# nimblephysics/nimblephysics

Measured on NVIDIA H100. Metric: differentiable world-steps/sec (fwd+bwd), batched Atlas, higher is better.
Workload: dtype f32

## Files before the change

nimblephysics_b200/csrc/nb2_dyn.cuh:

```cuda
#pragma once
#include <stddef.h>

#include "nb2_math.cuh"
#include "nb2_model.h"
#include "../../include/nb2.h"

namespace nb2 {

#define NB2_FWD_BODY_WORDS 16
struct FwdLayout {
  int oQ, oV, oAct, oBody, oSlot, oFree, total;
};
NB2_HD FwdLayout fwd_layout(int nb, int n, int nslots, int nfree) {
  FwdLayout L;
  L.oQ = 0; L.oV = n; L.oAct = 2 * n; L.oBody = 3 * n;
  L.oSlot = L.oBody + NB2_FWD_BODY_WORDS * nb;
  L.oFree = L.oSlot + 27 * nslots;
  L.total = L.oFree + 18 * nfree;
  return L;
}
struct BwdLayout {
  int oGQ, oGV, oLam, oQb, oVb, oSt, oAct, oBody, oSlot, oFree, total;
};
NB2_HD BwdLayout bwd_layout(int nb, int n, int nslots, int nfree, int slotw = 18) {
  BwdLayout L;
  L.oGQ = 0; L.oGV = n; L.oLam = 2 * n; L.oQb = 3 * n; L.oVb = 4 * n; L.oSt = 5 * n; L.oAct = 7 * n; L.oBody = 8 * n;
  L.oSlot = L.oBody + 7 * nb;
  L.oFree = L.oSlot + slotw * nslots;
  L.total = L.oFree + 6 * nfree;
  return L;
}

template <class R, int ST> NB2_HD V6<R> ld6(const R* p) {
  V6<R> v; v.a.x = p[0]; v.a.y = p[ST]; v.a.z = p[2 * ST]; v.l.x = p[3 * ST]; v.l.y = p[4 * ST]; v.l.z = p[5 * ST]; return v;
}
template <class R, int ST> NB2_HD void st6(R* p, const V6<R>& v) {
  p[0] = v.a.x; p[ST] = v.a.y; p[2 * ST] = v.a.z; p[3 * ST] = v.l.x; p[4 * ST] = v.l.y; p[5 * ST] = v.l.z;
}
template <class R, int ST> NB2_HD void add6(R* p, const V6<R>& v) {
  p[0] += v.a.x; p[ST] += v.a.y; p[2 * ST] += v.a.z; p[3 * ST] += v.l.x; p[4 * ST] += v.l.y; p[5 * ST] += v.l.z;
}
template <class R, int ST> NB2_HD SI<R> ldSI(const R* p) {
  SI<R> I;
  I.A.xx = p[0]; I.A.yy = p[ST]; I.A.zz = p[2 * ST]; I.A.xy = p[3 * ST]; I.A.xz = p[4 * ST]; I.A.yz = p[5 * ST];
  I.B.m00 = p[6 * ST]; I.B.m01 = p[7 * ST]; I.B.m02 = p[8 * ST]; I.B.m10 = p[9 * ST]; I.B.m11 = p[10 * ST]; I.B.m12 = p[11 * ST];
  I.B.m20 = p[12 * ST]; I.B.m21 = p[13 * ST]; I.B.m22 = p[14 * ST];
  I.C.xx = p[15 * ST]; I.C.yy = p[16 * ST]; I.C.zz = p[17 * ST]; I.C.xy = p[18 * ST]; I.C.xz = p[19 * ST]; I.C.yz = p[20 * ST];
  return I;
}
template <class R, int ST, bool ADD> NB2_HD void stSI(R* p, const SI<R>& I) {
#define NB2_W(k, val) if (ADD) p[(k) * ST] += (val); else p[(k) * ST] = (val);
  NB2_W(0, I.A.xx) NB2_W(1, I.A.yy) NB2_W(2, I.A.zz) NB2_W(3, I.A.xy) NB2_W(4, I.A.xz) NB2_W(5, I.A.yz)
  NB2_W(6, I.B.m00) NB2_W(7, I.B.m01) NB2_W(8, I.B.m02) NB2_W(9, I.B.m10) NB2_W(10, I.B.m11) NB2_W(11, I.B.m12)
  NB2_W(12, I.B.m20) NB2_W(13, I.B.m21) NB2_W(14, I.B.m22)
  NB2_W(15, I.C.xx) NB2_W(16, I.C.yy) NB2_W(17, I.C.zz) NB2_W(18, I.C.xy) NB2_W(19, I.C.xz) NB2_W(20, I.C.yz)
#undef NB2_W
}
template <class R> NB2_HD void sv_st6(R* sv, size_t B, int k, const V6<R>& v) {
  sv[(size_t)k * B] = v.a.x; sv[(size_t)(k + 1) * B] = v.a.y; sv[(size_t)(k + 2) * B] = v.a.z;
  sv[(size_t)(k + 3) * B] = v.l.x; sv[(size_t)(k + 4) * B] = v.l.y; sv[(size_t)(k + 5) * B] = v.l.z;
}
template <class R> NB2_HD V6<R> tof(const V6<R>& v) { return v; }
template <class R> NB2_HD V6<R> sv_ld6(const R* sv, size_t B, int k) {
  V6<R> v;
  v.a.x = (R)sv[(size_t)k * B]; v.a.y = (R)sv[(size_t)(k + 1) * B]; v.a.z = (R)sv[(size_t)(k + 2) * B];
  v.l.x = (R)sv[(size_t)(k + 3) * B]; v.l.y = (R)sv[(size_t)(k + 4) * B]; v.l.z = (R)sv[(size_t)(k + 5) * B];
  return v;
}

#define NB2_BT_WORDS 22
template <class R> NB2_HD Xf<R> xtree(const Nb2ModelDev<R>& M, const R* bt, int i) {
  Xf<R> T;
  if (bt) {
    const R* t = bt + NB2_BT_WORDS * i;
    T.R_.m00 = t[0]; T.R_.m01 = t[1]; T.R_.m02 = t[2]; T.R_.m10 = t[3]; T.R_.m11 = t[4]; T.R_.m12 = t[5];
    T.R_.m20 = t[6]; T.R_.m21 = t[7]; T.R_.m22 = t[8];
    T.p = mk3<R>(t[9], t[10], t[11]);
    return T;
  }
  T.R_.m00 = M.Xtree[i][0]; T.R_.m01 = M.Xtree[i][1]; T.R_.m02 = M.Xtree[i][2];
  T.R_.m10 = M.Xtree[i][3]; T.R_.m11 = M.Xtree[i][4]; T.R_.m12 = M.Xtree[i][5];
  T.R_.m20 = M.Xtree[i][6]; T.R_.m21 = M.Xtree[i][7]; T.R_.m22 = M.Xtree[i][8];
  T.p = mk3<R>(M.Xtree[i][9], M.Xtree[i][10], M.Xtree[i][11]);
  return T;
}
template <class R> NB2_HD Xf<R> xtree(const Nb2ModelDev<R>& M, int i) { return xtree<R>(M, (const R*)nullptr, i); }
template <class R> NB2_HD Xf<R> xf_rev(const Nb2ModelDev<R>& M, const R* bt, int i, R s, R c) {
  Xf<R> X = xtree(M, bt, i), T;
  T.R_.m00 = c * X.R_.m00 + s * X.R_.m01; T.R_.m01 = c * X.R_.m01 - s * X.R_.m00; T.R_.m02 = X.R_.m02;
  T.R_.m10 = c * X.R_.m10 + s * X.R_.m11; T.R_.m11 = c * X.R_.m11 - s * X.R_.m10; T.R_.m12 = X.R_.m12;
  T.R_.m20 = c * X.R_.m20 + s * X.R_.m21; T.R_.m21 = c * X.R_.m21 - s * X.R_.m20; T.R_.m22 = X.R_.m22;
  T.p = X.p;
  return T;
}
template <class R> NB2_HD Xf<R> xf_rev(const Nb2ModelDev<R>& M, int i, R s, R c) { return xf_rev<R>(M, (const R*)nullptr, i, s, c); }
template <class R> NB2_HD Xf<R> xf_pris(const Nb2ModelDev<R>& M, const R* bt, int i, R d) {
  Xf<R> T = xtree(M, bt, i);
  T.p.x += T.R_.m02 * d; T.p.y += T.R_.m12 * d; T.p.z += T.R_.m22 * d;
  return T;
}
template <class R> NB2_HD Xf<R> xf_pris(const Nb2ModelDev<R>& M, int i, R d) { return xf_pris<R>(M, (const R*)nullptr, i, d); }
template <class R> NB2_HD void inertia_of(const Nb2ModelDev<R>& M, const R* bt, const double* wi, size_t wiB, int i, R* m, V3<R>* h, S3<R>* Ib) {
  if (wi) {
    const double* t = wi + (size_t)(10 * i) * wiB;
    *m = (R)t[0]; *h = mk3<R>((R)t[wiB], (R)t[2 * wiB], (R)t[3 * wiB]);
    Ib->xx = (R)t[4 * wiB]; Ib->yy = (R)t[5 * wiB]; Ib->zz = (R)t[6 * wiB];
    Ib->xy = (R)t[7 * wiB]; Ib->xz = (R)t[8 * wiB]; Ib->yz = (R)t[9 * wiB];
    return;
  }
  if (bt) {
    const R* t = bt + NB2_BT_WORDS * i + 12;
    *m = t[0]; *h = mk3<R>(t[1], t[2], t[3]);
    Ib->xx = t[4]; Ib->yy = t[5]; Ib->zz = t[6]; Ib->xy = t[7]; Ib->xz = t[8]; Ib->yz = t[9];
    return;
  }
  *m = M.inertia[i][0];
  *h = mk3<R>(M.inertia[i][1], M.inertia[i][2], M.inertia[i][3]);
  Ib->xx = M.inertia[i][4]; Ib->yy = M.inertia[i][5]; Ib->zz = M.inertia[i][6];
  Ib->xy = M.inertia[i][7]; Ib->xz = M.inertia[i][8]; Ib->yz = M.inertia[i][9];
}
template <class R, int ST> NB2_HD Xf<R> ldXf(const R* p) {
  Xf<R> T;
  T.R_.m00 = p[0]; T.R_.m01 = p[ST]; T.R_.m02 = p[2 * ST]; T.R_.m10 = p[3 * ST]; T.R_.m11 = p[4 * ST]; T.R_.m12 = p[5 * ST];
  T.R_.m20 = p[6 * ST]; T.R_.m21 = p[7 * ST]; T.R_.m22 = p[8 * ST];
  T.p = mk3<R>(p[9 * ST], p[10 * ST], p[11 * ST]);
  return T;
}
template <class R, int ST> NB2_HD void stXf(R* p, const Xf<R>& T) {
  p[0] = T.R_.m00; p[ST] = T.R_.m01; p[2 * ST] = T.R_.m02; p[3 * ST] = T.R_.m10; p[4 * ST] = T.R_.m11; p[5 * ST] = T.R_.m12;
  p[6 * ST] = T.R_.m20; p[7 * ST] = T.R_.m21; p[8 * ST] = T.R_.m22; p[9 * ST] = T.p.x; p[10 * ST] = T.p.y; p[11 * ST] = T.p.z;
}
template <class R, int ST> NB2_HD Xf<R> body_xf_fwd(const Nb2ModelDev<R>& M, const R* bt, int i, const R* scr, const FwdLayout& L) {
  const int jt = M.jtype[i];
  if (jt == NB2_JT_REV) { const R* b = scr + (size_t)(L.oBody + NB2_FWD_BODY_WORDS * i + 6) * ST; return xf_rev(M, bt, i, b[0], b[ST]); }
  if (jt == NB2_JT_PRIS) return xf_pris(M, bt, i, scr[(size_t)(L.oQ + M.dof_off[i]) * ST]);
  return ldXf<R, ST>(scr + (size_t)(L.oFree + 18 * M.free_idx[i]) * ST);
}
template <class R> NB2_HD V6<R> S_times(int jt, R x) {
  V6<R> s = zero6<R>();
  if (jt == NB2_JT_REV) s.a.z = x; else s.l.z = x;
  return s;
}
template <class R> NB2_HD R S_dot(int jt, const V6<R>& f) { return (jt == NB2_JT_REV) ? f.a.z : f.l.z; }

template <class R, int ST> NB2_HD R tau_of(const Nb2ModelDev<R>& M, const R* scr, int oAct, int d) {
  const int a = M.act_of_dof[d];
  return (a >= 0) ? scr[(size_t)(oAct + a) * ST] : R(0);
}

template <class R, int ST>
NB2_HD void fwd_pass1(const Nb2ModelDev<R>& M, R* scr, int lo, int hi, const R* bt = nullptr) {
  const int nb = M.nb, n = M.ndof;
  const FwdLayout L = fwd_layout(nb, n, M.nslots, M.nfree);
  const R dt = M.dt;
  (void)nb; (void)n; (void)dt;
  for (int i = lo; i < hi; i++) {
    const int jt = M.jtype[i], p = M.parent[i], o = M.dof_off[i];
    R* bs = scr + (size_t)(L.oBody + NB2_FWD_BODY_WORDS * i) * ST;
    V6<R> Vp = (p >= 0) ? ld6<R, ST>(scr + (size_t)(L.oBody + NB2_FWD_BODY_WORDS * p) * ST) : zero6<R>();
    V6<R> V;
    if (jt == NB2_JT_REV) {
      R s, c; nb2_sincos(scr[(size_t)(L.oQ + o) * ST], &s, &c);
      bs[6 * ST] = s; bs[7 * ST] = c;
      V = AdInvT(xf_rev(M, bt, i, s, c), Vp);
      V.a.z += scr[(size_t)(L.oV + o) * ST];
    } else if (jt == NB2_JT_PRIS) {
      V = AdInvT(xf_pris(M, bt, i, scr[(size_t)(L.oQ + o) * ST]), Vp);
      V.l.z += scr[(size_t)(L.oV + o) * ST];
    } else {
      const R* q = scr + (size_t)(L.oQ + o) * ST;
      const R* v = scr + (size_t)(L.oV + o) * ST;
      Xf<R> X = xtree(M, bt, i), T;
      M3<R> Rq = expmap(mk3<R>(q[0], q[ST], q[2 * ST]));
      T.R_ = mul(X.R_, Rq);
      T.p = mul(X.R_, mk3<R>(q[3 * ST], q[4 * ST], q[5 * ST])) + X.p;
      stXf<R, ST>(scr + (size_t)(L.oFree + 18 * M.free_idx[i]) * ST, T);
      V = AdInvT(T, Vp) + ld6<R, ST>(v);
    }
    st6<R, ST>(bs, V);
  }

}

template <class R, int ST>
NB2_HD void fwd_pass2(const Nb2ModelDev<R>& M, R* scr, R* sv, size_t B, bool save, int lo, int hi, const R* bt = nullptr, R* iinv_out = nullptr,
                      const double* wi = nullptr, size_t wiB = 0) {
  const int nb = M.nb, n = M.ndof;
  const FwdLayout L = fwd_layout(nb, n, M.nslots, M.nfree);
  const R dt = M.dt;
  (void)nb; (void)n; (void)dt;
  SI<R> hI = zeroSI<R>();
  V6<R> hp = zero6<R>();
  bool hvalid = false;
  for (int i = hi - 1; i >= lo; i--) {
    const int jt = M.jtype[i], p = M.parent[i], o = M.dof_off[i], fl = M.flags[i];
    R* bs = scr + (size_t)(L.oBody + NB2_FWD_BODY_WORDS * i) * ST;
    R m; V3<R> h; S3<R> Ib; inertia_of(M, bt, wi, wiB, i, &m, &h, &Ib);
    const V6<R> V = ld6<R, ST>(bs);
    SI<R> IA = rigidSI(m, h, Ib);
    V6<R> pA = crf(V, mulG(m, h, Ib, V));
    if (hvalid) { IA = IA + hI; pA = pA + hp; }
    if (fl & NB2_F_HAS_SLOT) {
      for (int k = 0; k < M.slot_count[i]; k++) {
        const R* sl = scr + (size_t)(L.oSlot + 27 * (M.slot_self[i] + k)) * ST;
        IA = IA + ldSI<R, ST>(sl);
        pA = pA + ld6<R, ST>(sl + 21 * ST);
      }
    }
    SI<R> Pi; V6<R> beta;
    if (jt != NB2_JT_FREE) {
      const R vq = scr[(size_t)(L.oV + o) * ST];
      V6<R> U, eta;
      R D;
      if (jt == NB2_JT_REV) {
        U.a = mk3<R>(IA.A.xz, IA.A.yz, IA.A.zz); U.l = mk3<R>(IA.B.m20, IA.B.m21, IA.B.m22); D = IA.A.zz;
        eta.a = mk3<R>(V.a.y * vq, -V.a.x * vq, R(0)); eta.l = mk3<R>(V.l.y * vq, -V.l.x * vq, R(0));
      } else {
        U.a = mk3<R>(IA.B.m02, IA.B.m12, IA.B.m22); U.l = mk3<R>(IA.C.xz, IA.C.yz, IA.C.zz); D = IA.C.zz;
        eta.a = zero3<R>(); eta.l = mk3<R>(V.a.y * vq, -V.a.x * vq, R(0));
      }
      const R psi = nb2_rcp(D);
      const R qv = scr[(size_t)(L.oQ + o) * ST];
      const R u = tau_of<R, ST>(M, scr, L.oAct, o) - M.spring[o] * (qv - M.rest[o] + vq * dt) - M.damping[o] * vq
                  - (dot(U, eta) + S_dot(jt, pA));
      st6<R, ST>(bs + 8 * ST, U);
      bs[14 * ST] = psi; bs[15 * ST] = u;
      if (p >= 0) {
        const R k = -psi;
        Pi = IA;
        Pi.A.xx += k * U.a.x * U.a.x; Pi.A.yy += k * U.a.y * U.a.y; Pi.A.zz += k * U.a.z * U.a.z;
        Pi.A.xy += k * U.a.x * U.a.y; Pi.A.xz += k * U.a.x * U.a.z; Pi.A.yz += k * U.a.y * U.a.z;
        Pi.C.xx += k * U.l.x * U.l.x; Pi.C.yy += k * U.l.y * U.l.y; Pi.C.zz += k * U.l.z * U.l.z;
        Pi.C.xy += k * U.l.x * U.l.y; Pi.C.xz += k * U.l.x * U.l.z; Pi.C.yz += k * U.l.y * U.l.z;
        Pi.B.m00 += k * U.a.x * U.l.x; Pi.B.m01 += k * U.a.x * U.l.y; Pi.B.m02 += k * U.a.x * U.l.z;
        Pi.B.m10 += k * U.a.y * U.l.x; Pi.B.m11 += k * U.a.y * U.l.y; Pi.B.m12 += k * U.a.y * U.l.z;
        Pi.B.m20 += k * U.a.z * U.l.x; Pi.B.m21 += k * U.a.z * U.l.y; Pi.B.m22 += k * U.a.z * U.l.z;
        beta = pA + mul(IA, eta) + U * (psi * u);
      }
    } else {
      const R* q = scr + (size_t)(L.oQ + o) * ST;
      const R* v = scr + (size_t)(L.oV + o) * ST;
      R t[6];
#pragma unroll
      for (int k = 0; k < 6; k++) t[k] = tau_of<R, ST>(M, scr, L.oAct, o + k);
      const V6<R> Vj = ld6<R, ST>(v);
      const V6<R> eta = ad(V, Vj);
      const V6<R> bf = mul(IA, eta) + pA;
      V6<R> u;
      u.a.x = t[0] - M.spring[o] * (q[0] - M.rest[o] + Vj.a.x * dt) - M.damping[o] * Vj.a.x - bf.a.x;
      u.a.y = t[1] - M.spring[o + 1] * (q[ST] - M.rest[o + 1] + Vj.a.y * dt) - M.damping[o + 1] * Vj.a.y - bf.a.y;
      u.a.z = t[2] - M.spring[o + 2] * (q[2 * ST] - M.rest[o + 2] + Vj.a.z * dt) - M.damping[o + 2] * Vj.a.z - bf.a.z;
      u.l.x = t[3] - M.spring[o + 3] * (q[3 * ST] - M.rest[o + 3] + Vj.l.x * dt) - M.damping[o + 3] * Vj.l.x - bf.l.x;
      u.l.y = t[4] - M.spring[o + 4] * (q[4 * ST] - M.rest[o + 4] + Vj.l.y * dt) - M.damping[o + 4] * Vj.l.y - bf.l.y;
      u.l.z = t[5] - M.spring[o + 5] * (q[5 * ST] - M.rest[o + 5] + Vj.l.z * dt) - M.damping[o + 5] * Vj.l.z - bf.l.z;
      const SI<R> Iinv = spd6_inverse(IA);
      const V6<R> y = mul(Iinv, u);
      st6<R, ST>(scr + (size_t)(L.oFree + 18 * M.free_idx[i] + 12) * ST, y);
      if (iinv_out) stSI<R, 1, false>(iinv_out + 21 * M.free_idx[i], Iinv);
      if (save) {
        const int k0 = nb * 21 + M.free_idx[i] * 33;
        R* s = sv + (size_t)k0 * B;
        s[0] = (R)Iinv.A.xx; s[B] = (R)Iinv.A.yy; s[2 * B] = (R)Iinv.A.zz; s[3 * B] = (R)Iinv.A.xy; s[4 * B] = (R)Iinv.A.xz; s[5 * B] = (R)Iinv.A.yz;
        s[6 * B] = (R)Iinv.B.m00; s[7 * B] = (R)Iinv.B.m01; s[8 * B] = (R)Iinv.B.m02; s[9 * B] = (R)Iinv.B.m10; s[10 * B] = (R)Iinv.B.m11; s[11 * B] = (R)Iinv.B.m12;
        s[12 * B] = (R)Iinv.B.m20; s[13 * B] = (R)Iinv.B.m21; s[14 * B] = (R)Iinv.B.m22;
        s[15 * B] = (R)Iinv.C.xx; s[16 * B] = (R)Iinv.C.yy; s[17 * B] = (R)Iinv.C.zz; s[18 * B] = (R)Iinv.C.xy; s[19 * B] = (R)Iinv.C.xz; s[20 * B] = (R)Iinv.C.yz;
      }
      if (p >= 0) { Pi = zeroSI<R>(); beta = bf + u; }
    }
    hvalid = false;
    if (p >= 0) {
      const Xf<R> T = body_xf_fwd<R, ST>(M, bt, i, scr, L);
      const SI<R> Ic = xform_inertia(T, Pi);
      const V6<R> pc = dAdInvT(T, beta);
      if (fl & NB2_F_HANDOFF) { hI = Ic; hp = pc; hvalid = true; }
      else {
        R* sl = scr + (size_t)(L.oSlot + 27 * M.slot_parent[i]) * ST;
        stSI<R, ST, false>(sl, Ic); st6<R, ST>(sl + 21 * ST, pc);
      }
    }
  }

}

template <class R, int ST>
NB2_HD void fwd_pass3(const Nb2ModelDev<R>& M, R* scr, R* sv, size_t B, bool save, int lo, int hi, const R* bt = nullptr) {
  const int nb = M.nb, n = M.ndof;
  const FwdLayout L = fwd_layout(nb, n, M.nslots, M.nfree);
  const R dt = M.dt;
  (void)nb; (void)n; (void)dt;
  V6<R> A0; A0.a = zero3<R>(); A0.l = mk3<R>(-M.gravity[0], -M.gravity[1], -M.gravity[2]);
  for (int i = lo; i < hi; i++) {
    const int jt = M.jtype[i], p = M.parent[i], o = M.dof_off[i];
    R* bs = scr + (size_t)(L.oBody + NB2_FWD_BODY_WORDS * i) * ST;
    const Xf<R> T = body_xf_fwd<R, ST>(M, bt, i, scr, L);
    const V6<R> Ap = AdInvT(T, (p >= 0) ? ld6<R, ST>(scr + (size_t)(L.oBody + NB2_FWD_BODY_WORDS * p) * ST) : A0);
    const V6<R> V = ld6<R, ST>(bs);
    V6<R> A;
    if (jt != NB2_JT_FREE) {
      const R vq = scr[(size_t)(L.oV + o) * ST], qv = scr[(size_t)(L.oQ + o) * ST];
      const V6<R> U = ld6<R, ST>(bs + 8 * ST);
      const R psi = bs[14 * ST], u = bs[15 * ST];
      const R qdd = psi * (u - dot(U, Ap));
      A = Ap;
      if (jt == NB2_JT_REV) { A.a.z += qdd; A.a.x += V.a.y * vq; A.a.y -= V.a.x * vq; A.l.x += V.l.y * vq; A.l.y -= V.l.x * vq; }
      else { A.l.z += qdd; A.l.x += V.a.y * vq; A.l.y -= V.a.x * vq; }
      scr[(size_t)(L.oQ + o) * ST] = qv + vq * dt;
      scr[(size_t)(L.oV + o) * ST] = vq + qdd * dt;
      if (save) {
        R* s = sv + (size_t)(i * 21) * B;
        sv_st6(s, B, 0, tof(V)); sv_st6(s, B, 6, tof(A)); sv_st6(s, B, 12, tof(U));
        s[18 * B] = (R)psi;
        s[19 * B] = (jt == NB2_JT_REV) ? (R)bs[6 * ST] : R(0); s[20 * B] = (jt == NB2_JT_REV) ? (R)bs[7 * ST] : R(0);
        sv[(size_t)(nb * 21 + M.nfree * 33 + o) * B] = qdd;
      }
    } else {
      const R* q = scr + (size_t)(L.oQ + o) * ST;
      const R* fr = scr + (size_t)(L.oFree + 18 * M.free_idx[i]) * ST;
      const V6<R> Vj = ld6<R, ST>(scr + (size_t)(L.oV + o) * ST);
      const V6<R> y = ld6<R, ST>(fr + 12 * ST);
      const V6<R> qdd = y - Ap;
      A = y + ad(V, Vj);
      const V3<R> phi = mk3<R>(q[0], q[ST], q[2 * ST]);
      const M3<R> Rq = expmap(phi);
      const V3<R> phin = logmap(mul(Rq, expmap(Vj.a * dt)));
      const V3<R> pn = mk3<R>(q[3 * ST], q[4 * ST], q[5 * ST]) + mul(Rq, Vj.l * dt);
      R* qo = scr + (size_t)(L.oQ + o) * ST;
      R* vo = scr + (size_t)(L.oV + o) * ST;
      qo[0] = phin.x; qo[ST] = phin.y; qo[2 * ST] = phin.z; qo[3 * ST] = pn.x; qo[4 * ST] = pn.y; qo[5 * ST] = pn.z;
      vo[0] = Vj.a.x + qdd.a.x * dt; vo[ST] = Vj.a.y + qdd.a.y * dt; vo[2 * ST] = Vj.a.z + qdd.a.z * dt;
      vo[3 * ST] = Vj.l.x + qdd.l.x * dt; vo[4 * ST] = Vj.l.y + qdd.l.y * dt; vo[5 * ST] = Vj.l.z + qdd.l.z * dt;
      if (save) {
        R* s = sv + (size_t)(i * 21) * B;
        sv_st6(s, B, 0, tof(V)); sv_st6(s, B, 6, tof(A));
        for (int k = 12; k < 21; k++) s[(size_t)k * B] = R(0);
        R* sf = sv + (size_t)(nb * 21 + M.free_idx[i] * 33 + 21) * B;
        for (int k = 0; k < 12; k++) sf[(size_t)k * B] = fr[(size_t)k * ST];
        R* sq = sv + (size_t)(nb * 21 + M.nfree * 33 + o) * B;
        sq[0] = qdd.a.x; sq[B] = qdd.a.y; sq[2 * B] = qdd.a.z; sq[3 * B] = qdd.l.x; sq[4 * B] = qdd.l.y; sq[5 * B] = qdd.l.z;
      }
    }
    st6<R, ST>(bs, A);
  }
}

#define NB2_IO_UNROLL 4
struct alignas(16) F4 { float x, y, z, w; };
NB2_HD unsigned fast_div(unsigned idx, unsigned magic) {
#ifdef __CUDA_ARCH__
  return __umulhi(idx, magic);
#else
  return (unsigned)(((unsigned long long)idx * magic) >> 32);
#endif
}
template <class F> NB2_HD void group_read(const float* src, int tot, int tid, int nthr, const F& f) {
  if ((((size_t)src) & 15) == 0) {
    const F4* s4 = reinterpret_cast<const F4*>(src);
    const int tot4 = tot >> 2;
    for (int base = tid; base < tot4; base += nthr * NB2_IO_UNROLL) {
      F4 v[NB2_IO_UNROLL];
#pragma unroll
      for (int u = 0; u < NB2_IO_UNROLL; u++) { const int j = base + u * nthr; if (j < tot4) v[u] = s4[j]; }
#pragma unroll
      for (int u = 0; u < NB2_IO_UNROLL; u++) {
        const int j = base + u * nthr;
        if (j < tot4) { f(4 * j, v[u].x); f(4 * j + 1, v[u].y); f(4 * j + 2, v[u].z); f(4 * j + 3, v[u].w); }
      }
    }
    for (int idx = 4 * tot4 + tid; idx < tot; idx += nthr) f(idx, src[idx]);
  } else {
    for (int base = tid; base < tot; base += nthr * NB2_IO_UNROLL) {
      float v[NB2_IO_UNROLL];
#pragma unroll
      for (int u = 0; u < NB2_IO_UNROLL; u++) { const int idx = base + u * nthr; v[u] = (idx < tot) ? src[idx] : 0.f; }
#pragma unroll
      for (int u = 0; u < NB2_IO_UNROLL; u++) { const int idx = base + u * nthr; if (idx < tot) f(idx, v[u]); }
    }
  }
}
template <class F> NB2_HD void group_write(float* dst, int tot, int tid, int nthr, const F& f) {
  if ((((size_t)dst) & 15) == 0) {
    F4* d4 = reinterpret_cast<F4*>(dst);
    const int tot4 = tot >> 2;
    for (int j = tid; j < tot4; j += nthr) { F4 v; v.x = f(4 * j); v.y = f(4 * j + 1); v.z = f(4 * j + 2); v.w = f(4 * j + 3); d4[j] = v; }
    for (int idx = 4 * tot4 + tid; idx < tot; idx += nthr) dst[idx] = f(idx);
  } else {
    for (int idx = tid; idx < tot; idx += nthr) dst[idx] = f(idx);
  }
}

template <class R, int ST> struct WordScatter {
  R* scr0; int width, base; unsigned magic; float* copy;
  NB2_HD void operator()(int idx, float v) const {
    const int slot = (int)fast_div((unsigned)idx, magic), d = idx - slot * width;
    scr0[(size_t)(base + d) * ST + slot] = (R)v;
    if (copy) copy[idx] = v;
  }
};
template <class R, int ST> struct WordGather {
  const R* scr0; int width, base; unsigned magic;
  NB2_HD float operator()(int idx) const {
    const int slot = (int)fast_div((unsigned)idx, magic), d = idx - slot * width;
    return (float)scr0[(size_t)(base + d) * ST + slot];
  }
};

template <class R, int ST>
NB2_HD void fwd_load(const Nb2ModelDev<R>& M, R* scr0, const float* st0, const float* act0, int nworlds, int tid, int nthr,
                     float* st_copy0 = nullptr, float* act_copy0 = nullptr) {
  const int n2 = 2 * M.ndof, na = M.na;
  const FwdLayout L = fwd_layout(M.nb, M.ndof, M.nslots, M.nfree);
  WordScatter<R, ST> ss{scr0, n2, L.oQ, M.magic_n2, st_copy0};
  group_read(st0, nworlds * n2, tid, nthr, ss);
  WordScatter<R, ST> as{scr0, na, L.oAct, M.magic_na, act_copy0};
  group_read(act0, nworlds * na, tid, nthr, as);
}
template <class R, int ST>
NB2_HD void fwd_store(const Nb2ModelDev<R>& M, const R* scr0, float* out0, int nworlds, int tid, int nthr) {
  const int n2 = 2 * M.ndof;
  const FwdLayout L = fwd_layout(M.nb, M.ndof, M.nslots, M.nfree);
  WordGather<R, ST> sg{scr0, n2, L.oQ, M.magic_n2};
  group_write(out0, nworlds * n2, tid, nthr, sg);
}

#define NB2_FWD_STAGES 8
#define NB2_FWD_SYNC_MASK 0x6Bu
#define NB2_FWD_SYNC_MASK_1LANE 0x41u
template <class R, int ST>
NB2_HD void world_forward_stage(const Nb2ModelDev<R>& M, R* scr, R* sv, size_t B, bool save, int lane, int stage, const R* bt = nullptr, R* iinv_out = nullptr,
                                const double* wi = nullptr, size_t wiB = 0) {
  const int pass = (stage + 1) >> 1;
  const bool trunk = (stage == 1) | (stage == 4) | (stage == 5);
  if (trunk && lane != 0) return;
  const int nr = trunk ? M.trunk_n : M.limb_n[lane];
  for (int rr = 0; rr < nr; rr++) {
    const int r = (pass == 2) ? nr - 1 - rr : rr;
    const int lo = trunk ? M.trunk_lo[r] : M.limb_lo[lane][r], hi = trunk ? M.trunk_hi[r] : M.limb_hi[lane][r];
    if (pass == 1) fwd_pass1<R, ST>(M, scr, lo, hi, bt);
    else if (pass == 2) fwd_pass2<R, ST>(M, scr, sv, B, save, lo, hi, bt, iinv_out, wi, wiB);
    else fwd_pass3<R, ST>(M, scr, sv, B, save, lo, hi, bt);
  }
}

template <class T, int ST> struct SPd { T* p; NB2_HD T& operator[](int i) const { return p[(size_t)i * ST]; } NB2_HD SPd operator+(int k) const { SPd r; r.p = p + (size_t)k * ST; return r; } };
template <int ST>
struct BwdContactData {
  SPd<double, ST> Aacc, Uplus, aeff, vplus, inj, JcTmu;
  const int16_t* inj_of_body;
  int active; int error;
  int bounce = 0, pass2 = 0;
};

NB2_HD float mul_rn(float a, float b) {
#ifdef __CUDA_ARCH__
  return __fmul_rn(a, b);
#else
  return a * b;
#endif
}
NB2_HD double mul_rn(double a, double b) {
#ifdef __CUDA_ARCH__
  return __dmul_rn(a, b);
#else
  return a * b;
#endif
}
template <class R> NB2_HD V3<R> cross_rn(const V3<R>& a, const V3<R>& b) {
  return mk3<R>(mul_rn(a.y, b.z) - mul_rn(a.z, b.y), mul_rn(a.z, b.x) - mul_rn(a.x, b.z), mul_rn(a.x, b.y) - mul_rn(a.y, b.x));
}
template <class R> NB2_HD void inertia_param_form(const V6<R>& Y, const V6<R>& X, R* t) {
  t[0] = mul_rn(Y.l.x, X.l.x) + mul_rn(Y.l.y, X.l.y) + mul_rn(Y.l.z, X.l.z);
  const V3<R> dh = cross_rn(X.l, Y.a) + cross_rn(Y.l, X.a);
  t[1] = dh.x; t[2] = dh.y; t[3] = dh.z;
  t[4] = mul_rn(Y.a.x, X.a.x); t[5] = mul_rn(Y.a.y, X.a.y); t[6] = mul_rn(Y.a.z, X.a.z);
  t[7] = mul_rn(Y.a.x, X.a.y) + mul_rn(Y.a.y, X.a.x); t[8] = mul_rn(Y.a.x, X.a.z) + mul_rn(Y.a.z, X.a.x);
  t[9] = mul_rn(Y.a.y, X.a.z) + mul_rn(Y.a.z, X.a.y);
}

template <class R, int ST, bool CONTACT>
NB2_HD void bwd_B1(const Nb2ModelDev<R>& M, R* scr, const float* st, const R* sv, size_t B, int lo, int hi, const R* bt = nullptr) {
  const int nb = M.nb, n = M.ndof;
  constexpr int SLOTW = CONTACT ? 42 : 18;
  const BwdLayout L = bwd_layout(nb, n, M.nslots, M.nfree, SLOTW);
  const R dt = M.dt;
  const int kFree = nb * 21, kQdd = nb * 21 + M.nfree * 33;
  (void)n; (void)dt; (void)kFree; (void)kQdd;
  V6<R> hp = zero6<R>();
  bool hvalid = false;
  for (int i = hi - 1; i >= lo; i--) {
    const int jt = M.jtype[i], p = M.parent[i], o = M.dof_off[i], fl = M.flags[i];
    const R* s = sv + (size_t)(i * 21) * B;
    V6<R> pI = hvalid ? hp : zero6<R>();
    if (fl & NB2_F_HAS_SLOT)
      for (int k = 0; k < M.slot_count[i]; k++) pI = pI + ld6<R, ST>(scr + (size_t)(L.oSlot + SLOTW * (M.slot_self[i] + k)) * ST);
    V6<R> beta;
    if (jt != NB2_JT_FREE) {
      const R up = scr[(size_t)(L.oGV + o) * ST] - S_dot(jt, pI);
      scr[(size_t)(L.oBody + 7 * i) * ST] = up;
      if (p >= 0) beta = pI + sv_ld6<R>(s, B, 12) * ((R)s[18 * B] * up);
    } else {
      const V6<R> up = ld6<R, ST>(scr + (size_t)(L.oGV + o) * ST) - pI;
      st6<R, ST>(scr + (size_t)(L.oFree + 6 * M.free_idx[i]) * ST, up);
      if (p >= 0) beta = pI + up;
    }
    hvalid = false;
    if (p >= 0) {
      Xf<R> T;
      if (jt == NB2_JT_REV) T = xf_rev(M, bt, i, (R)s[19 * B], (R)s[20 * B]);
      else if (jt == NB2_JT_PRIS) T = xf_pris(M, bt, i, scr[(size_t)(L.oSt + o) * ST]);
      else { R t12[12]; for (int k = 0; k < 12; k++) t12[k] = (R)sv[(size_t)(kFree + M.free_idx[i] * 33 + 21 + k) * B]; T = ldXf<R, 1>(t12); }
      const V6<R> pc = dAdInvT(T, beta);
      if (fl & NB2_F_HANDOFF) { hp = pc; hvalid = true; }
      else {
        R* sl = scr + (size_t)(L.oSlot + SLOTW * M.slot_parent[i]) * ST;
        st6<R, ST>(sl, pc);
      }
    }
  }
}

template <class R, int ST, bool CONTACT>
NB2_HD void bwd_B2(const Nb2ModelDev<R>& M, R* scr, const float* st, const R* sv, size_t B, int lo, int hi, const R* bt = nullptr) {
  const int nb = M.nb, n = M.ndof;
  constexpr int SLOTW = CONTACT ? 42 : 18;
  const BwdLayout L = bwd_layout(nb, n, M.nslots, M.nfree, SLOTW);
  const R dt = M.dt;
  const int kFree = nb * 21, kQdd = nb * 21 + M.nfree * 33;
  (void)n; (void)dt; (void)kFree; (void)kQdd;
  for (int i = lo; i < hi; i++) {
    const int jt = M.jtype[i], p = M.parent[i], o = M.dof_off[i];
    const R* s = sv + (size_t)(i * 21) * B;
    R* bs = scr + (size_t)(L.oBody + 7 * i) * ST;
    V6<R> W;
    if (jt != NB2_JT_FREE) {
      Xf<R> T = (jt == NB2_JT_REV) ? xf_rev(M, bt, i, (R)s[19 * B], (R)s[20 * B]) : xf_pris(M, bt, i, scr[(size_t)(L.oSt + o) * ST]);
      W = (p >= 0) ? AdInvT(T, ld6<R, ST>(scr + (size_t)(L.oBody + 7 * p + 1) * ST)) : zero6<R>();
      const R lam = (R)s[18 * B] * (bs[0] - dot(sv_ld6<R>(s, B, 12), W));
      scr[(size_t)(L.oLam + o) * ST] = lam;
      if (jt == NB2_JT_REV) W.a.z += lam; else W.l.z += lam;
    } else {
      const R* sf = sv + (size_t)(kFree + M.free_idx[i] * 33) * B;
      R t12[12]; for (int k = 0; k < 12; k++) t12[k] = (R)sf[(size_t)(21 + k) * B];
      const Xf<R> T = ldXf<R, 1>(t12);
      const V6<R> Wp = (p >= 0) ? AdInvT(T, ld6<R, ST>(scr + (size_t)(L.oBody + 7 * p + 1) * ST)) : zero6<R>();
      R i21[21]; for (int k = 0; k < 21; k++) i21[k] = (R)sf[(size_t)k * B];
      const SI<R> Iinv = ldSI<R, 1>(i21);
      W = mul(Iinv, ld6<R, ST>(scr + (size_t)(L.oFree + 6 * M.free_idx[i]) * ST));
      st6<R, ST>(scr + (size_t)(L.oLam + o) * ST, W - Wp);
    }
    st6<R, ST>(bs + ST, W);
  }
}

template <class R, int ST, bool CONTACT>
NB2_HD void bwd_B3(const Nb2ModelDev<R>& M, R* scr, const float* st, const R* sv, size_t B, const BwdContactData<ST>& cd, int lo, int hi,
                   float* gI = nullptr, const R* bt = nullptr, size_t gIB = 0, const double* wi = nullptr, size_t wiB = 0, double* gIa = nullptr) {
  const int nb = M.nb, n = M.ndof;
  constexpr int SLOTW = CONTACT ? 42 : 18;
  const BwdLayout L = bwd_layout(nb, n, M.nslots, M.nfree, SLOTW);
  const R dt = M.dt;
  const int kFree = nb * 21, kQdd = nb * 21 + M.nfree * 33;
  (void)n; (void)dt; (void)kFree; (void)kQdd;
  V6<R> hA = zero6<R>(), hV = zero6<R>(), hf = zero6<R>();
  V6<R> hUw = zero6<R>(), hUp = zero6<R>(), hG = zero6<R>(), hH = zero6<R>();
  bool hvalid = false;
  for (int i = hi - 1; i >= lo; i--) {
    const int jt = M.jtype[i], p = M.parent[i], o = M.dof_off[i], fl = M.flags[i];
    const R* s = sv + (size_t)(i * 21) * B;
    R m; V3<R> h; S3<R> Ib; inertia_of(M, bt, wi, wiB, i, &m, &h, &Ib);
    const V6<R> V = sv_ld6<R>(s, B, 0);
    V6<R> A = sv_ld6<R>(s, B, 6);
    if (CONTACT && cd.active && !cd.pass2) { const auto a6 = cd.Aacc + 6 * i; A.a = mk3<R>((R)a6[0], (R)a6[1], (R)a6[2]); A.l = mk3<R>((R)a6[3], (R)a6[4], (R)a6[5]); }
    const V6<R> W = ld6<R, ST>(scr + (size_t)(L.oBody + 7 * i + 1) * ST);
    const V6<R> GV = mulG(m, h, Ib, V);
    V6<R> f = mulG(m, h, Ib, A) + crf(V, GV);
    if (gI || gIa) {
      V6<R> Y2;
      Y2.a = cross_rn(V.a, W.a);
      Y2.l = cross_rn(V.a, W.l) + cross_rn(V.l, W.a);
      R t[10];
      inertia_param_form(W, A, t);
      R t2[10];
      inertia_param_form(Y2, V, t2);
#pragma unroll
      for (int k = 0; k < 10; k++) {
        const float gk = (float)(-dt * (t[k] - t2[k]));
        if (gIa) gIa[(size_t)(10 * i + k) * gIB] += (double)gk;
        else if (CONTACT && cd.pass2) gI[(size_t)(10 * i + k) * gIB] += gk; else gI[(size_t)(10 * i + k) * gIB] = gk;
      }
    }
    V6<R> Abar = mulG(m, h, Ib, W);
    V6<R> Vbar = mulG(m, h, Ib, ad(W, V)) - crf(W, GV);
    if (hvalid) { Abar = Abar + hA; Vbar = Vbar + hV; f = f + hf; }
    V6<R> Uw = zero6<R>(), Up = zero6<R>(), Gc = zero6<R>(), Hc = zero6<R>();
    if (CONTACT && cd.active) {
      const int ci = cd.inj_of_body[i];
      if (ci >= 0) {
        const auto b24 = cd.inj + 24 * ci;
        Uw.a = mk3<R>((R)b24[0], (R)b24[1], (R)b24[2]); Uw.l = mk3<R>((R)b24[3], (R)b24[4], (R)b24[5]);
        Up.a = mk3<R>((R)b24[6], (R)b24[7], (R)b24[8]); Up.l = mk3<R>((R)b24[9], (R)b24[10], (R)b24[11]);
        Gc.a = mk3<R>((R)b24[12], (R)b24[13], (R)b24[14]); Gc.l = mk3<R>((R)b24[15], (R)b24[16], (R)b24[17]);
        Hc.a = mk3<R>((R)b24[18], (R)b24[19], (R)b24[20]); Hc.l = mk3<R>((R)b24[21], (R)b24[22], (R)b24[23]);
      }
      if (hvalid) { Uw = Uw + hUw; Up = Up + hUp; Gc = Gc + hG; Hc = Hc + hH; }
    }
    if (fl & NB2_F_HAS_SLOT) {
      for (int k = 0; k < M.slot_count[i]; k++) {
        const R* sl = scr + (size_t)(L.oSlot + SLOTW * (M.slot_self[i] + k)) * ST;
        Abar = Abar + ld6<R, ST>(sl); Vbar = Vbar + ld6<R, ST>(sl + 6 * ST); f = f + ld6<R, ST>(sl + 12 * ST);
        if (CONTACT && cd.active) { Uw = Uw + ld6<R, ST>(sl + 18 * ST); Up = Up + ld6<R, ST>(sl + 24 * ST); Gc = Gc + ld6<R, ST>(sl + 30 * ST); Hc = Hc + ld6<R, ST>(sl + 36 * ST); }
      }
    }
    V6<R> Sv, Sa, Sl;
    Xf<R> T;
    if (jt != NB2_JT_FREE) {
      Sv = S_times<R>(jt, scr[(size_t)(L.oSt + n + o) * ST]);
      Sa = S_times<R>(jt, (CONTACT && cd.active && !cd.pass2) ? (R)cd.aeff[o] : (R)sv[(size_t)(kQdd + o) * B]);
      Sl = S_times<R>(jt, scr[(size_t)(L.oLam + o) * ST]);
      T = (jt == NB2_JT_REV) ? xf_rev(M, bt, i, (R)s[19 * B], (R)s[20 * B]) : xf_pris(M, bt, i, scr[(size_t)(L.oSt + o) * ST]);
    } else {
      Sv.a = mk3<R>(scr[(size_t)(L.oSt + n + o) * ST], scr[(size_t)(L.oSt + n + o + 1) * ST], scr[(size_t)(L.oSt + n + o + 2) * ST]); Sv.l = mk3<R>(scr[(size_t)(L.oSt + n + o + 3) * ST], scr[(size_t)(L.oSt + n + o + 4) * ST], scr[(size_t)(L.oSt + n + o + 5) * ST]);
      Sa = sv_ld6<R>(sv + (size_t)(kQdd + o) * B, B, 0);
      if (CONTACT && cd.active && !cd.pass2) { const auto a6 = cd.aeff + o; Sa.a = mk3<R>((R)a6[0], (R)a6[1], (R)a6[2]); Sa.l = mk3<R>((R)a6[3], (R)a6[4], (R)a6[5]); }
      Sl = ld6<R, ST>(scr + (size_t)(L.oLam + o) * ST);
      R t12[12]; for (int k = 0; k < 12; k++) t12[k] = (R)sv[(size_t)(kFree + M.free_idx[i] * 33 + 21 + k) * B];
      T = ldXf<R, 1>(t12);
    }
    Vbar = Vbar + crf(Sv, Abar);
    const V6<R> vb6 = Vbar - crf(V, Abar);
    const V6<R> Alam = A - Sa - ad(V, Sv), Vlam = V - Sv, Wlam = W - Sl;
    V6<R> c6 = zero6<R>() - (crf(Alam, Abar) + crf(Vlam, Vbar) + crf(Wlam, f));
    if (CONTACT && cd.active) {
      V6<R> Upl; { const auto u6 = cd.Uplus + 6 * i; Upl.a = mk3<R>((R)u6[0], (R)u6[1], (R)u6[2]); Upl.l = mk3<R>((R)u6[3], (R)u6[4], (R)u6[5]); }
      V6<R> Svp;
      if (jt != NB2_JT_FREE) Svp = S_times<R>(jt, (R)cd.vplus[o]);
      else { const auto v6p = cd.vplus + o; Svp.a = mk3<R>((R)v6p[0], (R)v6p[1], (R)v6p[2]); Svp.l = mk3<R>((R)v6p[3], (R)v6p[4], (R)v6p[5]); }
      c6 = c6 - crf(Wlam, Uw) - crf(Upl - Svp, Up) + Gc;
      if (!cd.pass2) {
        if (jt != NB2_JT_FREE) cd.JcTmu[o] = (double)S_dot(jt, Hc);
        else { auto j6 = cd.JcTmu + o; j6[0] = (double)Hc.a.x; j6[1] = (double)Hc.a.y; j6[2] = (double)Hc.a.z; j6[3] = (double)Hc.l.x; j6[4] = (double)Hc.l.y; j6[5] = (double)Hc.l.z; }
      }
    }
    const bool add = CONTACT && cd.pass2;
    if (jt != NB2_JT_FREE) {
      const R vb = S_dot(jt, vb6), qb = S_dot(jt, c6);
      scr[(size_t)(L.oVb + o) * ST] = add ? scr[(size_t)(L.oVb + o) * ST] + vb : vb;
      scr[(size_t)(L.oQb + o) * ST] = add ? scr[(size_t)(L.oQb + o) * ST] + qb : qb;
    } else {
      const V3<R> phi = mk3<R>(scr[(size_t)(L.oSt + o) * ST], scr[(size_t)(L.oSt + o + 1) * ST], scr[(size_t)(L.oSt + o + 2) * ST]);
      V6<R> qb, vb = vb6;
      qb.a = mulT(so3_Jr(phi), c6.a);
      qb.l = mul(expmap(phi), c6.l);
      if (add) { vb = vb + ld6<R, ST>(scr + (size_t)(L.oVb + o) * ST); qb = qb + ld6<R, ST>(scr + (size_t)(L.oQb + o) * ST); }
      st6<R, ST>(scr + (size_t)(L.oVb + o) * ST, vb);
      st6<R, ST>(scr + (size_t)(L.oQb + o) * ST, qb);
    }
    hvalid = false;
    if (p >= 0) {
      const V6<R> cA = dAdInvT(T, Abar), cV = dAdInvT(T, Vbar), cf = dAdInvT(T, f);
      V6<R> cUw, cUp, cG, cH;
      if (CONTACT && cd.active) { cUw = dAdInvT(T, Uw); cUp = dAdInvT(T, Up); cG = dAdInvT(T, Gc); cH = dAdInvT(T, Hc); }
      if (fl & NB2_F_HANDOFF) { hA = cA; hV = cV; hf = cf; if (CONTACT && cd.active) { hUw = cUw; hUp = cUp; hG = cG; hH = cH; } hvalid = true; }
      else {
        R* sl = scr + (size_t)(L.oSlot + SLOTW * M.slot_parent[i]) * ST;
        st6<R, ST>(sl, cA); st6<R, ST>(sl + 6 * ST, cV); st6<R, ST>(sl + 12 * ST, cf);
        if (CONTACT && cd.active) { st6<R, ST>(sl + 18 * ST, cUw); st6<R, ST>(sl + 24 * ST, cUp); st6<R, ST>(sl + 30 * ST, cG); st6<R, ST>(sl + 36 * ST, cH); }
      }
    }
  }
}

template <class R, int ST>
NB2_HD void finish_dof(const Nb2ModelDev<R>& M, R* scr, const BwdLayout& L, int d, R gq_, R gv_, R lam) {
  const int n = M.ndof;
  float gq = (float)gq_, gv = (float)gv_;
  const float qd = (float)scr[(size_t)(L.oSt + d) * ST], vd = (float)scr[(size_t)(L.oSt + n + d) * ST];
  if (qd == M.pos_lo[d] && gq > 0.f) gq = 0.f;
  if (qd == M.pos_hi[d] && gq < 0.f) gq = 0.f;
  if (vd == M.vel_lo[d] && gv > 0.f) gv = 0.f;
  if (vd == M.vel_hi[d] && gv < 0.f) gv = 0.f;
  scr[(size_t)(L.oQb + d) * ST] = (R)gq;
  scr[(size_t)(L.oVb + d) * ST] = (R)gv;
  const int a = M.act_of_dof[d];
  if (a >= 0) {
    float gt = (float)(M.dt * lam);
    const float fd = (float)scr[(size_t)(L.oAct + a) * ST];
    if (fd == M.force_lo[d] && gt > 0.f) gt = 0.f;
    if (fd == M.force_hi[d] && gt < 0.f) gt = 0.f;
    scr[(size_t)(L.oAct + a) * ST] = (R)gt;
  }
}

template <class R, int ST, bool CONTACT>
NB2_HD void bwd_assemble(const Nb2ModelDev<R>& M, R* scr, const float* st, const BwdContactData<ST>& cd, int lo, int hi) {
  const int nb = M.nb, n = M.ndof;
  constexpr int SLOTW = CONTACT ? 42 : 18;
  const BwdLayout L = bwd_layout(nb, n, M.nslots, M.nfree, SLOTW);
  const R dt = M.dt;
  const int kFree = nb * 21, kQdd = nb * 21 + M.nfree * 33;
  (void)n; (void)dt; (void)kFree; (void)kQdd;
  for (int i = lo; i < hi; i++) {
    const int jt = M.jtype[i], o = M.dof_off[i];
    if (jt != NB2_JT_FREE) {
      const R lam = scr[(size_t)(L.oLam + o) * ST];
      const R gq = scr[(size_t)(L.oGQ + o) * ST];
      R gv = scr[(size_t)(L.oGV + o) * ST];
      if (CONTACT && cd.active) gv -= (R)cd.JcTmu[o];
      finish_dof<R, ST>(M, scr, L, o, gq - dt * (scr[(size_t)(L.oQb + o) * ST] + M.spring[o] * lam),
                        dt * gq + gv - dt * (scr[(size_t)(L.oVb + o) * ST] + (M.damping[o] + dt * M.spring[o]) * lam), lam);
    } else {
      const V3<R> phi = mk3<R>(scr[(size_t)(L.oSt + o) * ST], scr[(size_t)(L.oSt + o + 1) * ST], scr[(size_t)(L.oSt + o + 2) * ST]);
      const V3<R> w = mk3<R>(scr[(size_t)(L.oSt + n + o) * ST], scr[(size_t)(L.oSt + n + o + 1) * ST], scr[(size_t)(L.oSt + n + o + 2) * ST]);
      const V3<R> vl = mk3<R>(scr[(size_t)(L.oSt + n + o + 3) * ST], scr[(size_t)(L.oSt + n + o + 4) * ST], scr[(size_t)(L.oSt + n + o + 5) * ST]);
      const M3<R> Rq = expmap(phi), E = expmap(w * dt);
      const V3<R> phin = logmap(mul(Rq, E));
      const V6<R> g = ld6<R, ST>(scr + (size_t)(L.oGQ + o) * ST);
      const V3<R> t = mulT(so3_Jr_inv(phin), g.a);
      V6<R> gq, gvp;
      gq.a = mulT(so3_Jr(phi), mul(E, t) + cross(vl * dt, mulT(Rq, g.l)));
      gq.l = g.l;
      gvp.a = mulT(so3_Jr(w * dt), t) * dt;
      gvp.l = mulT(Rq, g.l) * dt;
      const V6<R> lam = ld6<R, ST>(scr + (size_t)(L.oLam + o) * ST);
      const V6<R> qb = ld6<R, ST>(scr + (size_t)(L.oQb + o) * ST), vb = ld6<R, ST>(scr + (size_t)(L.oVb + o) * ST);
      V6<R> gv = ld6<R, ST>(scr + (size_t)(L.oGV + o) * ST);
      if (CONTACT && cd.active) { const auto j6 = cd.JcTmu + o; gv.a = gv.a - mk3<R>((R)j6[0], (R)j6[1], (R)j6[2]); gv.l = gv.l - mk3<R>((R)j6[3], (R)j6[4], (R)j6[5]); }
      R lamv[6] = {lam.a.x, lam.a.y, lam.a.z, lam.l.x, lam.l.y, lam.l.z};
      R qbv[6] = {qb.a.x, qb.a.y, qb.a.z, qb.l.x, qb.l.y, qb.l.z}, vbv[6] = {vb.a.x, vb.a.y, vb.a.z, vb.l.x, vb.l.y, vb.l.z};
      R gqv[6] = {gq.a.x, gq.a.y, gq.a.z, gq.l.x, gq.l.y, gq.l.z}, gvpv[6] = {gvp.a.x, gvp.a.y, gvp.a.z, gvp.l.x, gvp.l.y, gvp.l.z};
      R gvv[6] = {gv.a.x, gv.a.y, gv.a.z, gv.l.x, gv.l.y, gv.l.z};
#pragma unroll
      for (int k = 0; k < 6; k++) {
        finish_dof<R, ST>(M, scr, L, o + k, gqv[k] - dt * (qbv[k] + M.spring[o + k] * lamv[k]),
                          gvpv[k] + gvv[k] - dt * (vbv[k] + (M.damping[o + k] + dt * M.spring[o + k]) * lamv[k]), lamv[k]);
      }
    }
  }
}

template <class R, int ST, bool CONTACT>
NB2_HD void bwd_load(const Nb2ModelDev<R>& M, R* scr0, const float* st0, const float* act0, const float* gnext0, int nworlds, int tid, int nthr) {
  const int n = M.ndof, n2 = 2 * n;
  constexpr int SLOTW = CONTACT ? 42 : 18;
  const BwdLayout L = bwd_layout(M.nb, n, M.nslots, M.nfree, SLOTW);
  WordScatter<R, ST> sg{scr0, n2, L.oGQ, M.magic_n2, nullptr};
  group_read(gnext0, nworlds * n2, tid, nthr, sg);
  WordScatter<R, ST> sx{scr0, n2, L.oSt, M.magic_n2, nullptr};
  group_read(st0, nworlds * n2, tid, nthr, sx);
  WordScatter<R, ST> sa{scr0, M.na, L.oAct, M.magic_na, nullptr};
  group_read(act0, nworlds * M.na, tid, nthr, sa);
}
struct NanGather { NB2_HD float operator()(int) const { return nanf(""); } };
template <class F> struct AddTo { F f; const float* dst; NB2_HD float operator()(int idx) const { return dst[idx] + f(idx); } };
template <class R, int ST, bool CONTACT>
NB2_HD void bwd_store(const Nb2ModelDev<R>& M, const R* scr0, float* gstate0, float* gaction0,
                      bool cd_error, int nworlds, int tid, int nthr, bool accumulate_state = false) {
  const int n = M.ndof, n2 = 2 * n, na = M.na;
  constexpr int SLOTW = CONTACT ? 42 : 18;
  const BwdLayout L = bwd_layout(M.nb, n, M.nslots, M.nfree, SLOTW);
  if (cd_error) {
    group_write(gstate0, nworlds * n2, tid, nthr, NanGather());
    group_write(gaction0, nworlds * na, tid, nthr, NanGather());
    return;
  }
  WordGather<R, ST> gs{scr0, n2, L.oQb, M.magic_n2};
  if (accumulate_state) {
    AddTo<WordGather<R, ST>> acc{gs, gstate0};
    group_write(gstate0, nworlds * n2, tid, nthr, acc);
  } else group_write(gstate0, nworlds * n2, tid, nthr, gs);
  WordGather<R, ST> ga{scr0, na, L.oAct, M.magic_na};
  group_write(gaction0, nworlds * na, tid, nthr, ga);
}

#define NB2_BWD_STAGES 10
#define NB2_BWD_SYNC_MASK 0x14Bu
#define NB2_BWD_SYNC_MASK_1LANE 0x101u
#define NB2_CBWD_ITERS 10
struct CBwdIter { int stage; bool second; };
NB2_HD constexpr CBwdIter cbwd_iter(int it) {
  return {(it < 4) ? it + 1 : (it == 4 || it == 6) ? 5 : (it == 5 || it == 7) ? 7 : (it == 8) ? 6 : 8, static_cast<bool>((it == 6) | (it == 7))};
}
template <class R, int ST, bool CONTACT = false>
NB2_HD void world_backward_stage(const Nb2ModelDev<R>& M, R* scr, const R* sv, size_t B, int lane, int stage, float* gI = nullptr, const R* bt = nullptr,
                                 size_t gIB = 0, const BwdContactData<ST>* cdp = nullptr, const double* wi = nullptr, size_t wiB = 0,
                                 double* gIa = nullptr) {
  const float* st = nullptr;
  BwdContactData<ST> cd;
  if (CONTACT && cdp) cd = *cdp; else { cd.active = 0; cd.error = 0; cd.inj_of_body = nullptr; }
  const int pass = (stage == 1 || stage == 2) ? 1 : (stage == 3 || stage == 4) ? 2 : (stage == 5 || stage == 7) ? 3 : 4;
  const bool trunk = (stage == 2) | (stage == 3) | (stage == 7) | (stage == 8);
  if (trunk && lane != 0) return;
  const int nr = trunk ? M.trunk_n : M.limb_n[lane];
  for (int rr = 0; rr < nr; rr++) {
    const int r = (pass == 1 || pass == 3) ? nr - 1 - rr : rr;
    const int lo = trunk ? M.trunk_lo[r] : M.limb_lo[lane][r], hi = trunk ? M.trunk_hi[r] : M.limb_hi[lane][r];
    if (pass == 1) bwd_B1<R, ST, CONTACT>(M, scr, st, sv, B, lo, hi, bt);
    else if (pass == 2) bwd_B2<R, ST, CONTACT>(M, scr, st, sv, B, lo, hi, bt);
    else if (pass == 3) bwd_B3<R, ST, CONTACT>(M, scr, st, sv, B, cd, lo, hi, gI, bt, gIB ? gIB : B, wi, wiB, gIa);
    else bwd_assemble<R, ST, CONTACT>(M, scr, st, cd, lo, hi);
  }
}

template <class R> NB2_HD R comp6(const V6<R>& v, int k) {
  return k == 0 ? v.a.x : k == 1 ? v.a.y : k == 2 ? v.a.z : k == 3 ? v.l.x : k == 4 ? v.l.y : v.l.z;
}
template <class R, int ST>
NB2_HD void id_rows_load(R* scr0, const R* src, int width, unsigned magic, int base, int nworlds, int tid, int nthr) {
  for (int idx = tid; idx < nworlds * width; idx += nthr) {
    const int slot = (int)fast_div((unsigned)idx, magic), d = idx - slot * width;
    scr0[(size_t)(base + d) * ST + slot] = src[idx];
  }
}
template <class R, int ST>
NB2_HD void id_rows_store(const R* scr0, R* dst, int width, unsigned magic, int base, int nworlds, int tid, int nthr) {
  for (int idx = tid; idx < nworlds * width; idx += nthr) {
    const int slot = (int)fast_div((unsigned)idx, magic), d = idx - slot * width;
    dst[idx] = scr0[(size_t)(base + d) * ST + slot];
  }
}

template <class R, int ST>
NB2_HD void id_pass_acc(const Nb2ModelDev<R>& M, R* scr, R* sv, size_t B, bool save, int lo, int hi, const R* bt) {
  const FwdLayout L = fwd_layout(M.nb, M.ndof, M.nslots, M.nfree);
  const R rdt = R(1) / M.dt;
  const int kFree = M.nb * 21, kQdd = M.nb * 21 + M.nfree * 33;
  V6<R> A0; A0.a = zero3<R>(); A0.l = mk3<R>(-M.gravity[0], -M.gravity[1], -M.gravity[2]);
  for (int i = lo; i < hi; i++) {
    const int jt = M.jtype[i], p = M.parent[i], o = M.dof_off[i];
    R* bs = scr + (size_t)(L.oBody + NB2_FWD_BODY_WORDS * i) * ST;
    const Xf<R> T = body_xf_fwd<R, ST>(M, bt, i, scr, L);
    const V6<R> Ap = AdInvT(T, (p >= 0) ? ld6<R, ST>(scr + (size_t)(L.oBody + NB2_FWD_BODY_WORDS * p + 8) * ST) : A0);
    const V6<R> V = ld6<R, ST>(bs);
    V6<R> A = Ap;
    if (jt != NB2_JT_FREE) {
      const R vq = scr[(size_t)(L.oV + o) * ST];
      const R a = (scr[(size_t)(L.oAct + o) * ST] - vq) * rdt;
      if (jt == NB2_JT_REV) { A.a.z += a; A.a.x += V.a.y * vq; A.a.y -= V.a.x * vq; A.l.x += V.l.y * vq; A.l.y -= V.l.x * vq; }
      else { A.l.z += a; A.l.x += V.a.y * vq; A.l.y -= V.a.x * vq; }
      if (save) sv[(size_t)(kQdd + o) * B] = a;
    } else {
      const V6<R> Vj = ld6<R, ST>(scr + (size_t)(L.oV + o) * ST);
      const V6<R> a = (ld6<R, ST>(scr + (size_t)(L.oAct + o) * ST) - Vj) * rdt;
      A = Ap + a + ad(V, Vj);
      if (save) {
        sv_st6(sv + (size_t)(kQdd + o) * B, B, 0, a);
        const R* fr = scr + (size_t)(L.oFree + 18 * M.free_idx[i]) * ST;
        R* sf = sv + (size_t)(kFree + M.free_idx[i] * 33 + 21) * B;
        for (int k = 0; k < 12; k++) sf[(size_t)k * B] = fr[(size_t)k * ST];
      }
    }
    st6<R, ST>(bs + 8 * ST, A);
    if (save) {
      R* s = sv + (size_t)(i * 21) * B;
      sv_st6(s, B, 0, V); sv_st6(s, B, 6, A);
      s[19 * B] = (jt == NB2_JT_REV) ? bs[6 * ST] : R(0); s[20 * B] = (jt == NB2_JT_REV) ? bs[7 * ST] : R(0);
    }
  }
}

template <class R, int ST>
NB2_HD void id_pass_force(const Nb2ModelDev<R>& M, R* scr, int lo, int hi, const R* bt, const double* wi, size_t wiB) {
  const FwdLayout L = fwd_layout(M.nb, M.ndof, M.nslots, M.nfree);
  const R dt = M.dt;
  V6<R> hf = zero6<R>();
  bool hvalid = false;
  for (int i = hi - 1; i >= lo; i--) {
    const int jt = M.jtype[i], p = M.parent[i], o = M.dof_off[i], fl = M.flags[i];
    const R* bs = scr + (size_t)(L.oBody + NB2_FWD_BODY_WORDS * i) * ST;
    R m; V3<R> h; S3<R> Ib; inertia_of(M, bt, wi, wiB, i, &m, &h, &Ib);
    const V6<R> V = ld6<R, ST>(bs), A = ld6<R, ST>(bs + 8 * ST);
    V6<R> f = mulG(m, h, Ib, A) + crf(V, mulG(m, h, Ib, V));
    if (hvalid) f = f + hf;
    if (fl & NB2_F_HAS_SLOT)
      for (int k = 0; k < M.slot_count[i]; k++) f = f + ld6<R, ST>(scr + (size_t)(L.oSlot + 27 * (M.slot_self[i] + k)) * ST);
    const int nd = (jt == NB2_JT_FREE) ? 6 : 1;
    for (int k = 0; k < nd; k++) {
      const int d = o + k;
      const R qd = scr[(size_t)(L.oQ + d) * ST], vd = scr[(size_t)(L.oV + d) * ST];
      const R fk = (jt == NB2_JT_FREE) ? comp6(f, k) : S_dot(jt, f);
      scr[(size_t)(L.oAct + d) * ST] = fk + M.spring[d] * (qd - M.rest[d] + vd * dt) + M.damping[d] * vd;
    }
    hvalid = false;
    if (p >= 0) {
      const V6<R> fc = dAdInvT(body_xf_fwd<R, ST>(M, bt, i, scr, L), f);
      if (fl & NB2_F_HANDOFF) { hf = fc; hvalid = true; }
      else st6<R, ST>(scr + (size_t)(L.oSlot + 27 * M.slot_parent[i]) * ST, fc);
    }
  }
}

#define NB2_ID_FWD_STAGES 6
#define NB2_ID_FWD_SYNC_MASK 0x1Bu
#define NB2_ID_FWD_SYNC_MASK_1LANE 0x11u
template <class R, int ST>
NB2_HD void id_forward_stage(const Nb2ModelDev<R>& M, R* scr, R* sv, size_t B, bool save, int lane, int stage, const R* bt,
                             const double* wi, size_t wiB) {
  const bool trunk = (stage == 1) | (stage == 4);
  if (trunk && lane != 0) return;
  const int nr = trunk ? M.trunk_n : M.limb_n[lane];
  for (int rr = 0; rr < nr; rr++) {
    const int r = (stage >= 3) ? nr - 1 - rr : rr;
    const int lo = trunk ? M.trunk_lo[r] : M.limb_lo[lane][r], hi = trunk ? M.trunk_hi[r] : M.limb_hi[lane][r];
    if (stage <= 2) { fwd_pass1<R, ST>(M, scr, lo, hi, bt); id_pass_acc<R, ST>(M, scr, sv, B, save, lo, hi, bt); }
    else id_pass_force<R, ST>(M, scr, lo, hi, bt, wi, wiB);
  }
}
template <class R, int ST>
NB2_HD void id_load(const Nb2ModelDev<R>& M, R* scr0, const R* st0, const R* nv0, int nworlds, int tid, int nthr) {
  const FwdLayout L = fwd_layout(M.nb, M.ndof, M.nslots, M.nfree);
  id_rows_load<R, ST>(scr0, st0, 2 * M.ndof, M.magic_n2, L.oQ, nworlds, tid, nthr);
  id_rows_load<R, ST>(scr0, nv0, M.ndof, M.magic_n, L.oAct, nworlds, tid, nthr);
}
template <class R, int ST>
NB2_HD void id_store(const Nb2ModelDev<R>& M, const R* scr0, R* tau0, int nworlds, int tid, int nthr) {
  const FwdLayout L = fwd_layout(M.nb, M.ndof, M.nslots, M.nfree);
  id_rows_store<R, ST>(scr0, tau0, M.ndof, M.magic_n, L.oAct, nworlds, tid, nthr);
}

NB2_HD int id_bwd_words(int nb, int n, int nslots, int nfree) { return bwd_layout(nb, n, nslots, nfree).total + 6 * nslots; }
template <class R, int ST>
NB2_HD Xf<R> id_saved_xf(const Nb2ModelDev<R>& M, const R* bt, int i, const R* scr, const BwdLayout& L, const R* sv, size_t B) {
  const int jt = M.jtype[i];
  const R* s = sv + (size_t)(i * 21) * B;
  if (jt == NB2_JT_REV) return xf_rev(M, bt, i, s[19 * B], s[20 * B]);
  if (jt == NB2_JT_PRIS) return xf_pris(M, bt, i, scr[(size_t)(L.oSt + M.dof_off[i]) * ST]);
  R t12[12];
  for (int k = 0; k < 12; k++) t12[k] = sv[(size_t)(M.nb * 21 + M.free_idx[i] * 33 + 21 + k) * B];
  return ldXf<R, 1>(t12);
}
template <class R, int ST>
NB2_HD void id_bwd_field(const Nb2ModelDev<R>& M, R* scr, const R* sv, size_t B, int lo, int hi, const R* bt) {
  const BwdLayout L = bwd_layout(M.nb, M.ndof, M.nslots, M.nfree);
  for (int i = lo; i < hi; i++) {
    const int jt = M.jtype[i], p = M.parent[i], o = M.dof_off[i];
    V6<R> W = (p >= 0) ? AdInvT(id_saved_xf<R, ST>(M, bt, i, scr, L, sv, B), ld6<R, ST>(scr + (size_t)(L.oBody + 7 * p + 1) * ST)) : zero6<R>();
    if (jt != NB2_JT_FREE) W = W + S_times<R>(jt, scr[(size_t)(L.oLam + o) * ST]);
    else W = W + ld6<R, ST>(scr + (size_t)(L.oLam + o) * ST);
    st6<R, ST>(scr + (size_t)(L.oBody + 7 * i + 1) * ST, W);
  }
}
template <class R, int ST>
NB2_HD void id_bwd_mass(const Nb2ModelDev<R>& M, R* scr, const R* sv, size_t B, int lo, int hi, const R* bt, const double* wi, size_t wiB,
                        double* gI, size_t gIB) {
  const BwdLayout L = bwd_layout(M.nb, M.ndof, M.nslots, M.nfree);
  const int oS = L.total;
  const R dt = M.dt, rdt = R(1) / M.dt;
  V6<R> hA = zero6<R>();
  bool hvalid = false;
  for (int i = hi - 1; i >= lo; i--) {
    const int jt = M.jtype[i], p = M.parent[i], o = M.dof_off[i], fl = M.flags[i];
    R m; V3<R> h; S3<R> Ib; inertia_of(M, bt, wi, wiB, i, &m, &h, &Ib);
    const V6<R> W = ld6<R, ST>(scr + (size_t)(L.oBody + 7 * i + 1) * ST);
    V6<R> Ab = mulG(m, h, Ib, W);
    if (hvalid) Ab = Ab + hA;
    if (fl & NB2_F_HAS_SLOT)
      for (int k = 0; k < M.slot_count[i]; k++) Ab = Ab + ld6<R, ST>(scr + (size_t)(oS + 6 * (M.slot_self[i] + k)) * ST);
    if (gI) {
      const R* s = sv + (size_t)(i * 21) * B;
      const V6<R> V = sv_ld6<R>(s, B, 0), A = sv_ld6<R>(s, B, 6);
      V6<R> Y2;
      Y2.a = cross_rn(V.a, W.a);
      Y2.l = cross_rn(V.a, W.l) + cross_rn(V.l, W.a);
      R t[10], t2[10];
      inertia_param_form(W, A, t);
      inertia_param_form(Y2, V, t2);
      for (int k = 0; k < 10; k++) gI[(size_t)(10 * i + k) * gIB] = (double)(t[k] - t2[k]);
    }
    const int nd = (jt == NB2_JT_FREE) ? 6 : 1;
    for (int k = 0; k < nd; k++) {
      const int d = o + k;
      const R ml = ((jt == NB2_JT_FREE) ? comp6(Ab, k) : S_dot(jt, Ab)) * rdt, lam = scr[(size_t)(L.oLam + d) * ST];
      scr[(size_t)(L.oQb + d) * ST] += M.spring[d] * lam;
      scr[(size_t)(L.oVb + d) * ST] += (M.damping[d] + dt * M.spring[d]) * lam - ml;
      scr[(size_t)(L.oGQ + d) * ST] = ml;
    }
    hvalid = false;
    if (p >= 0) {
      const V6<R> cA = dAdInvT(id_saved_xf<R, ST>(M, bt, i, scr, L, sv, B), Ab);
      if (fl & NB2_F_HANDOFF) { hA = cA; hvalid = true; }
      else st6<R, ST>(scr + (size_t)(oS + 6 * M.slot_parent[i]) * ST, cA);
    }
  }
}
#define NB2_ID_BWD_STAGES 8
#define NB2_ID_BWD_SYNC_MASK 0x53u
#define NB2_ID_BWD_SYNC_MASK_1LANE 0x41u
template <class R, int ST>
NB2_HD void id_backward_stage(const Nb2ModelDev<R>& M, R* scr, const R* sv, size_t B, int lane, int stage, const R* bt,
                              const double* wi, size_t wiB, double* gI, size_t gIB) {
  const bool trunk = (stage == 1) | (stage == 5) | (stage == 6);
  if (trunk && lane != 0) return;
  BwdContactData<ST> cd; cd.active = 0; cd.error = 0; cd.inj_of_body = nullptr;
  const int nr = trunk ? M.trunk_n : M.limb_n[lane];
  for (int rr = 0; rr < nr; rr++) {
    const int r = (stage >= 3) ? nr - 1 - rr : rr;
    const int lo = trunk ? M.trunk_lo[r] : M.limb_lo[lane][r], hi = trunk ? M.trunk_hi[r] : M.limb_hi[lane][r];
    if (stage <= 2) id_bwd_field<R, ST>(M, scr, sv, B, lo, hi, bt);
    else if (stage == 3 || stage == 5) bwd_B3<R, ST, false>(M, scr, nullptr, sv, B, cd, lo, hi, nullptr, bt, B, wi, wiB, nullptr);
    else id_bwd_mass<R, ST>(M, scr, sv, B, lo, hi, bt, wi, wiB, gI, gIB);
  }
}
template <class R, int ST>
NB2_HD void id_bwd_load(const Nb2ModelDev<R>& M, R* scr0, const R* st0, const R* gtau0, int nworlds, int tid, int nthr) {
  const BwdLayout L = bwd_layout(M.nb, M.ndof, M.nslots, M.nfree);
  id_rows_load<R, ST>(scr0, st0, 2 * M.ndof, M.magic_n2, L.oSt, nworlds, tid, nthr);
  id_rows_load<R, ST>(scr0, gtau0, M.ndof, M.magic_n, L.oLam, nworlds, tid, nthr);
}
template <class R, int ST>
NB2_HD void id_bwd_store(const Nb2ModelDev<R>& M, const R* scr0, R* gstate0, R* gnext0, int nworlds, int tid, int nthr) {
  const BwdLayout L = bwd_layout(M.nb, M.ndof, M.nslots, M.nfree);
  id_rows_store<R, ST>(scr0, gstate0, 2 * M.ndof, M.magic_n2, L.oQb, nworlds, tid, nthr);
  id_rows_store<R, ST>(scr0, gnext0, M.ndof, M.magic_n, L.oGQ, nworlds, tid, nthr);
}

struct CidChain {
  int n;
  int16_t body[NB2_MAX_BODIES];
};
template <class R> NB2_HD int cid_chain(const Nb2ModelDev<R>& M, int body, CidChain* c) {
  if (body < 0 || body >= M.nb) return -1;
  int k = 0;
  for (int i = body; i >= 0; i = M.parent[i]) k++;
  c->n = k;
  for (int i = body; i >= 0; i = M.parent[i]) c->body[--k] = (int16_t)i;
  return M.jtype[c->body[0]] == NB2_JT_FREE ? c->n : -1;
}
template <class R> NB2_HD Xf<R> cid_xf(const Nb2ModelDev<R>& M, int i, const R* q) {
  const int jt = M.jtype[i], o = M.dof_off[i];
  if (jt == NB2_JT_REV) { R s, c; nb2_sincos(q[o], &s, &c); return xf_rev(M, i, s, c); }
  if (jt == NB2_JT_PRIS) return xf_pris(M, i, q[o]);
  const Xf<R> X = xtree(M, i);
  Xf<R> T;
  T.R_ = mul(X.R_, expmap(mk3<R>(q[o], q[o + 1], q[o + 2])));
  T.p = mul(X.R_, mk3<R>(q[o + 3], q[o + 4], q[o + 5])) + X.p;
  return T;
}
template <class R> NB2_HD V6<R> row6(const R* p) { V6<R> v; v.a = mk3<R>(p[0], p[1], p[2]); v.l = mk3<R>(p[3], p[4], p[5]); return v; }
template <class R> NB2_HD void put6(R* p, const V6<R>& v) { p[0] = v.a.x; p[1] = v.a.y; p[2] = v.a.z; p[3] = v.l.x; p[4] = v.l.y; p[5] = v.l.z; }
template <class R> NB2_HD void cid_sub_joint_force(const Nb2ModelDev<R>& M, int i, const V6<R>& F, R* tau) {
  const int jt = M.jtype[i], o = M.dof_off[i];
  if (jt == NB2_JT_FREE) { for (int k = 0; k < 6; k++) tau[o + k] -= comp6(F, k); }
  else tau[o] -= S_dot(jt, F);
}
template <class R> NB2_HD void cid_free_q_grad(const R* q, int o, const V6<R>& c, R* gq) {
  const V3<R> phi = mk3<R>(q[o], q[o + 1], q[o + 2]);
  const V3<R> ga = mulT(so3_Jr(phi), c.a), gl = mul(expmap(phi), c.l);
  gq[o] += ga.x; gq[o + 1] += ga.y; gq[o + 2] += ga.z; gq[o + 3] += gl.x; gq[o + 4] += gl.y; gq[o + 5] += gl.z;
}

template <class R, class Op> NB2_HD void cid_walk(const Nb2ModelDev<R>& M, const CidChain& c, const R* q, V6<R> F, Op op) {
  for (int k = 1; k < c.n; k++) {
    const int i = c.body[k];
    F = dAdT(cid_xf(M, i, q), F);
    op(i, F);
  }
}
template <class R> NB2_HD void cid_walk_tau(const Nb2ModelDev<R>& M, const CidChain& c, const R* q, const V6<R>& Fr, R* tau) {
  cid_walk(M, c, q, Fr, [&](int i, const V6<R>& F) { cid_sub_joint_force(M, i, F, tau); });
}

template <class R> NB2_HD void cid_forward(const Nb2ModelDev<R>& M, const CidChain& c, const R* q, R* tau, R* wrench) {
  const int r = c.body[0], o = M.dof_off[r];
  const V6<R> F = row6(tau + o);
// ... 157 lines not shown
```

nimblephysics_b200/csrc/nb2_kernels.cu:

```cuda
#include <cuda_runtime.h>
#include <stdio.h>
#include <stdlib.h>

#include <atomic>
#include <mutex>
#include <string>
#include <type_traits>
#include <vector>

#include "../../include/nb2.h"
#include "nb2_dyn.cuh"
#include "nb2_mm.cuh"
#include "nb2_cw.cuh"
#include "nb2_host_model.h"

static thread_local std::string g_err;
static std::atomic<long long> g_launches{0};

#define NB2_CUDA(call)                                                                           \
  do {                                                                                           \
    cudaError_t e_ = (call);                                                                     \
    if (e_ != cudaSuccess) {                                                                     \
      g_err = std::string(#call) + ": " + cudaGetErrorString(e_);                                \
      return NB2_ERR_CUDA;                                                                       \
    }                                                                                            \
  } while (0)

namespace {

template <int K> struct CoopShape {
  static constexpr int WPW = 32 / K;
  static constexpr int ST = (K == 1) ? 32 : WPW + 1;
};

template <int K> __host__ __device__ constexpr int body_table_words(int nb) { return (K > 1) ? ((nb * NB2_BT_WORDS + 3) & ~3) : 0; }
template <class R, int K>
__device__ __forceinline__ const R* stage_body_table(const Nb2ModelDev<R>& M, R* tab) {
  if constexpr (K == 1) return nullptr;
  else {
  using U = std::conditional_t<sizeof(R) == 4, float2, double>;
  constexpr int XU = 12 * sizeof(R) / sizeof(U), IU = 10 * sizeof(R) / sizeof(U), BU = XU + IU;
  static_assert(offsetof(Nb2ModelDev<R>, Xtree) % sizeof(U) == 0 && offsetof(Nb2ModelDev<R>, inertia) % sizeof(U) == 0, "unaligned body tables");
  const U* xs = reinterpret_cast<const U*>(&M.Xtree[0][0]);
  const U* is = reinterpret_cast<const U*>(&M.inertia[0][0]);
  U* t = reinterpret_cast<U*>(tab);
  for (int k = threadIdx.x; k < M.nb * BU; k += blockDim.x) {
    const int i = k / BU, j = k - i * BU;
    t[k] = (j < XU) ? xs[i * XU + j] : is[i * IU + j - XU];
  }
  __syncthreads();
  return tab;
  }
}

__device__ __forceinline__ unsigned smem_u32(const void* p) { return (unsigned)__cvta_generic_to_shared(p); }
__device__ __forceinline__ void mbar_init(unsigned long long* bar) {
  asm volatile("mbarrier.init.shared::cta.b64 [%0], 1;" ::"r"(smem_u32(bar)));
  asm volatile("fence.mbarrier_init.release.cluster;" ::: "memory");
}
__device__ __forceinline__ void mbar_expect_tx(unsigned long long* bar, unsigned bytes) {
  asm volatile("mbarrier.arrive.expect_tx.shared::cta.b64 _, [%0], %1;" ::"r"(smem_u32(bar)), "r"(bytes) : "memory");
}
__device__ __forceinline__ void bulk_g2s(void* dst, const void* src, unsigned bytes, unsigned long long* bar) {
  asm volatile("cp.async.bulk.shared::cluster.global.mbarrier::complete_tx::bytes [%0], [%1], %2, [%3];" ::"r"(smem_u32(dst)),
               "l"(__cvta_generic_to_global(src)), "r"(bytes), "r"(smem_u32(bar))
               : "memory");
}
__device__ __forceinline__ void mbar_wait(unsigned long long* bar, unsigned parity) {
  for (int it = 0; it < (1 << 20); it++) {
    unsigned ok;
    asm volatile("{ .reg .pred p; mbarrier.try_wait.parity.shared::cta.b64 p, [%1], %2; selp.u32 %0, 1, 0, p; }" : "=r"(ok) : "r"(smem_u32(bar)), "r"(parity) : "memory");
    if (ok) return;
  }
  __trap();
}
__device__ __forceinline__ bool bulk_ok(const void* p, size_t bytes) { return ((reinterpret_cast<size_t>(p) | bytes) & 15) == 0 && bytes > 0; }
template <int K> __host__ __device__ constexpr size_t staging_bytes(int floats_per_world) {
  return (((size_t)floats_per_world * CoopShape<K>::WPW * sizeof(float) + 15) & ~(size_t)15) + 16;
}

#ifdef NB2_STEP_CLOCKS
#define NB2_CLK_WARPS 8
#define NB2_CLK_EVERY 64
#define NB2_CLK_SLOTS 16
__device__ long long nb2_step_clk[2][NB2_CLK_WARPS][NB2_CLK_SLOTS];
#define NB2_CLK(dir, k)                                                                                                   \
  do {                                                                                                                    \
    const int w_ = blockIdx.x * (blockDim.x >> 5) + (threadIdx.x >> 5);                                                   \
    if ((threadIdx.x & 31) == 0 && w_ % NB2_CLK_EVERY == 0 && w_ / NB2_CLK_EVERY < NB2_CLK_WARPS) nb2_step_clk[dir][w_ / NB2_CLK_EVERY][k] = clock64(); \
  } while (0)
#else
#define NB2_CLK(dir, k)
#endif

template <class R, int K, bool PW>
__global__ void __launch_bounds__(128)
k_step_fwd(const __grid_constant__ Nb2ModelDev<R> M, int B, int w0, int count, const float* __restrict__ state,
           const float* __restrict__ action, float* __restrict__ next, R* __restrict__ saved, int words,
           float* __restrict__ state_copy, float* __restrict__ action_copy, const double* __restrict__ winertia) {
  extern __shared__ __align__(16) unsigned char nb2_smem[];
  NB2_CLK(0, 0);
  constexpr int WPW = CoopShape<K>::WPW, ST = CoopShape<K>::ST;
  const int li = threadIdx.x & 31, slot = li / K, lane = li % K;
  const int g0 = (blockIdx.x * (blockDim.x >> 5) + (threadIdx.x >> 5)) * WPW;
  const int nworlds = min(WPW, count - g0);
  const bool valid = slot < nworlds;
  const size_t wg = (size_t)w0 + (nworlds > 0 ? g0 : 0);
  R* scr0 = reinterpret_cast<R*>(nb2_smem) + body_table_words<K>(M.nb) + (size_t)(threadIdx.x >> 5) * words * ST;
  R* scr = scr0 + slot;
  R* sv = saved ? saved + wg + (valid ? slot : 0) : nullptr;
  const double* wi = PW ? winertia + wg + (valid ? slot : 0) : nullptr;
  constexpr unsigned sync_mask = (K > 1) ? NB2_FWD_SYNC_MASK : NB2_FWD_SYNC_MASK_1LANE;
  const float* st_src = state + wg * 2 * M.ndof;
  const float* act_src = action + wg * M.na;
  unsigned long long* bar = nullptr;
  if (nworlds > 0) {
    const size_t sb = (size_t)nworlds * 2 * M.ndof * sizeof(float), ab = (size_t)nworlds * M.na * sizeof(float);
    if (bulk_ok(st_src, sb) && bulk_ok(act_src, ab)) {
      unsigned char* stg = nb2_smem + (((size_t)body_table_words<K>(M.nb) + (size_t)(blockDim.x >> 5) * words * ST) * sizeof(R) + 15 & ~(size_t)15) +
                           (size_t)(threadIdx.x >> 5) * staging_bytes<K>(2 * M.ndof + M.na);
      bar = reinterpret_cast<unsigned long long*>(stg + staging_bytes<K>(2 * M.ndof + M.na) - 16);
      if (li == 0) {
        mbar_init(bar);
        mbar_expect_tx(bar, (unsigned)(sb + ab));
        bulk_g2s(stg, st_src, (unsigned)sb, bar);
        bulk_g2s(stg + sb, act_src, (unsigned)ab, bar);
      }
      st_src = reinterpret_cast<const float*>(stg);
      act_src = reinterpret_cast<const float*>(stg + sb);
    }
  }
  const R* bt = stage_body_table<R, K>(M, reinterpret_cast<R*>(nb2_smem));
  if (bar) {
    __syncwarp();
    mbar_wait(bar, 0);
  }
  NB2_CLK(0, 1);
#pragma unroll 1
  for (int sg = 0; sg < NB2_FWD_STAGES; sg++) {
    if (sg == 0) {
      if (nworlds > 0) nb2::fwd_load<R, ST>(M, scr0, st_src, act_src, nworlds, li, 32,
                                            state_copy ? state_copy + wg * 2 * M.ndof : nullptr, action_copy ? action_copy + wg * M.na : nullptr);
    }
    else if (sg == NB2_FWD_STAGES - 1) { if (nworlds > 0) nb2::fwd_store<R, ST>(M, scr0, next + wg * 2 * M.ndof, nworlds, li, 32); }
    else if (valid) nb2::world_forward_stage<R, ST>(M, scr, sv, (size_t)B, saved != nullptr, lane, sg, bt, nullptr, wi, (size_t)B);
    if ((sync_mask >> sg) & 1u) __syncwarp();
    NB2_CLK(0, 2 + sg);
  }
}

template <class R, int K, bool PW>
__global__ void __launch_bounds__(128)
k_step_bwd(const __grid_constant__ Nb2ModelDev<R> M, int B, int w0, int count, const float* __restrict__ state,
           const float* __restrict__ action, const R* __restrict__ saved, const float* __restrict__ gnext,
           float* __restrict__ gstate, float* __restrict__ gaction, float* __restrict__ ginertia, int words,
           int stage_saved, int accumulate_state, unsigned in_stage_off, const double* __restrict__ winertia, double* __restrict__ ginertia_acc) {
  extern __shared__ __align__(16) unsigned char nb2_smem[];
  NB2_CLK(1, 0);
  constexpr int WPW = CoopShape<K>::WPW, ST = CoopShape<K>::ST;
  const int li = threadIdx.x & 31, slot = li / K, lane = li % K;
  const int g0 = (blockIdx.x * (blockDim.x >> 5) + (threadIdx.x >> 5)) * WPW;
  const int nworlds = min(WPW, count - g0);
  const bool valid = slot < nworlds;
  const size_t wg = (size_t)w0 + (nworlds > 0 ? g0 : 0);
  const size_t w = wg + (valid ? slot : 0);
  R* scr0 = reinterpret_cast<R*>(nb2_smem) + body_table_words<K>(M.nb) + (size_t)(threadIdx.x >> 5) * words * ST;
  R* scr = scr0 + slot;
  const float* g_src = gnext + wg * 2 * M.ndof;
  const float* st_src = state + wg * 2 * M.ndof;
  const float* act_src = action + wg * M.na;
  unsigned long long* bar = nullptr;
  if (nworlds > 0 && in_stage_off) {
    const size_t sb = (size_t)nworlds * 2 * M.ndof * sizeof(float), ab = (size_t)nworlds * M.na * sizeof(float);
    if (bulk_ok(g_src, sb) && bulk_ok(st_src, sb) && bulk_ok(act_src, ab)) {
      unsigned char* stg = nb2_smem + in_stage_off + (size_t)(threadIdx.x >> 5) * staging_bytes<K>(4 * M.ndof + M.na);
      bar = reinterpret_cast<unsigned long long*>(stg + staging_bytes<K>(4 * M.ndof + M.na) - 16);
      if (li == 0) {
        mbar_init(bar);
        mbar_expect_tx(bar, (unsigned)(2 * sb + ab));
        bulk_g2s(stg, g_src, (unsigned)sb, bar);
        bulk_g2s(stg + sb, st_src, (unsigned)sb, bar);
        bulk_g2s(stg + 2 * sb, act_src, (unsigned)ab, bar);
      }
      g_src = reinterpret_cast<const float*>(stg);
      st_src = reinterpret_cast<const float*>(stg + sb);
      act_src = reinterpret_cast<const float*>(stg + 2 * sb);
    }
  }
  const R* svp = saved + wg + (valid ? slot : 0);
  size_t svB = (size_t)B;
  if (stage_saved && nworlds == WPW) {
    const int sw = nb2_saved_words(M.nb, M.ndof, M.nfree);
    R* svs = reinterpret_cast<R*>(nb2_smem) + ((body_table_words<K>(M.nb) + (size_t)(blockDim.x >> 5) * words * ST + 3) & ~(size_t)3)
             + (size_t)(threadIdx.x >> 5) * sw * WPW;
    constexpr int CH = (WPW * (int)sizeof(R)) / 16;
    const unsigned dst0 = (unsigned)__cvta_generic_to_shared(svs);
    const char* src0 = reinterpret_cast<const char*>(saved + wg);
    for (int idx = li; idx < sw * CH; idx += 32) {
      const int k = idx / CH, c = idx - k * CH;
      asm volatile("cp.async.cg.shared.global [%0], [%1], 16;" ::"r"(dst0 + (unsigned)(k * WPW * (int)sizeof(R) + c * 16)),
                   "l"(src0 + (size_t)k * B * sizeof(R) + c * 16));
    }
    asm volatile("cp.async.commit_group;");
    svp = svs + slot;
    svB = WPW;
  }
  constexpr unsigned sync_mask = (K > 1) ? NB2_BWD_SYNC_MASK : NB2_BWD_SYNC_MASK_1LANE;
  const R* bt = stage_body_table<R, K>(M, reinterpret_cast<R*>(nb2_smem));
  if (bar) {
    __syncwarp();
    mbar_wait(bar, 0);
  }
  NB2_CLK(1, 1);
#pragma unroll 1
  for (int sg = 0; sg < NB2_BWD_STAGES; sg++) {
    if (sg == 0) { if (nworlds > 0) nb2::bwd_load<R, ST, false>(M, scr0, st_src, act_src, g_src, nworlds, li, 32); }
    else if (sg == NB2_BWD_STAGES - 1) {
      if (nworlds > 0) nb2::bwd_store<R, ST, false>(M, scr0, gstate + wg * 2 * M.ndof, gaction + wg * M.na, false, nworlds, li, 32, accumulate_state != 0);
    } else if (valid) nb2::world_backward_stage<R, ST>(M, scr, svp, svB, lane, sg, ginertia ? ginertia + w : nullptr, bt, (size_t)B, nullptr,
                                                       (PW && winertia) ? winertia + w : nullptr, (size_t)B, (PW && ginertia_acc) ? ginertia_acc + w : nullptr);
    if (sg == 0 && stage_saved) asm volatile("cp.async.wait_group 0;" ::: "memory");
    if (((sync_mask >> sg) & 1u) || (sg == 0 && stage_saved)) __syncwarp();
    NB2_CLK(1, 2 + sg);
  }
}

template <class R, int K>
__global__ void __launch_bounds__(128)
k_id_fwd(const __grid_constant__ Nb2ModelDev<R> M, int B, const R* __restrict__ state, const R* __restrict__ next_vel, R* __restrict__ tau,
         R* __restrict__ saved, int words, const double* __restrict__ winertia) {
  extern __shared__ __align__(16) unsigned char nb2_smem[];
  constexpr int WPW = CoopShape<K>::WPW, ST = CoopShape<K>::ST;
  const int li = threadIdx.x & 31, slot = li / K, lane = li % K;
  const int g0 = (blockIdx.x * (blockDim.x >> 5) + (threadIdx.x >> 5)) * WPW;
  const int nworlds = min(WPW, B - g0);
  const bool valid = slot < nworlds;
  const size_t wg = nworlds > 0 ? g0 : 0, w = wg + (valid ? slot : 0);
  const R* bt = stage_body_table<R, K>(M, reinterpret_cast<R*>(nb2_smem));
  R* scr0 = reinterpret_cast<R*>(nb2_smem) + body_table_words<K>(M.nb) + (size_t)(threadIdx.x >> 5) * words * ST;
  R* scr = scr0 + slot;
  R* sv = saved ? saved + w : nullptr;
  const double* wi = winertia ? winertia + w : nullptr;
  constexpr unsigned sync_mask = (K > 1) ? NB2_ID_FWD_SYNC_MASK : NB2_ID_FWD_SYNC_MASK_1LANE;
#pragma unroll 1
  for (int sg = 0; sg < NB2_ID_FWD_STAGES; sg++) {
    if (sg == 0) { if (nworlds > 0) nb2::id_load<R, ST>(M, scr0, state + wg * 2 * M.ndof, next_vel + wg * M.ndof, nworlds, li, 32); }
    else if (sg == NB2_ID_FWD_STAGES - 1) { if (nworlds > 0) nb2::id_store<R, ST>(M, scr0, tau + wg * M.ndof, nworlds, li, 32); }
    else if (valid) nb2::id_forward_stage<R, ST>(M, scr, sv, (size_t)B, saved != nullptr, lane, sg, bt, wi, (size_t)B);
    if ((sync_mask >> sg) & 1u) __syncwarp();
  }
}

template <class R, int K>
__global__ void __launch_bounds__(128)
k_id_bwd(const __grid_constant__ Nb2ModelDev<R> M, int B, const R* __restrict__ state, const R* __restrict__ saved, const R* __restrict__ gtau,
         R* __restrict__ gstate, R* __restrict__ gnext, double* __restrict__ ginertia, int words, const double* __restrict__ winertia) {
  extern __shared__ __align__(16) unsigned char nb2_smem[];
  constexpr int WPW = CoopShape<K>::WPW, ST = CoopShape<K>::ST;
  const int li = threadIdx.x & 31, slot = li / K, lane = li % K;
  const int g0 = (blockIdx.x * (blockDim.x >> 5) + (threadIdx.x >> 5)) * WPW;
  const int nworlds = min(WPW, B - g0);
  const bool valid = slot < nworlds;
  const size_t wg = nworlds > 0 ? g0 : 0, w = wg + (valid ? slot : 0);
  const R* bt = stage_body_table<R, K>(M, reinterpret_cast<R*>(nb2_smem));
  R* scr0 = reinterpret_cast<R*>(nb2_smem) + body_table_words<K>(M.nb) + (size_t)(threadIdx.x >> 5) * words * ST;
  R* scr = scr0 + slot;
  const double* wi = winertia ? winertia + w : nullptr;
  double* gI = ginertia ? ginertia + w : nullptr;
  constexpr unsigned sync_mask = (K > 1) ? NB2_ID_BWD_SYNC_MASK : NB2_ID_BWD_SYNC_MASK_1LANE;
#pragma unroll 1
  for (int sg = 0; sg < NB2_ID_BWD_STAGES; sg++) {
    if (sg == 0) { if (nworlds > 0) nb2::id_bwd_load<R, ST>(M, scr0, state + wg * 2 * M.ndof, gtau + wg * M.ndof, nworlds, li, 32); }
    else if (sg == NB2_ID_BWD_STAGES - 1) {
      if (nworlds > 0) nb2::id_bwd_store<R, ST>(M, scr0, gstate + wg * 2 * M.ndof, gnext + wg * M.ndof, nworlds, li, 32);
    } else if (valid) nb2::id_backward_stage<R, ST>(M, scr, saved + w, (size_t)B, lane, sg, bt, wi, (size_t)B, gI, (size_t)B);
    if ((sync_mask >> sg) & 1u) __syncwarp();
  }
}

template <class R>
__global__ void __launch_bounds__(128)
k_cid_fwd(const __grid_constant__ Nb2ModelDev<R> M, const __grid_constant__ nb2::CidChain c, int B, const R* __restrict__ state,
          R* __restrict__ tau, R* __restrict__ wrench) {
  const int w = blockIdx.x * blockDim.x + threadIdx.x;
  if (w >= B) return;
  nb2::cid_forward<R>(M, c, state + (size_t)w * 2 * M.ndof, tau + (size_t)w * M.ndof, wrench + (size_t)w * 6);
}
template <class R>
__global__ void __launch_bounds__(128)
k_cid_bwd(const __grid_constant__ Nb2ModelDev<R> M, const __grid_constant__ nb2::CidChain c, int B, const R* __restrict__ state,
          const R* __restrict__ wrench, const R* __restrict__ gtau, const R* __restrict__ gwrench, R* __restrict__ seed, R* __restrict__ gstate) {
  const int w = blockIdx.x * blockDim.x + threadIdx.x;
  if (w >= B) return;
  const size_t n = M.ndof;
  nb2::cid_vjp<R>(M, c, state + w * 2 * n, wrench + (size_t)w * 6, gtau + w * n, gwrench + (size_t)w * 6, seed ? seed + w * n : nullptr,
                  seed ? nullptr : gstate + w * 2 * n);
}

template <class R>
__global__ void __launch_bounds__(128)
k_mcid_fwd(const __grid_constant__ Nb2ModelDev<R> M, const __grid_constant__ nb2::McidBodies<R> b, int B, const R* __restrict__ state,
           const R* __restrict__ guess, R* __restrict__ tau, R* __restrict__ wrench) {
  const int w = blockIdx.x * blockDim.x + threadIdx.x;
  if (w >= B) return;
  const size_t kw = (size_t)w * 6 * b.k;
  nb2::mcid_forward<R>(M, b, state + (size_t)w * 2 * M.ndof, guess ? guess + kw : nullptr, tau + (size_t)w * M.ndof, wrench + kw);
}
template <class R>
__global__ void __launch_bounds__(128)
k_mcid_bwd(const __grid_constant__ Nb2ModelDev<R> M, const __grid_constant__ nb2::McidBodies<R> b, int B, const R* __restrict__ state,
           const R* __restrict__ wrench, const R* __restrict__ guess, const R* __restrict__ gtau, const R* __restrict__ gwrench,
           R* __restrict__ seed, R* __restrict__ gguess, R* __restrict__ gstate) {
  const int w = blockIdx.x * blockDim.x + threadIdx.x;
  if (w >= B) return;
  const size_t n = M.ndof, kw = (size_t)w * 6 * b.k;
  nb2::mcid_vjp<R>(M, b, state + w * 2 * n, wrench + kw, guess ? guess + kw : nullptr, gtau + w * n, gwrench + kw, seed ? seed + w * n : nullptr,
                   seed && gguess ? gguess + kw : nullptr, seed ? nullptr : gstate + w * 2 * n);
}

template <class R>
__device__ __forceinline__ void mm_store_block(R* __restrict__ dst, const R* src, int words, int lane) {
  if (((reinterpret_cast<size_t>(dst) | (size_t)words * sizeof(R)) & 15) == 0) {
    const int nv = (int)((size_t)words * sizeof(R) / 16);
    for (int k = lane; k < nv; k += 32) reinterpret_cast<uint4*>(dst)[k] = reinterpret_cast<const uint4*>(src)[k];
  } else {
    for (int k = lane; k < words; k += 32) dst[k] = src[k];
  }
}
template <class R>
__global__ void __launch_bounds__(32)
k_mm_fwd(const __grid_constant__ Nb2ModelDev<R> M, int B, const R* __restrict__ pos, const double* __restrict__ winertia, R* __restrict__ out) {
  extern __shared__ __align__(16) unsigned char nb2_smem[];
  R* ws = reinterpret_cast<R*>(nb2_smem);
  const int lane = threadIdx.x;
  const size_t w = blockIdx.x, n = M.ndof;
  nb2::crba_init<R>(M, pos + w * n, winertia ? winertia + w : nullptr, (size_t)B, ws, lane, 32);
  __syncwarp();
  nb2::crba_composite<R>(M, ws, lane);
  __syncwarp();
  nb2::crba_columns<R>(M, ws, lane, 32);
  __syncwarp();
  mm_store_block<R>(out + w * n * n, ws + nb2::mm_layout(M.nb, M.ndof).oMat, M.ndof * M.ndof, lane);
}
template <class R>
__global__ void __launch_bounds__(32)
k_minv_fwd(const __grid_constant__ Nb2ModelDev<R> M, int B, const R* __restrict__ pos, const double* __restrict__ winertia, R* __restrict__ out) {
  extern __shared__ __align__(16) unsigned char nb2_smem[];
  R* ws = reinterpret_cast<R*>(nb2_smem);
// ... 399 lines not shown
      if (gv) fv = nb2::mk3<double>(gv[k], gv[k + 1], gv[k + 2]);
    }
    ik_fk_vjp(M, E.body, q, np + nb2::cross(We.p, fp), fp, nv + nb2::cross(We.p, fv), fv, g);
  }
}

__global__ void __launch_bounds__(64)
k_forward_dynamics(const __grid_constant__ Nb2ModelDev<double> M, int B, int words, const double* __restrict__ pos, const double* __restrict__ vel,
                   const double* __restrict__ force, double* __restrict__ accel, double* __restrict__ scratch) {
  const int w = blockIdx.x * blockDim.x + threadIdx.x;
  if (w >= B) return;
  double* scr = scratch + (size_t)w * words;
  const nb2::FwdLayout L = nb2::fwd_layout(M.nb, M.ndof, M.nslots, M.nfree);
  const int n = M.ndof;
  for (int d = 0; d < n; d++) { scr[L.oQ + d] = pos[(size_t)w * n + d]; scr[L.oV + d] = vel[(size_t)w * n + d]; }
  for (int a = 0; a < M.na; a++) scr[L.oAct + a] = force[(size_t)w * n + M.action_map[a]];
  for (int sg = 1; sg < NB2_FWD_STAGES - 1; sg++)
    for (int lane = 0; lane < M.lanes; lane++) nb2::world_forward_stage<double, 1>(M, scr, nullptr, 1, false, lane, sg);
  for (int d = 0; d < n; d++) accel[(size_t)w * n + d] = (scr[L.oV + d] - vel[(size_t)w * n + d]) / M.dt;
}

__global__ void __launch_bounds__(32)
k_lcp_batch(nb2::cw::Dims d, int B, int mcap, double cfm, int mode, int early_termination, const int* __restrict__ ms, const double* __restrict__ A,
            const double* __restrict__ b, const double* __restrict__ lo, const double* __restrict__ hi, const int* __restrict__ findex,
            const double* __restrict__ x0, double* __restrict__ x, int* __restrict__ labels, int* __restrict__ status) {
  extern __shared__ __align__(16) unsigned char nb2_smem[];
  const int w = blockIdx.x, lane = threadIdx.x & 31;
  if (w >= B) return;
  nb2::cw::Ws* wsm = warp_workspace(nb2_smem, d, lane);
  const nb2::cw::Ws ws = *wsm;
  const int m = ms[w], ld = m | 1;
  const size_t ov = (size_t)w * mcap;
  for (int e = lane; e < m * m; e += 32) { const int r = e / m, c = e - r * m; ws.A[(size_t)r * ld + c] = A[((size_t)w * mcap + r) * mcap + c]; }
  for (int i = lane; i < m; i += 32) { ws.b[i] = b[ov + i]; ws.lo[i] = lo[ov + i]; ws.hi[i] = hi[ov + i]; ws.findex[i] = findex[ov + i]; }
  __syncwarp();
  int st;
  if (mode == 0) {
    nb2::cw::DzWork W;
    for (int e = lane; e < m * ld; e += 32) ws.M1[e] = ws.A[e];
    for (int i = lane; i < m; i += 32) { ws.v1[i] = ws.b[i]; ws.v2[i] = ws.lo[i]; ws.v3[i] = ws.hi[i]; ws.i1[i] = ws.findex[i]; }
    __syncwarp();
    W.A = ws.M1; W.ld = ld; W.x = ws.x; W.b = ws.v1; W.w = ws.v5; W.lo = ws.v2; W.hi = ws.v3; W.L = ws.M2; W.d = ws.v6; W.delta_x = ws.v7; W.delta_w = ws.v8;
    W.Dell = ws.v9; W.ell = ws.v10; W.tmp = ws.v11; W.findex = ws.i1; W.p = ws.clampIdx; W.C = ws.ubIdx; W.state = ws.i4;
    st = nb2::cw::dantzig_solve(W, m, early_termination != 0);
  } else {
    st = nb2::cw::lcp_chain(m, ws, *wsm, cfm, x0 ? x0 + ov : nullptr);
  }
  __syncwarp();
  for (int i = lane; i < m; i += 32) { x[ov + i] = ws.x[i]; if (labels) labels[ov + i] = (mode == 1) ? ws.mapping[i] : 0; }
  if (lane == 0) status[w] = st;
}

constexpr int kMaxSmem = 227 * 1024;

}

template <class F> static int with_lanes(int lanes, F&& f) {
  switch (lanes) {
    case 1: return f(std::integral_constant<int, 1>());
    case 2: return f(std::integral_constant<int, 2>());
    case 4: return f(std::integral_constant<int, 4>());
    case 8: return f(std::integral_constant<int, 8>());
  }
  g_err = "bad lane count"; return NB2_ERR_INVALID;
}
template <class F> static int with_precision(int precision, F&& f) { return precision == NB2_FP64 ? f(double()) : f(float()); }
template <auto Kern> static int allow_max_smem() {
  static std::atomic<bool> done[64];
  int dev = 0; NB2_CUDA(cudaGetDevice(&dev));
  if (!done[dev & 63].load(std::memory_order_acquire)) {
    NB2_CUDA(cudaFuncSetAttribute(Kern, cudaFuncAttributeMaxDynamicSharedMemorySize, kMaxSmem));
    done[dev & 63].store(true, std::memory_order_release);
  }
  return NB2_OK;
}

struct LaunchShape { int warps_per_block = 0; int resident_warps = 0; };
struct nb2_variant {
  Nb2ModelDev<float> mf;
  Nb2ModelDev<double> md;
  int fwd_words, bwd_words, id_bwd_words;
  int depth;
  LaunchShape shape[4][2];
};
enum { LF_STEP_FWD = 0, LF_STEP_BWD = 1, LF_ID_FWD = 2, LF_ID_BWD = 3 };

struct nb2_model {
  Nb2ModelDev<float> mf;
  Nb2ModelDev<double> md;
  Nb2ContactDev contact;
  bool has_contacts = false;
  bool contact_restitution = false;
  int contact_mc = 0;
  int contact_variant = 0;
  int saved_words;
  int sm_count;
  std::vector<nb2_variant> variants;
  int forced_lanes = 0;
  float *d_state = nullptr, *d_action = nullptr, *d_next = nullptr, *d_gnext = nullptr,
        *d_gstate = nullptr, *d_gaction = nullptr;
  void* d_saved = nullptr;
  int host_cap = 0;
  int host_B = 0;
  void* hc_ws = nullptr; double *hc_x = nullptr, *hc_rec = nullptr; int32_t *hc_m = nullptr, *hc_labels = nullptr, *hc_status = nullptr, *hc_nc = nullptr, *hc_sticky = nullptr;
  int hc_cap = 0;
  cudaStream_t host_streams[4] = {nullptr, nullptr, nullptr, nullptr};
  std::mutex mu;
};

template <class R> static const Nb2ModelDev<R>& model_of(const nb2_variant& v);
template <> const Nb2ModelDev<float>& model_of<float>(const nb2_variant& v) { return v.mf; }
template <> const Nb2ModelDev<double>& model_of<double>(const nb2_variant& v) { return v.md; }

static void init_variant(nb2_variant& v) {
  v.fwd_words = nb2::fwd_layout(v.mf.nb, v.mf.ndof, v.mf.nslots, v.mf.nfree).total;
  v.bwd_words = nb2::bwd_layout(v.mf.nb, v.mf.ndof, v.mf.nslots, v.mf.nfree).total;
  v.id_bwd_words = nb2::id_bwd_words(v.mf.nb, v.mf.ndof, v.mf.nslots, v.mf.nfree);
  int trunk = 0, longest = 0;
  for (int r = 0; r < v.mf.trunk_n; r++) trunk += v.mf.trunk_hi[r] - v.mf.trunk_lo[r];
  for (int l = 0; l < v.mf.lanes; l++) {
    int len = 0;
    for (int r = 0; r < v.mf.limb_n[l]; r++) len += v.mf.limb_hi[l][r] - v.mf.limb_lo[l][r];
    if (len > longest) longest = len;
  }
  v.depth = trunk + longest;
}

template <class Kern>
static LaunchShape occupancy_shape(Kern kern, size_t bytes_per_warp, size_t bytes_per_block) {
  LaunchShape best;
  for (int w = 1; w <= 4; w *= 2) {
    const size_t smem = bytes_per_warp * w + bytes_per_block;
    if (smem > (size_t)kMaxSmem) break;
    int blocks = 0;
    if (cudaOccupancyMaxActiveBlocksPerMultiprocessor(&blocks, kern, w * 32, smem) != cudaSuccess) { cudaGetLastError(); continue; }
    if (blocks * w > best.resident_warps) { best.resident_warps = blocks * w; best.warps_per_block = w; }
  }
  return best;
}

static int block_warps(int total_warps, int sm_count, const LaunchShape& sh, size_t per_warp) {
  if ((long long)total_warps > (long long)sm_count * sh.resident_warps) return sh.warps_per_block;
  int w = 1;
  while (w < 4 && total_warps > sm_count * w && (size_t)(2 * w) * per_warp <= (size_t)kMaxSmem) w *= 2;
  return w;
}

template <class R, int K>
static int prepare_k(nb2_variant& v, int dir) {
  constexpr int ST = CoopShape<K>::ST;
  LaunchShape& sh = v.shape[dir][sizeof(R) == 8];
  const size_t scratch_and_staging =
      dir == LF_ID_FWD ? (size_t)v.fwd_words * ST * sizeof(R) : dir == LF_ID_BWD ? (size_t)v.id_bwd_words * ST * sizeof(R) :
      (size_t)(dir ? v.bwd_words : v.fwd_words) * ST * sizeof(R) +
          (dir ? staging_bytes<K>(4 * v.mf.ndof + v.mf.na) : staging_bytes<K>(2 * v.mf.ndof + v.mf.na));
  const size_t per_block = (size_t)body_table_words<K>(v.mf.nb) * sizeof(R) + 16;
  if (scratch_and_staging + per_block > (size_t)kMaxSmem) {
    g_err = "model needs " + std::to_string(scratch_and_staging) + " B of shared memory per warp (> 227 KB)"; return NB2_ERR_UNSUPPORTED;
  }
  int rc;
  if (dir == 0) {
    if ((rc = allow_max_smem<k_step_fwd<R, K, false>>()) || (rc = allow_max_smem<k_step_fwd<R, K, true>>())) return rc;
    if (!sh.warps_per_block) sh = occupancy_shape(k_step_fwd<R, K, false>, scratch_and_staging, per_block);
  } else if (dir == LF_STEP_BWD) {
    if ((rc = allow_max_smem<k_step_bwd<R, K, false>>()) || (rc = allow_max_smem<k_step_bwd<R, K, true>>())) return rc;
    if (!sh.warps_per_block) sh = occupancy_shape(k_step_bwd<R, K, false>, scratch_and_staging, per_block);
  } else if (dir == LF_ID_FWD) {
    if ((rc = allow_max_smem<k_id_fwd<R, K>>())) return rc;
    if (!sh.warps_per_block) sh = occupancy_shape(k_id_fwd<R, K>, scratch_and_staging, per_block);
  } else {
    if ((rc = allow_max_smem<k_id_bwd<R, K>>())) return rc;
    if (!sh.warps_per_block) sh = occupancy_shape(k_id_bwd<R, K>, scratch_and_staging, per_block);
  }
  if (!sh.warps_per_block) { g_err = "no launch shape fits this model"; return NB2_ERR_UNSUPPORTED; }
  return NB2_OK;
}
template <class R>
static int prepare_variant(nb2_variant& v, int dir) {
  return with_lanes(v.mf.lanes, [&](auto k) { return prepare_k<R, decltype(k)::value>(v, dir); });
}

template <class R>
static int pick_variant(nb2_model* m, int B, int dir, nb2_variant** out) {
  nb2_variant* best = nullptr;
  double best_cost = 0;
  for (auto& v : m->variants) {
    if (m->forced_lanes && v.mf.lanes != m->forced_lanes) continue;
    int rc = prepare_variant<R>(v, dir);
    if (rc) { if (m->variants.size() == 1 || m->forced_lanes) return rc; continue; }
    const LaunchShape& sh = v.shape[dir][sizeof(R) == 8];
    const double warps = ((double)B * v.mf.lanes + 31) / 32;
    double waves = warps / ((double)m->sm_count * sh.resident_warps);
    if (waves < 1) waves = 1;
    const double cost = (v.depth + 3) * waves;
    if (!best || cost < best_cost - 1e-9) { best = &v; best_cost = cost; }
  }
  if (!best) { g_err = "no usable schedule"; return NB2_ERR_UNSUPPORTED; }
  *out = best;
  return NB2_OK;
}

template <class R, int K>
static int launch_fwd_k(const nb2_variant& v, int sm_count, int Btot, int w0, int B, const float* state, const float* action,
                        float* next, R* saved, cudaStream_t st, float* state_copy, float* action_copy, const double* wi) {
  constexpr int WPW = CoopShape<K>::WPW, ST = CoopShape<K>::ST;
  const LaunchShape& sh = v.shape[0][sizeof(R) == 8];
  const size_t per_warp = (size_t)v.fwd_words * ST * sizeof(R) + staging_bytes<K>(2 * v.mf.ndof + v.mf.na);
  const int total_warps = (B + WPW - 1) / WPW;
  const int warps = block_warps(total_warps, sm_count, sh, per_warp);
  const int blocks = (total_warps + warps - 1) / warps;
  const size_t smem = per_warp * warps + (size_t)body_table_words<K>(v.mf.nb) * sizeof(R) + 16;
  if (wi) k_step_fwd<R, K, true><<<blocks, warps * 32, smem, st>>>(model_of<R>(v), Btot, w0, B, state, action, next, saved, v.fwd_words, state_copy, action_copy, wi);
  else k_step_fwd<R, K, false><<<blocks, warps * 32, smem, st>>>(model_of<R>(v), Btot, w0, B, state, action, next, saved, v.fwd_words, state_copy, action_copy, nullptr);
  g_launches++;
  NB2_CUDA(cudaGetLastError());
  return NB2_OK;
}
template <class R>
static int launch_fwd(nb2_model* m, int B, const float* state, const float* action, float* next, R* saved, cudaStream_t st,
                      int Btot = -1, int w0 = 0, float* state_copy = nullptr, float* action_copy = nullptr, const double* wi = nullptr) {
  if (Btot < 0) Btot = B;
  nb2_variant* pv = nullptr;
  int rc = pick_variant<R>(m, B, 0, &pv);
  if (rc) return rc;
  return with_lanes(pv->mf.lanes, [&](auto k) {
    return launch_fwd_k<R, decltype(k)::value>(*pv, m->sm_count, Btot, w0, B, state, action, next, saved, st, state_copy, action_copy, wi);
  });
}
static bool no_stage_saved() {
  static const bool off = [] { const char* e = getenv("NB2_NO_STAGE_SAVED"); return e && atoi(e); }();
  return off;
}
template <class R, int K>
static int launch_bwd_k(const nb2_variant& v, int sm_count, int Btot, int w0, int B, const float* state, const float* action,
                        const R* saved, const float* gnext, float* gstate, float* gaction, float* ginertia, cudaStream_t st, int accumulate,
                        const double* wi, double* gIa) {
  constexpr int WPW = CoopShape<K>::WPW, ST = CoopShape<K>::ST;
  const LaunchShape& sh = v.shape[1][sizeof(R) == 8];
  const size_t scratch_per_warp = (size_t)v.bwd_words * ST * sizeof(R);
  const int total_warps = (B + WPW - 1) / WPW;
  const int warps = block_warps(total_warps, sm_count, sh, scratch_per_warp);
  const int blocks = (total_warps + warps - 1) / warps;
  const size_t tab = (size_t)body_table_words<K>(v.mf.nb) * sizeof(R);
  const size_t stage_per_warp = (size_t)nb2_saved_words(v.mf.nb, v.mf.ndof, v.mf.nfree) * WPW * sizeof(R);
  const bool aligned = (((size_t)Btot * sizeof(R)) % 16 == 0) && (((size_t)w0 * sizeof(R)) % 16 == 0) && ((reinterpret_cast<size_t>(saved) & 15) == 0) &&
                       ((WPW * sizeof(R)) % 16 == 0);
  const size_t in_per_warp = staging_bytes<K>(4 * v.mf.ndof + v.mf.na);
  const size_t smem_staged = (scratch_per_warp + stage_per_warp) * warps + tab + 16;
  const int blocks_per_sm = (blocks + sm_count - 1) / sm_count;
  const bool stage = aligned && (smem_staged + in_per_warp * warps) * blocks_per_sm + 1024 * blocks_per_sm <= (size_t)kMaxSmem && !no_stage_saved();
  const size_t base = ((stage ? smem_staged : scratch_per_warp * warps + tab) + 15) & ~(size_t)15;
  const bool in_stage = base + in_per_warp * warps <= (size_t)kMaxSmem;
  const size_t smem = in_stage ? base + in_per_warp * warps : base;
  if (wi || gIa) k_step_bwd<R, K, true><<<blocks, warps * 32, smem, st>>>(model_of<R>(v), Btot, w0, B, state, action, saved, gnext, gstate, gaction, ginertia,
                                                                   v.bwd_words, stage ? 1 : 0, accumulate, in_stage ? (unsigned)base : 0u, wi, gIa);
  else k_step_bwd<R, K, false><<<blocks, warps * 32, smem, st>>>(model_of<R>(v), Btot, w0, B, state, action, saved, gnext, gstate, gaction, ginertia,
                                                                 v.bwd_words, stage ? 1 : 0, accumulate, in_stage ? (unsigned)base : 0u, nullptr, nullptr);
  g_launches++;
  NB2_CUDA(cudaGetLastError());
  return NB2_OK;
}
template <class R>
static int launch_bwd(nb2_model* m, int B, const float* state, const float* action,
                      const R* saved, const float* gnext, float* gstate, float* gaction, float* ginertia, cudaStream_t st,
                      int Btot = -1, int w0 = 0, int accumulate = 0, const double* wi = nullptr, double* gIa = nullptr) {
  if (Btot < 0) Btot = B;
  nb2_variant* pv = nullptr;
  int rc = pick_variant<R>(m, B, 1, &pv);
  if (rc) return rc;
  return with_lanes(pv->mf.lanes, [&](auto k) {
    return launch_bwd_k<R, decltype(k)::value>(*pv, m->sm_count, Btot, w0, B, state, action, saved, gnext, gstate, gaction, ginertia, st, accumulate, wi, gIa);
  });
}

template <class R, int K>
static int launch_id_k(const nb2_variant& v, int sm_count, int B, int dir, const R* state, const R* next_vel, R* tau, R* saved, const R* gtau,
                       R* gstate, R* gnext, double* gI, const double* wi, cudaStream_t st) {
  constexpr int WPW = CoopShape<K>::WPW, ST = CoopShape<K>::ST;
  const int words = dir == LF_ID_FWD ? v.fwd_words : v.id_bwd_words;
  const size_t per_warp = (size_t)words * ST * sizeof(R);
  const int total_warps = (B + WPW - 1) / WPW;
  const int warps = block_warps(total_warps, sm_count, v.shape[dir][sizeof(R) == 8], per_warp);
  const int blocks = (total_warps + warps - 1) / warps;
  const size_t smem = per_warp * warps + (size_t)body_table_words<K>(v.mf.nb) * sizeof(R);
  if (dir == LF_ID_FWD) k_id_fwd<R, K><<<blocks, warps * 32, smem, st>>>(model_of<R>(v), B, state, next_vel, tau, saved, words, wi);
  else k_id_bwd<R, K><<<blocks, warps * 32, smem, st>>>(model_of<R>(v), B, state, saved, gtau, gstate, gnext, gI, words, wi);
  g_launches++;
  NB2_CUDA(cudaGetLastError());
  return NB2_OK;
}
template <class R>
static int launch_id(nb2_model* m, int B, int dir, const R* state, const R* next_vel, R* tau, R* saved, const R* gtau, R* gstate, R* gnext,
                     double* gI, const double* wi, cudaStream_t st) {
  nb2_variant* pv = nullptr;
  int rc = pick_variant<R>(m, B, dir, &pv);
  if (rc) return rc;
  return with_lanes(pv->mf.lanes, [&](auto k) {
    return launch_id_k<R, decltype(k)::value>(*pv, m->sm_count, B, dir, state, next_vel, tau, saved, gtau, gstate, gnext, gI, wi, st);
  });
}

static int cid_chain_of(const nb2_model* m, int body, nb2::CidChain* c, const char* who) {
  if (nb2::cid_chain(m->mf, body, c) < 0) {
    g_err = std::string(who) + ": contact body " + std::to_string(body) + " is not a canonical body of the model under a free root";
    return NB2_ERR_INVALID;
  }
  return NB2_OK;
}
template <class R>
static int launch_cid(const nb2_model* m, const nb2::CidChain& c, int B, bool fwd, const R* state, R* tau, const R* wrench_in, R* wrench_out,
                      const R* gtau, const R* gwrench, R* seed, R* gstate, cudaStream_t st) {
  const int threads = 128, blocks = (B + threads - 1) / threads;
  if (fwd) k_cid_fwd<R><<<blocks, threads, 0, st>>>(model_of<R>(m->variants[0]), c, B, state, tau, wrench_out);
  else k_cid_bwd<R><<<blocks, threads, 0, st>>>(model_of<R>(m->variants[0]), c, B, state, wrench_in, gtau, gwrench, seed, gstate);
  g_launches++;
  NB2_CUDA(cudaGetLastError());
  return NB2_OK;
}

template <class R>
static int mcid_bodies_of(const nb2_model* m, int k, const int32_t* body, const double* point, nb2::McidBodies<R>* b, const char* who) {
  if (k < 1 || k > NB2_MAX_CONTACT_BODIES) {
    g_err = std::string(who) + ": " + std::to_string(k) + " contact bodies, expected 1.." + std::to_string(NB2_MAX_CONTACT_BODIES);
    return NB2_ERR_INVALID;
  }
  if (nb2::mcid_bodies(m->mf, k, body, point, b) < 0) {
    g_err = std::string(who) + ": the contact bodies are not canonical bodies of the model under one free root";
    return NB2_ERR_INVALID;
  }
  return NB2_OK;
}
template <class R>
static int launch_mcid(const nb2_model* m, const nb2::McidBodies<R>& b, int B, bool fwd, const R* state, const R* guess, R* tau,
                       const R* wrench_in, R* wrench_out, const R* gtau, const R* gwrench, R* seed, R* gguess, R* gstate, cudaStream_t st) {
  const int threads = 128, blocks = (B + threads - 1) / threads;
  if (fwd) k_mcid_fwd<R><<<blocks, threads, 0, st>>>(model_of<R>(m->variants[0]), b, B, state, guess, tau, wrench_out);
  else k_mcid_bwd<R><<<blocks, threads, 0, st>>>(model_of<R>(m->variants[0]), b, B, state, wrench_in, guess, gtau, gwrench, seed, gguess, gstate);
  g_launches++;
  NB2_CUDA(cudaGetLastError());
  return NB2_OK;
}

static int host_chunks(int B) {
  static const int forced = [] { const char* e = getenv("NB2_HOST_CHUNKS"); return e ? atoi(e) : 1; }();
  return (forced >= 1 && forced <= 4 && forced <= B) ? forced : 1;
}
static bool zero_copy_enabled() {
  static const bool on = [] { const char* e = getenv("NB2_NO_ZEROCOPY"); return !(e && atoi(e)); }();
  return on;
}
template <class T> static T* mapped_alias(const T* host) {
  cudaPointerAttributes a;
  if (cudaPointerGetAttributes(&a, host) != cudaSuccess) { cudaGetLastError(); return nullptr; }
  if (a.type != cudaMemoryTypeHost || !a.devicePointer) return nullptr;
  return (T*)a.devicePointer;
}

static nb2::cw::Dims cdims(const nb2_model* m, int MC, int bwd, int mode = NB2_WS_FULL) {
  return nb2::cw::make_dims(m->md.nb, m->md.ndof, m->md.nfree, MC, 3 * MC, m->contact.ncb, m->contact.max_chain_dofs, bwd, mode);
}
static int wpb_cap(int which) {
  static int caps[4] = {0, 0, 0, 0};
  static const bool init = [] { const char* e = getenv("NB2_WPB"); if (e) sscanf(e, "%d,%d,%d,%d", &caps[0], &caps[1], &caps[2], &caps[3]); return true; }();
  (void)init;
  return caps[which];
}
static int pick_wpb(int B, int sm_count, size_t smem_per_warp, int max_warps, int which = -1) {
  int w = (int)((size_t)kMaxSmem / (smem_per_warp ? smem_per_warp : 1));
  if (which >= 0 && wpb_cap(which) > 0 && wpb_cap(which) < max_warps) max_warps = wpb_cap(which);
  if (w > max_warps) w = max_warps;
  const int spread = (B + sm_count - 1) / sm_count;
  if (w > spread) w = spread;
  return w < 1 ? 1 : w;
}
static bool contact_fused() {
  static const bool on = [] { const char* e = getenv("NB2_CONTACT_FUSED"); return e && atoi(e); }();
  return on;
}
static int pool_slots(int B) { int s = B / 16; if (s < 32) s = 32; if (s > 4096) s = 4096; return s; }
static size_t pool_stride(const nb2_model* m) { return (nb2::cw::ws_doubles(cdims(m, NB2_MAX_CONTACTS, 1)) + 1) & ~(size_t)1; }
static CStepArgs cstep_args(const nb2_model* m, const nb2_variant& v, int B, void* workspace, int bwd) {
// ... 21 lines not shown
  P.todo = (int*)(P.exch + (size_t)B * P.exch_stride);
  return P;
}
template <auto Kern> static int cstep_smem_attr(size_t smem) {
  if (int rc = allow_max_smem<Kern>()) return rc;
  if (smem > (size_t)kMaxSmem) { g_err = "the fused contact kernel needs " + std::to_string(smem) + " B of shared memory per world (> 227 KB)"; return NB2_ERR_UNSUPPORTED; }
  return NB2_OK;
}

extern "C" {

const char* nb2_last_error(void) { return g_err.c_str(); }
const char* nb2_version(void) { return "nb2 0.2 (sm_90a; cooperative-lane ABA + adjoint, warp-per-world contact / boxed-LCP stage)"; }
long long nb2_launch_count(void) { return g_launches.load(); }

int nb2_model_create(const nb2_model_desc* desc, nb2_model** out) {
  if (!desc || !out) { g_err = "null argument"; return NB2_ERR_INVALID; }
  nb2_model* m = new nb2_model();
  std::string err;
  if (!nb2_fill_model(*desc, m->mf, err) || !nb2_fill_model(*desc, m->md, err)) {
    g_err = err; delete m;
    return (desc->nb > NB2_MAX_BODIES || desc->ndof > NB2_MAX_DOFS) ? NB2_ERR_UNSUPPORTED : NB2_ERR_INVALID;
  }
  if ((desc->nshapes > 0 && desc->npairs > 0) || desc->nlimits > 0) {
    if (!nb2_fill_contact(*desc, m->contact, err)) { g_err = err; delete m; return NB2_ERR_UNSUPPORTED; }
    m->has_contacts = true;
    for (int p = 0; p < desc->npairs; p++)
      if (m->contact.shape_rest[desc->pair_a[p]] * m->contact.shape_rest[desc->pair_b[p]] > 1e-3) m->contact_restitution = true;
    int mc = 0;
    for (int p = 0; p < desc->npairs; p++) mc += (desc->shape_type[desc->pair_a[p]] == 0 && desc->shape_type[desc->pair_b[p]] == 0) ? 4 : 1;
    mc += desc->nlimits;
    if (const char* e = getenv("NB2_CONTACT_MC")) mc = atoi(e);
    m->contact_mc = mc < 2 ? 2 : (mc > NB2_MAX_CONTACTS ? NB2_MAX_CONTACTS : mc);
  }
  {
    nb2_variant v;
    v.mf = m->mf; v.md = m->md;
    init_variant(v);
    m->variants.push_back(v);
  }
  m->saved_words = nb2_saved_words(m->mf.nb, m->mf.ndof, m->mf.nfree);
  int dev = 0;
  cudaDeviceProp prop;
  if (cudaGetDevice(&dev) != cudaSuccess || cudaGetDeviceProperties(&prop, dev) != cudaSuccess) {
    g_err = "no CUDA device available: nimblephysics_b200 has no CPU fallback";
    delete m;
    return NB2_ERR_CUDA;
  }
  m->sm_count = prop.multiProcessorCount;
  *out = m;
  return NB2_OK;
}

int nb2_model_add_schedule(nb2_model* m, const nb2_model_desc* desc) {
  if (!m || !desc) { g_err = "null argument"; return NB2_ERR_INVALID; }
  nb2_variant v;
  std::string err;
  if (!nb2_fill_model(*desc, v.mf, err) || !nb2_fill_model(*desc, v.md, err)) { g_err = err; return NB2_ERR_INVALID; }
  bool same = v.md.nb == m->md.nb && v.md.ndof == m->md.ndof && v.md.na == m->md.na && v.md.nfree == m->md.nfree && v.md.dt == m->md.dt;
  for (int i = 0; same && i < m->md.nb; i++) {
    same = v.md.parent[i] == m->md.parent[i] && v.md.jtype[i] == m->md.jtype[i] && v.md.dof_off[i] == m->md.dof_off[i];
    for (int k = 0; same && k < 12; k++) same = v.md.Xtree[i][k] == m->md.Xtree[i][k];
    for (int k = 0; same && k < 10; k++) same = v.md.inertia[i][k] == m->md.inertia[i][k];
  }
  if (!same) { g_err = "nb2_model_add_schedule: the descriptor describes a different model"; return NB2_ERR_INVALID; }
  for (const auto& o : m->variants) if (o.mf.lanes == v.mf.lanes) { g_err = "nb2_model_add_schedule: a schedule with this lane count exists"; return NB2_ERR_INVALID; }
  init_variant(v);
  std::lock_guard<std::mutex> lk(m->mu);
  m->variants.push_back(v);
  for (size_t k = 0; k < m->variants.size(); k++) if (m->variants[k].depth < m->variants[m->contact_variant].depth) m->contact_variant = (int)k;
  return NB2_OK;
}
int nb2_model_set_inertia(nb2_model* m, const double* inertia) {
  if (!m || !inertia) { g_err = "null argument"; return NB2_ERR_INVALID; }
  for (int i = 0; i < m->md.nb; i++)
    if (!(inertia[10 * i] > 0)) { g_err = "nb2_model_set_inertia: body " + std::to_string(i) + " has non-positive mass"; return NB2_ERR_INVALID; }
  std::lock_guard<std::mutex> lk(m->mu);
  auto put = [&](Nb2ModelDev<float>& mf, Nb2ModelDev<double>& md) {
    for (int i = 0; i < md.nb; i++)
      for (int k = 0; k < 10; k++) { md.inertia[i][k] = inertia[10 * i + k]; mf.inertia[i][k] = (float)inertia[10 * i + k]; }
  };
  put(m->mf, m->md);
  for (auto& v : m->variants) put(v.mf, v.md);
  return NB2_OK;
}
int nb2_model_set_lanes(nb2_model* m, int lanes) {
  if (!m) { g_err = "null argument"; return NB2_ERR_INVALID; }
  if (lanes != 0) {
    bool found = false;
    for (const auto& o : m->variants) found = found || o.mf.lanes == lanes;
    if (!found) { g_err = "nb2_model_set_lanes: no schedule with " + std::to_string(lanes) + " lanes was added"; return NB2_ERR_INVALID; }
  }
  m->forced_lanes = lanes;
  return NB2_OK;
}
int nb2_model_lanes_for(nb2_model* m, int B, int backward, int precision) {
  if (!m || B <= 0) return -1;
  nb2_variant* pv = nullptr;
  const int rc = with_precision(precision, [&](auto r) { return pick_variant<decltype(r)>(m, B, backward ? 1 : 0, &pv); });
  return rc ? -1 : pv->mf.lanes;
}

void nb2_model_destroy(nb2_model* m) {
  if (!m) return;
  cudaFree(m->d_state); cudaFree(m->d_action); cudaFree(m->d_next); cudaFree(m->d_saved);
  cudaFree(m->d_gnext); cudaFree(m->d_gstate); cudaFree(m->d_gaction);
  cudaFree(m->hc_ws); cudaFree(m->hc_x); cudaFree(m->hc_rec); cudaFree(m->hc_m); cudaFree(m->hc_labels); cudaFree(m->hc_status); cudaFree(m->hc_nc); cudaFree(m->hc_sticky);
  for (auto& hs : m->host_streams) if (hs) cudaStreamDestroy(hs);
  delete m;
}
int nb2_model_has_contacts(const nb2_model* m) { return (m && m->has_contacts) ? 1 : 0; }
size_t nb2_contact_workspace_bytes(const nb2_model* m, int B) {
  if (!m || !m->has_contacts || B <= 0) return 0;
  return 64 + ((size_t)pool_slots(B) * pool_stride(m) + (size_t)B * nb2::cw::xlayout(m->md.ndof).total) * sizeof(double) + (size_t)B * sizeof(int);
}
int nb2_step_forward_contact(const nb2_model* cm, int B, const float* state, const float* action, float* next_state,
                             void* saved_fp64, void* workspace, double* x_lcp, int32_t* m_lcp, int32_t* labels,
                             int32_t* status, int32_t* ncontacts, float* cinfo, double* contact_record, int32_t* status_accum, void* stream) {
  return nb2_step_forward_contact_pw(cm, B, state, action, nullptr, next_state, saved_fp64, workspace, x_lcp, m_lcp, labels, status, ncontacts, cinfo,
                                     contact_record, status_accum, stream);
}
int nb2_step_forward_contact_pw(const nb2_model* cm, int B, const float* state, const float* action, const double* world_inertia, float* next_state,
                                void* saved_fp64, void* workspace, double* x_lcp, int32_t* m_lcp, int32_t* labels,
                                int32_t* status, int32_t* ncontacts, float* cinfo, double* contact_record, int32_t* status_accum, void* stream) {
  nb2_model* m = const_cast<nb2_model*>(cm);
  if (m && B == 0) return NB2_OK;
  if (!m || B < 0 || !state || !action || !next_state || !workspace || !x_lcp || !m_lcp || !labels || !status || !ncontacts) {
    g_err = "nb2_step_forward_contact: bad argument"; return NB2_ERR_INVALID;
  }
  if (!m->has_contacts) { g_err = "nb2_step_forward_contact: the model has no collision pairs"; return NB2_ERR_INVALID; }
  if (contact_record && !saved_fp64) { g_err = "nb2_step_forward_contact: a contact record without the saved stream cannot be back-propagated"; return NB2_ERR_INVALID; }
  if (B == 0) return NB2_OK;
  cudaStream_t st = (cudaStream_t)stream;
  const nb2_variant& v = m->variants[m->contact_variant];
  const CStepArgs P = cstep_args(m, v, B, workspace, 0);
  const size_t smem = ((((size_t)P.fwd_words + 1) & ~(size_t)1) + NB2_WS_DESC_DOUBLES + P.ws_small_doubles) * sizeof(double);
  int rc = cstep_smem_attr<k_cstep_fwd>(smem);
  if (rc) return rc;
  NB2_CUDA(cudaMemsetAsync(workspace, 0, 64, st));
  if (contact_fused() || !saved_fp64) {
    k_cstep_fwd<<<B, 32, smem, st>>>(v.md, m->contact, P, state, action, next_state, (double*)saved_fp64, x_lcp, m_lcp, labels, status, ncontacts, cinfo,
                                     contact_record, status_accum, world_inertia);
    g_launches++;
    NB2_CUDA(cudaGetLastError());
    return NB2_OK;
  }
  const size_t smem_s = (NB2_WS_DESC_DOUBLES + nb2::cw::ws_doubles(P.ds_solve)) * sizeof(double);
  const size_t smem_a = (NB2_WS_DESC_DOUBLES + nb2::cw::ws_doubles(P.ds_apply)) * sizeof(double);
  if ((rc = cstep_smem_attr<k_cbuild>(smem)) || (rc = cstep_smem_attr<k_csolve<0>>(smem_s)) || (rc = cstep_smem_attr<k_csolve<1>>(smem_s)) ||
      (rc = cstep_smem_attr<k_capply>(smem_a)))
    return rc;
  const int wpb_b = pick_wpb(B, m->sm_count, smem, NB2_CBUILD_MAXW, 0), wpb_s = pick_wpb(B, m->sm_count, smem_s, NB2_CSOLVE_MAXW, 1),
            wpb_a = pick_wpb(B, m->sm_count, smem_a, NB2_CAPPLY_MAXW, 2);
  k_cbuild<<<(B + wpb_b - 1) / wpb_b, 32 * wpb_b, smem * wpb_b, st>>>(v.md, m->contact, P, state, action, next_state, (double*)saved_fp64, m_lcp, status, ncontacts, cinfo,
                                                                      contact_record, smem, world_inertia);
  k_csolve<0><<<(B + wpb_s - 1) / wpb_s, 32 * wpb_s, smem_s * wpb_s, st>>>(m->contact, P, m->md.ndof, x_lcp, m_lcp, labels, status, contact_record, status_accum, smem_s,
                                                                         P.todo, P.todo_count);
  k_csolve<1><<<(B + wpb_s - 1) / wpb_s, 32 * wpb_s, smem_s * wpb_s, st>>>(m->contact, P, m->md.ndof, x_lcp, m_lcp, labels, status, contact_record, status_accum, smem_s,
                                                                         P.todo, P.todo_count);
  k_capply<<<(B + wpb_a - 1) / wpb_a, 32 * wpb_a, smem_a * wpb_a, st>>>(v.md, m->contact, P, state, next_state, (const double*)saved_fp64, x_lcp, labels, contact_record,
                                                                        smem_a);
  g_launches += 4;
  NB2_CUDA(cudaGetLastError());
  return NB2_OK;
}
size_t nb2_contact_record_bytes(const nb2_model* m, int B) {
  if (!m || !m->has_contacts || B <= 0) return 0;
  return nb2::cw::record_doubles(m->mf.ndof) * sizeof(double) * (size_t)B;
}
}
static int cbwd_launch(nb2_model* m, int B, const float* state, const float* action, const void* saved_fp64, const double* contact_record, void* workspace,
                       const float* grad_next_state, float* grad_state, float* grad_action, float* grad_inertia, int32_t* status_accum, cudaStream_t st,
                       int accumulate, const double* wi = nullptr, double* gIa = nullptr) {
  const nb2_variant& v = m->variants[m->contact_variant];
  const CStepArgs P = cstep_args(m, v, B, workspace, 1);
  const size_t smem_base = ((((size_t)P.bwd_words + 1) & ~(size_t)1) + NB2_WS_DESC_DOUBLES + ((P.ws_small_doubles + 1) & ~(size_t)1)) * sizeof(double);
  const size_t smem_staged = smem_base + ((((size_t)P.saved_words + 1) & ~(size_t)1) + 2) * sizeof(double);
  const int stage = pick_wpb(B, m->sm_count, smem_staged, NB2_CBWD_MAXW, 3) == pick_wpb(B, m->sm_count, smem_base, NB2_CBWD_MAXW, 3);
  const size_t smem = stage ? smem_staged : smem_base;
  const bool bounce = m->contact_restitution;
  int rc = bounce ? cstep_smem_attr<k_cstep_bwd<true>>(smem) : cstep_smem_attr<k_cstep_bwd<false>>(smem);
  if (rc) return rc;
  NB2_CUDA(cudaMemsetAsync(workspace, 0, 64, st));
  const int wpb = pick_wpb(B, m->sm_count, smem, NB2_CBWD_MAXW, 3);
  if (bounce)
    k_cstep_bwd<true><<<(B + wpb - 1) / wpb, 32 * wpb, smem * wpb, st>>>(v.md, m->contact, P, state, action, (const double*)saved_fp64, contact_record, grad_next_state,
                                                                         grad_state, grad_action, grad_inertia, status_accum, smem, stage, accumulate, wi, gIa);
  else
    k_cstep_bwd<false><<<(B + wpb - 1) / wpb, 32 * wpb, smem * wpb, st>>>(v.md, m->contact, P, state, action, (const double*)saved_fp64, contact_record, grad_next_state,
                                                                          grad_state, grad_action, grad_inertia, status_accum, smem, stage, accumulate, wi, gIa);
  g_launches++;
// ... 676 lines not shown
```

Measured before the change: 64.81 million.

## Pack per-body and per-DOF model data into aligned shared-memory table records

```diff
diff --git a/nimblephysics_b200/csrc/nb2_dyn.cuh b/nimblephysics_b200/csrc/nb2_dyn.cuh
--- a/nimblephysics_b200/csrc/nb2_dyn.cuh
+++ b/nimblephysics_b200/csrc/nb2_dyn.cuh
@@ -1,5 +1,6 @@
 #pragma once
 #include <stddef.h>
+#include <string.h>
 
 #include "nb2_math.cuh"
 #include "nb2_model.h"
@@ -68,11 +69,61 @@
   return v;
 }
 
-#define NB2_BT_WORDS 22
+template <class R> struct BodyTab {
+  static constexpr int QUAD = 24 * (int)sizeof(R);
+  static constexpr int REC = QUAD + 16;
+  static constexpr int CLIP = (3 * (int)sizeof(R) + 4 + 15) & ~15;
+  static constexpr int DOF = CLIP + 32;
+  NB2_HD static constexpr int bytes(int nb, int ndof) { return nb * REC + ndof * DOF; }
+};
+template <class R> struct alignas(16) Q16 { R v[16 / sizeof(R)]; };
+template <class R, int N> NB2_HD void ld_q16(const R* t, R* out) {
+  constexpr int E = 16 / (int)sizeof(R);
+  static_assert(N % E == 0, "whole 16-byte units only");
+#pragma unroll
+  for (int k = 0; k < N / E; k++) {
+    const Q16<R> q = reinterpret_cast<const Q16<R>*>(t)[k];
+#pragma unroll
+    for (int e = 0; e < E; e++) out[k * E + e] = q.v[e];
+  }
+}
+struct alignas(16) I4 { int x, y, z, w; };
+NB2_HD int lo16(int w) { return (int)(int16_t)(w & 0xffff); }
+NB2_HD int hi16(int w) { return w >> 16; }
+struct BodyRec { int jt, p, o, fl, slot_self, slot_parent, slot_count, fi; };
+template <class R> NB2_HD BodyRec body_rec(const Nb2ModelDev<R>& M, const R* bt, int i) {
+  BodyRec b;
+  if (bt) {
+    const I4 q = *reinterpret_cast<const I4*>(reinterpret_cast<const unsigned char*>(bt) + BodyTab<R>::REC * i + BodyTab<R>::QUAD);
+    b.p = lo16(q.x); b.jt = hi16(q.x); b.o = lo16(q.y); b.fl = hi16(q.y);
+    b.slot_self = lo16(q.z); b.slot_parent = hi16(q.z); b.slot_count = lo16(q.w); b.fi = hi16(q.w);
+    return b;
+  }
+  b.jt = M.jtype[i]; b.p = M.parent[i]; b.o = M.dof_off[i]; b.fl = M.flags[i];
+  b.slot_self = M.slot_self[i]; b.slot_parent = M.slot_parent[i]; b.slot_count = M.slot_count[i]; b.fi = M.free_idx[i];
+  return b;
+}
+template <class R> struct DofRec { R spring, damping, rest; int act; };
+template <class R> NB2_HD const unsigned char* dof_tab(const Nb2ModelDev<R>& M, const R* bt, int d) {
+  return reinterpret_cast<const unsigned char*>(bt) + BodyTab<R>::REC * M.nb + BodyTab<R>::DOF * d;
+}
+template <class R> NB2_HD DofRec<R> dof_rec(const Nb2ModelDev<R>& M, const R* bt, int d) {
+  DofRec<R> r;
+  if (bt) {
+    R w[BodyTab<R>::CLIP / sizeof(R)];
+    ld_q16<R, BodyTab<R>::CLIP / sizeof(R)>(reinterpret_cast<const R*>(dof_tab(M, bt, d)), w);
+    r.spring = w[0]; r.damping = w[1]; r.rest = w[2];
+    int a; memcpy(&a, &w[3], sizeof(int)); r.act = a;
+    return r;
+  }
+  r.spring = M.spring[d]; r.damping = M.damping[d]; r.rest = M.rest[d]; r.act = M.act_of_dof[d];
+  return r;
+}
 template <class R> NB2_HD Xf<R> xtree(const Nb2ModelDev<R>& M, const R* bt, int i) {
   Xf<R> T;
   if (bt) {
-    const R* t = bt + NB2_BT_WORDS * i;
+    R t[12];
+    ld_q16<R, 12>(reinterpret_cast<const R*>(reinterpret_cast<const unsigned char*>(bt) + BodyTab<R>::REC * i), t);
     T.R_.m00 = t[0]; T.R_.m01 = t[1]; T.R_.m02 = t[2]; T.R_.m10 = t[3]; T.R_.m11 = t[4]; T.R_.m12 = t[5];
     T.R_.m20 = t[6]; T.R_.m21 = t[7]; T.R_.m22 = t[8];
     T.p = mk3<R>(t[9], t[10], t[11]);
@@ -109,7 +160,8 @@
     return;
   }
   if (bt) {
-    const R* t = bt + NB2_BT_WORDS * i + 12;
+    R t[12];
+    ld_q16<R, 12>(reinterpret_cast<const R*>(reinterpret_cast<const unsigned char*>(bt) + BodyTab<R>::REC * i) + 12, t);
     *m = t[0]; *h = mk3<R>(t[1], t[2], t[3]);
     Ib->xx = t[4]; Ib->yy = t[5]; Ib->zz = t[6]; Ib->xy = t[7]; Ib->xz = t[8]; Ib->yz = t[9];
     return;
@@ -130,11 +182,14 @@
   p[0] = T.R_.m00; p[ST] = T.R_.m01; p[2 * ST] = T.R_.m02; p[3 * ST] = T.R_.m10; p[4 * ST] = T.R_.m11; p[5 * ST] = T.R_.m12;
   p[6 * ST] = T.R_.m20; p[7 * ST] = T.R_.m21; p[8 * ST] = T.R_.m22; p[9 * ST] = T.p.x; p[10 * ST] = T.p.y; p[11 * ST] = T.p.z;
 }
+template <class R, int ST> NB2_HD Xf<R> body_xf_fwd(const Nb2ModelDev<R>& M, const R* bt, const BodyRec& br, int i, const R* scr, const FwdLayout& L) {
+  const int jt = br.jt;
+  if (jt == NB2_JT_REV) { const R* b = scr + (size_t)(L.oBody + NB2_FWD_BODY_WORDS * i + 6) * ST; return xf_rev(M, bt, i, b[0], b[ST]); }
+  if (jt == NB2_JT_PRIS) return xf_pris(M, bt, i, scr[(size_t)(L.oQ + br.o) * ST]);
+  return ldXf<R, ST>(scr + (size_t)(L.oFree + 18 * br.fi) * ST);
+}
 template <class R, int ST> NB2_HD Xf<R> body_xf_fwd(const Nb2ModelDev<R>& M, const R* bt, int i, const R* scr, const FwdLayout& L) {
-  const int jt = M.jtype[i];
-  if (jt == NB2_JT_REV) { const R* b = scr + (size_t)(L.oBody + NB2_FWD_BODY_WORDS * i + 6) * ST; return xf_rev(M, bt, i, b[0], b[ST]); }
-  if (jt == NB2_JT_PRIS) return xf_pris(M, bt, i, scr[(size_t)(L.oQ + M.dof_off[i]) * ST]);
-  return ldXf<R, ST>(scr + (size_t)(L.oFree + 18 * M.free_idx[i]) * ST);
+  return body_xf_fwd<R, ST>(M, bt, body_rec(M, bt, i), i, scr, L);
 }
 template <class R> NB2_HD V6<R> S_times(int jt, R x) {
   V6<R> s = zero6<R>();
@@ -143,8 +198,8 @@
 }
 template <class R> NB2_HD R S_dot(int jt, const V6<R>& f) { return (jt == NB2_JT_REV) ? f.a.z : f.l.z; }
 
-template <class R, int ST> NB2_HD R tau_of(const Nb2ModelDev<R>& M, const R* scr, int oAct, int d) {
-  const int a = M.act_of_dof[d];
+template <class R, int ST> NB2_HD R tau_of(const DofRec<R>& dr, const R* scr, int oAct) {
+  const int a = dr.act;
   return (a >= 0) ? scr[(size_t)(oAct + a) * ST] : R(0);
 }
 
@@ -155,7 +210,8 @@
   const R dt = M.dt;
   (void)nb; (void)n; (void)dt;
   for (int i = lo; i < hi; i++) {
-    const int jt = M.jtype[i], p = M.parent[i], o = M.dof_off[i];
+    const BodyRec br = body_rec(M, bt, i);
+    const int jt = br.jt, p = br.p, o = br.o;
     R* bs = scr + (size_t)(L.oBody + NB2_FWD_BODY_WORDS * i) * ST;
     V6<R> Vp = (p >= 0) ? ld6<R, ST>(scr + (size_t)(L.oBody + NB2_FWD_BODY_WORDS * p) * ST) : zero6<R>();
     V6<R> V;
@@ -174,7 +230,7 @@
       M3<R> Rq = expmap(mk3<R>(q[0], q[ST], q[2 * ST]));
       T.R_ = mul(X.R_, Rq);
       T.p = mul(X.R_, mk3<R>(q[3 * ST], q[4 * ST], q[5 * ST])) + X.p;
-      stXf<R, ST>(scr + (size_t)(L.oFree + 18 * M.free_idx[i]) * ST, T);
+      stXf<R, ST>(scr + (size_t)(L.oFree + 18 * br.fi) * ST, T);
       V = AdInvT(T, Vp) + ld6<R, ST>(v);
     }
     st6<R, ST>(bs, V);
@@ -193,7 +249,8 @@
   V6<R> hp = zero6<R>();
   bool hvalid = false;
   for (int i = hi - 1; i >= lo; i--) {
-    const int jt = M.jtype[i], p = M.parent[i], o = M.dof_off[i], fl = M.flags[i];
+    const BodyRec br = body_rec(M, bt, i);
+    const int jt = br.jt, p = br.p, o = br.o, fl = br.fl;
     R* bs = scr + (size_t)(L.oBody + NB2_FWD_BODY_WORDS * i) * ST;
     R m; V3<R> h; S3<R> Ib; inertia_of(M, bt, wi, wiB, i, &m, &h, &Ib);
     const V6<R> V = ld6<R, ST>(bs);
@@ -201,8 +258,8 @@
     V6<R> pA = crf(V, mulG(m, h, Ib, V));
     if (hvalid) { IA = IA + hI; pA = pA + hp; }
     if (fl & NB2_F_HAS_SLOT) {
-      for (int k = 0; k < M.slot_count[i]; k++) {
-        const R* sl = scr + (size_t)(L.oSlot + 27 * (M.slot_self[i] + k)) * ST;
+      for (int k = 0; k < br.slot_count; k++) {
+        const R* sl = scr + (size_t)(L.oSlot + 27 * (br.slot_self + k)) * ST;
         IA = IA + ldSI<R, ST>(sl);
         pA = pA + ld6<R, ST>(sl + 21 * ST);
       }
@@ -221,7 +278,8 @@
       }
       const R psi = nb2_rcp(D);
       const R qv = scr[(size_t)(L.oQ + o) * ST];
-      const R u = tau_of<R, ST>(M, scr, L.oAct, o) - M.spring[o] * (qv - M.rest[o] + vq * dt) - M.damping[o] * vq
+      const DofRec<R> dr = dof_rec(M, bt, o);
+      const R u = tau_of<R, ST>(dr, scr, L.oAct) - dr.spring * (qv - dr.rest + vq * dt) - dr.damping * vq
                   - (dot(U, eta) + S_dot(jt, pA));
       st6<R, ST>(bs + 8 * ST, U);
       bs[14 * ST] = psi; bs[15 * ST] = u;
@@ -240,25 +298,26 @@
     } else {
       const R* q = scr + (size_t)(L.oQ + o) * ST;
       const R* v = scr + (size_t)(L.oV + o) * ST;
-      R t[6];
-#pragma unroll
-      for (int k = 0; k < 6; k++) t[k] = tau_of<R, ST>(M, scr, L.oAct, o + k);
       const V6<R> Vj = ld6<R, ST>(v);
       const V6<R> eta = ad(V, Vj);
       const V6<R> bf = mul(IA, eta) + pA;
+      const auto uk = [&](int k, R qk, R vk, R bk) {
+        const DofRec<R> d = dof_rec(M, bt, o + k);
+        return tau_of<R, ST>(d, scr, L.oAct) - d.spring * (qk - d.rest + vk * dt) - d.damping * vk - bk;
+      };
       V6<R> u;
-      u.a.x = t[0] - M.spring[o] * (q[0] - M.rest[o] + Vj.a.x * dt) - M.damping[o] * Vj.a.x - bf.a.x;
-      u.a.y = t[1] - M.spring[o + 1] * (q[ST] - M.rest[o + 1] + Vj.a.y * dt) - M.damping[o + 1] * Vj.a.y - bf.a.y;
-      u.a.z = t[2] - M.spring[o + 2] * (q[2 * ST] - M.rest[o + 2] + Vj.a.z * dt) - M.damping[o + 2] * Vj.a.z - bf.a.z;
-      u.l.x = t[3] - M.spring[o + 3] * (q[3 * ST] - M.rest[o + 3] + Vj.l.x * dt) - M.damping[o + 3] * Vj.l.x - bf.l.x;
-      u.l.y = t[4] - M.spring[o + 4] * (q[4 * ST] - M.rest[o + 4] + Vj.l.y * dt) - M.damping[o + 4] * Vj.l.y - bf.l.y;
-      u.l.z = t[5] - M.spring[o + 5] * (q[5 * ST] - M.rest[o + 5] + Vj.l.z * dt) - M.damping[o + 5] * Vj.l.z - bf.l.z;
+      u.a.x = uk(0, q[0], Vj.a.x, bf.a.x);
+      u.a.y = uk(1, q[ST], Vj.a.y, bf.a.y);
+      u.a.z = uk(2, q[2 * ST], Vj.a.z, bf.a.z);
+      u.l.x = uk(3, q[3 * ST], Vj.l.x, bf.l.x);
+      u.l.y = uk(4, q[4 * ST], Vj.l.y, bf.l.y);
+      u.l.z = uk(5, q[5 * ST], Vj.l.z, bf.l.z);
       const SI<R> Iinv = spd6_inverse(IA);
       const V6<R> y = mul(Iinv, u);
-      st6<R, ST>(scr + (size_t)(L.oFree + 18 * M.free_idx[i] + 12) * ST, y);
-      if (iinv_out) stSI<R, 1, false>(iinv_out + 21 * M.free_idx[i], Iinv);
+      st6<R, ST>(scr + (size_t)(L.oFree + 18 * br.fi + 12) * ST, y);
+      if (iinv_out) stSI<R, 1, false>(iinv_out + 21 * br.fi, Iinv);
       if (save) {
-        const int k0 = nb * 21 + M.free_idx[i] * 33;
+        const int k0 = nb * 21 + br.fi * 33;
         R* s = sv + (size_t)k0 * B;
         s[0] = (R)Iinv.A.xx; s[B] = (R)Iinv.A.yy; s[2 * B] = (R)Iinv.A.zz; s[3 * B] = (R)Iinv.A.xy; s[4 * B] = (R)Iinv.A.xz; s[5 * B] = (R)Iinv.A.yz;
         s[6 * B] = (R)Iinv.B.m00; s[7 * B] = (R)Iinv.B.m01; s[8 * B] = (R)Iinv.B.m02; s[9 * B] = (R)Iinv.B.m10; s[10 * B] = (R)Iinv.B.m11; s[11 * B] = (R)Iinv.B.m12;
@@ -269,12 +328,12 @@
     }
     hvalid = false;
     if (p >= 0) {
-      const Xf<R> T = body_xf_fwd<R, ST>(M, bt, i, scr, L);
+      const Xf<R> T = body_xf_fwd<R, ST>(M, bt, br, i, scr, L);
       const SI<R> Ic = xform_inertia(T, Pi);
       const V6<R> pc = dAdInvT(T, beta);
       if (fl & NB2_F_HANDOFF) { hI = Ic; hp = pc; hvalid = true; }
       else {
-        R* sl = scr + (size_t)(L.oSlot + 27 * M.slot_parent[i]) * ST;
+        R* sl = scr + (size_t)(L.oSlot + 27 * br.slot_parent) * ST;
         stSI<R, ST, false>(sl, Ic); st6<R, ST>(sl + 21 * ST, pc);
       }
     }
@@ -290,9 +349,10 @@
   (void)nb; (void)n; (void)dt;
   V6<R> A0; A0.a = zero3<R>(); A0.l = mk3<R>(-M.gravity[0], -M.gravity[1], -M.gravity[2]);
   for (int i = lo; i < hi; i++) {
-    const int jt = M.jtype[i], p = M.parent[i], o = M.dof_off[i];
+    const BodyRec br = body_rec(M, bt, i);
+    const int jt = br.jt, p = br.p, o = br.o;
     R* bs = scr + (size_t)(L.oBody + NB2_FWD_BODY_WORDS * i) * ST;
-    const Xf<R> T = body_xf_fwd<R, ST>(M, bt, i, scr, L);
+    const Xf<R> T = body_xf_fwd<R, ST>(M, bt, br, i, scr, L);
     const V6<R> Ap = AdInvT(T, (p >= 0) ? ld6<R, ST>(scr + (size_t)(L.oBody + NB2_FWD_BODY_WORDS * p) * ST) : A0);
     const V6<R> V = ld6<R, ST>(bs);
     V6<R> A;
@@ -315,7 +375,7 @@
       }
     } else {
       const R* q = scr + (size_t)(L.oQ + o) * ST;
-      const R* fr = scr + (size_t)(L.oFree + 18 * M.free_idx[i]) * ST;
+      const R* fr = scr + (size_t)(L.oFree + 18 * br.fi) * ST;
       const V6<R> Vj = ld6<R, ST>(scr + (size_t)(L.oV + o) * ST);
       const V6<R> y = ld6<R, ST>(fr + 12 * ST);
       const V6<R> qdd = y - Ap;
@@ -333,7 +393,7 @@
         R* s = sv + (size_t)(i * 21) * B;
         sv_st6(s, B, 0, tof(V)); sv_st6(s, B, 6, tof(A));
         for (int k = 12; k < 21; k++) s[(size_t)k * B] = R(0);
-        R* sf = sv + (size_t)(nb * 21 + M.free_idx[i] * 33 + 21) * B;
+        R* sf = sv + (size_t)(nb * 21 + br.fi * 33 + 21) * B;
         for (int k = 0; k < 12; k++) sf[(size_t)k * B] = fr[(size_t)k * ST];
         R* sq = sv + (size_t)(nb * 21 + M.nfree * 33 + o) * B;
         sq[0] = qdd.a.x; sq[B] = qdd.a.y; sq[2 * B] = qdd.a.z; sq[3 * B] = qdd.l.x; sq[4 * B] = qdd.l.y; sq[5 * B] = qdd.l.z;
@@ -487,11 +547,12 @@
   V6<R> hp = zero6<R>();
   bool hvalid = false;
   for (int i = hi - 1; i >= lo; i--) {
-    const int jt = M.jtype[i], p = M.parent[i], o = M.dof_off[i], fl = M.flags[i];
+    const BodyRec br = body_rec(M, bt, i);
+    const int jt = br.jt, p = br.p, o = br.o, fl = br.fl;
     const R* s = sv + (size_t)(i * 21) * B;
     V6<R> pI = hvalid ? hp : zero6<R>();
     if (fl & NB2_F_HAS_SLOT)
-      for (int k = 0; k < M.slot_count[i]; k++) pI = pI + ld6<R, ST>(scr + (size_t)(L.oSlot + SLOTW * (M.slot_self[i] + k)) * ST);
+      for (int k = 0; k < br.slot_count; k++) pI = pI + ld6<R, ST>(scr + (size_t)(L.oSlot + SLOTW * (br.slot_self + k)) * ST);
     V6<R> beta;
     if (jt != NB2_JT_FREE) {
       const R up = scr[(size_t)(L.oGV + o) * ST] - S_dot(jt, pI);
@@ -499,7 +560,7 @@
       if (p >= 0) beta = pI + sv_ld6<R>(s, B, 12) * ((R)s[18 * B] * up);
     } else {
       const V6<R> up = ld6<R, ST>(scr + (size_t)(L.oGV + o) * ST) - pI;
-      st6<R, ST>(scr + (size_t)(L.oFree + 6 * M.free_idx[i]) * ST, up);
+      st6<R, ST>(scr + (size_t)(L.oFree + 6 * br.fi) * ST, up);
       if (p >= 0) beta = pI + up;
     }
     hvalid = false;
@@ -507,11 +568,11 @@
       Xf<R> T;
       if (jt == NB2_JT_REV) T = xf_rev(M, bt, i, (R)s[19 * B], (R)s[20 * B]);
       else if (jt == NB2_JT_PRIS) T = xf_pris(M, bt, i, scr[(size_t)(L.oSt + o) * ST]);
-      else { R t12[12]; for (int k = 0; k < 12; k++) t12[k] = (R)sv[(size_t)(kFree + M.free_idx[i] * 33 + 21 + k) * B]; T = ldXf<R, 1>(t12); }
+      else { R t12[12]; for (int k = 0; k < 12; k++) t12[k] = (R)sv[(size_t)(kFree + br.fi * 33 + 21 + k) * B]; T = ldXf<R, 1>(t12); }
       const V6<R> pc = dAdInvT(T, beta);
       if (fl & NB2_F_HANDOFF) { hp = pc; hvalid = true; }
       else {
-        R* sl = scr + (size_t)(L.oSlot + SLOTW * M.slot_parent[i]) * ST;
+        R* sl = scr + (size_t)(L.oSlot + SLOTW * br.slot_parent) * ST;
         st6<R, ST>(sl, pc);
       }
     }
@@ -527,7 +588,8 @@
   const int kFree = nb * 21, kQdd = nb * 21 + M.nfree * 33;
   (void)n; (void)dt; (void)kFree; (void)kQdd;
   for (int i = lo; i < hi; i++) {
-    const int jt = M.jtype[i], p = M.parent[i], o = M.dof_off[i];
+    const BodyRec br = body_rec(M, bt, i);
+    const int jt = br.jt, p = br.p, o = br.o;
     const R* s = sv + (size_t)(i * 21) * B;
     R* bs = scr + (size_t)(L.oBody + 7 * i) * ST;
     V6<R> W;
@@ -538,13 +600,13 @@
       scr[(size_t)(L.oLam + o) * ST] = lam;
       if (jt == NB2_JT_REV) W.a.z += lam; else W.l.z += lam;
     } else {
-      const R* sf = sv + (size_t)(kFree + M.free_idx[i] * 33) * B;
+      const R* sf = sv + (size_t)(kFree + br.fi * 33) * B;
       R t12[12]; for (int k = 0; k < 12; k++) t12[k] = (R)sf[(size_t)(21 + k) * B];
       const Xf<R> T = ldXf<R, 1>(t12);
       const V6<R> Wp = (p >= 0) ? AdInvT(T, ld6<R, ST>(scr + (size_t)(L.oBody + 7 * p + 1) * ST)) : zero6<R>();
       R i21[21]; for (int k = 0; k < 21; k++) i21[k] = (R)sf[(size_t)k * B];
       const SI<R> Iinv = ldSI<R, 1>(i21);
-      W = mul(Iinv, ld6<R, ST>(scr + (size_t)(L.oFree + 6 * M.free_idx[i]) * ST));
+      W = mul(Iinv, ld6<R, ST>(scr + (size_t)(L.oFree + 6 * br.fi) * ST));
       st6<R, ST>(scr + (size_t)(L.oLam + o) * ST, W - Wp);
     }
     st6<R, ST>(bs + ST, W);
@@ -564,7 +626,8 @@
   V6<R> hUw = zero6<R>(), hUp = zero6<R>(), hG = zero6<R>(), hH = zero6<R>();
   bool hvalid = false;
   for (int i = hi - 1; i >= lo; i--) {
-    const int jt = M.jtype[i], p = M.parent[i], o = M.dof_off[i], fl = M.flags[i];
+    const BodyRec br = body_rec(M, bt, i);
+    const int jt = br.jt, p = br.p, o = br.o, fl = br.fl;
     const R* s = sv + (size_t)(i * 21) * B;
     R m; V3<R> h; S3<R> Ib; inertia_of(M, bt, wi, wiB, i, &m, &h, &Ib);
     const V6<R> V = sv_ld6<R>(s, B, 0);
@@ -604,8 +667,8 @@
       if (hvalid) { Uw = Uw + hUw; Up = Up + hUp; Gc = Gc + hG; Hc = Hc + hH; }
     }
     if (fl & NB2_F_HAS_SLOT) {
-      for (int k = 0; k < M.slot_count[i]; k++) {
-        const R* sl = scr + (size_t)(L.oSlot + SLOTW * (M.slot_self[i] + k)) * ST;
+      for (int k = 0; k < br.slot_count; k++) {
+        const R* sl = scr + (size_t)(L.oSlot + SLOTW * (br.slot_self + k)) * ST;
         Abar = Abar + ld6<R, ST>(sl); Vbar = Vbar + ld6<R, ST>(sl + 6 * ST); f = f + ld6<R, ST>(sl + 12 * ST);
         if (CONTACT && cd.active) { Uw = Uw + ld6<R, ST>(sl + 18 * ST); Up = Up + ld6<R, ST>(sl + 24 * ST); Gc = Gc + ld6<R, ST>(sl + 30 * ST); Hc = Hc + ld6<R, ST>(sl + 36 * ST); }
       }
@@ -622,7 +685,7 @@
       Sa = sv_ld6<R>(sv + (size_t)(kQdd + o) * B, B, 0);
       if (CONTACT && cd.active && !cd.pass2) { const auto a6 = cd.aeff + o; Sa.a = mk3<R>((R)a6[0], (R)a6[1], (R)a6[2]); Sa.l = mk3<R>((R)a6[3], (R)a6[4], (R)a6[5]); }
       Sl = ld6<R, ST>(scr + (size_t)(L.oLam + o) * ST);
-      R t12[12]; for (int k = 0; k < 12; k++) t12[k] = (R)sv[(size_t)(kFree + M.free_idx[i] * 33 + 21 + k) * B];
+      R t12[12]; for (int k = 0; k < 12; k++) t12[k] = (R)sv[(size_t)(kFree + br.fi * 33 + 21 + k) * B];
       T = ldXf<R, 1>(t12);
     }
     Vbar = Vbar + crf(Sv, Abar);
@@ -661,7 +724,7 @@
       if (CONTACT && cd.active) { cUw = dAdInvT(T, Uw); cUp = dAdInvT(T, Up); cG = dAdInvT(T, Gc); cH = dAdInvT(T, Hc); }
       if (fl & NB2_F_HANDOFF) { hA = cA; hV = cV; hf = cf; if (CONTACT && cd.active) { hUw = cUw; hUp = cUp; hG = cG; hH = cH; } hvalid = true; }
       else {
-        R* sl = scr + (size_t)(L.oSlot + SLOTW * M.slot_parent[i]) * ST;
+        R* sl = scr + (size_t)(L.oSlot + SLOTW * br.slot_parent) * ST;
         st6<R, ST>(sl, cA); st6<R, ST>(sl + 6 * ST, cV); st6<R, ST>(sl + 12 * ST, cf);
         if (CONTACT && cd.active) { st6<R, ST>(sl + 18 * ST, cUw); st6<R, ST>(sl + 24 * ST, cUp); st6<R, ST>(sl + 30 * ST, cG); st6<R, ST>(sl + 36 * ST, cH); }
       }
@@ -670,28 +733,31 @@
 }
 
 template <class R, int ST>
-NB2_HD void finish_dof(const Nb2ModelDev<R>& M, R* scr, const BwdLayout& L, int d, R gq_, R gv_, R lam) {
+NB2_HD void finish_dof(const Nb2ModelDev<R>& M, const R* bt, const DofRec<R>& dr, R* scr, const BwdLayout& L, int d, R gq_, R gv_, R lam) {
   const int n = M.ndof;
+  float c[8];
+  if (bt) ld_q16<float, 8>(reinterpret_cast<const float*>(dof_tab(M, bt, d) + BodyTab<R>::CLIP), c);
+  else { c[0] = M.pos_lo[d]; c[1] = M.pos_hi[d]; c[2] = M.vel_lo[d]; c[3] = M.vel_hi[d]; c[4] = M.force_lo[d]; c[5] = M.force_hi[d]; }
   float gq = (float)gq_, gv = (float)gv_;
   const float qd = (float)scr[(size_t)(L.oSt + d) * ST], vd = (float)scr[(size_t)(L.oSt + n + d) * ST];
-  if (qd == M.pos_lo[d] && gq > 0.f) gq = 0.f;
-  if (qd == M.pos_hi[d] && gq < 0.f) gq = 0.f;
-  if (vd == M.vel_lo[d] && gv > 0.f) gv = 0.f;
-  if (vd == M.vel_hi[d] && gv < 0.f) gv = 0.f;
+  if (qd == c[0] && gq > 0.f) gq = 0.f;
+  if (qd == c[1] && gq < 0.f) gq = 0.f;
+  if (vd == c[2] && gv > 0.f) gv = 0.f;
+  if (vd == c[3] && gv < 0.f) gv = 0.f;
   scr[(size_t)(L.oQb + d) * ST] = (R)gq;
   scr[(size_t)(L.oVb + d) * ST] = (R)gv;
-  const int a = M.act_of_dof[d];
+  const int a = dr.act;
   if (a >= 0) {
     float gt = (float)(M.dt * lam);
     const float fd = (float)scr[(size_t)(L.oAct + a) * ST];
-    if (fd == M.force_lo[d] && gt > 0.f) gt = 0.f;
-    if (fd == M.force_hi[d] && gt < 0.f) gt = 0.f;
+    if (fd == c[4] && gt > 0.f) gt = 0.f;
+    if (fd == c[5] && gt < 0.f) gt = 0.f;
     scr[(size_t)(L.oAct + a) * ST] = (R)gt;
   }
 }
 
 template <class R, int ST, bool CONTACT>
-NB2_HD void bwd_assemble(const Nb2ModelDev<R>& M, R* scr, const float* st, const BwdContactData<ST>& cd, int lo, int hi) {
+NB2_HD void bwd_assemble(const Nb2ModelDev<R>& M, R* scr, const float* st, const BwdContactData<ST>& cd, int lo, int hi, const R* bt = nullptr) {
   const int nb = M.nb, n = M.ndof;
   constexpr int SLOTW = CONTACT ? 42 : 18;
   const BwdLayout L = bwd_layout(nb, n, M.nslots, M.nfree, SLOTW);
@@ -699,14 +765,16 @@
   const int kFree = nb * 21, kQdd = nb * 21 + M.nfree * 33;
   (void)n; (void)dt; (void)kFree; (void)kQdd;
   for (int i = lo; i < hi; i++) {
-    const int jt = M.jtype[i], o = M.dof_off[i];
+    const BodyRec br = body_rec(M, bt, i);
+    const int jt = br.jt, o = br.o;
     if (jt != NB2_JT_FREE) {
+      const DofRec<R> dr = dof_rec(M, bt, o);
       const R lam = scr[(size_t)(L.oLam + o) * ST];
       const R gq = scr[(size_t)(L.oGQ + o) * ST];
       R gv = scr[(size_t)(L.oGV + o) * ST];
       if (CONTACT && cd.active) gv -= (R)cd.JcTmu[o];
-      finish_dof<R, ST>(M, scr, L, o, gq - dt * (scr[(size_t)(L.oQb + o) * ST] + M.spring[o] * lam),
-                        dt * gq + gv - dt * (scr[(size_t)(L.oVb + o) * ST] + (M.damping[o] + dt * M.spring[o]) * lam), lam);
+      finish_dof<R, ST>(M, bt, dr, scr, L, o, gq - dt * (scr[(size_t)(L.oQb + o) * ST] + dr.spring * lam),
+                        dt * gq + gv - dt * (scr[(size_t)(L.oVb + o) * ST] + (dr.damping + dt * dr.spring) * lam), lam);
     } else {
       const V3<R> phi = mk3<R>(scr[(size_t)(L.oSt + o) * ST], scr[(size_t)(L.oSt + o + 1) * ST], scr[(size_t)(L.oSt + o + 2) * ST]);
       const V3<R> w = mk3<R>(scr[(size_t)(L.oSt + n + o) * ST], scr[(size_t)(L.oSt + n + o + 1) * ST], scr[(size_t)(L.oSt + n + o + 2) * ST]);
@@ -730,8 +798,9 @@
       R gvv[6] = {gv.a.x, gv.a.y, gv.a.z, gv.l.x, gv.l.y, gv.l.z};
 #pragma unroll
       for (int k = 0; k < 6; k++) {
-        finish_dof<R, ST>(M, scr, L, o + k, gqv[k] - dt * (qbv[k] + M.spring[o + k] * lamv[k]),
-                          gvpv[k] + gvv[k] - dt * (vbv[k] + (M.damping[o + k] + dt * M.spring[o + k]) * lamv[k]), lamv[k]);
+        const DofRec<R> dr = dof_rec(M, bt, o + k);
+        finish_dof<R, ST>(M, bt, dr, scr, L, o + k, gqv[k] - dt * (qbv[k] + dr.spring * lamv[k]),
+                          gvpv[k] + gvv[k] - dt * (vbv[k] + (dr.damping + dt * dr.spring) * lamv[k]), lamv[k]);
       }
     }
   }
@@ -796,7 +865,7 @@
     if (pass == 1) bwd_B1<R, ST, CONTACT>(M, scr, st, sv, B, lo, hi, bt);
     else if (pass == 2) bwd_B2<R, ST, CONTACT>(M, scr, st, sv, B, lo, hi, bt);
     else if (pass == 3) bwd_B3<R, ST, CONTACT>(M, scr, st, sv, B, cd, lo, hi, gI, bt, gIB ? gIB : B, wi, wiB, gIa);
-    else bwd_assemble<R, ST, CONTACT>(M, scr, st, cd, lo, hi);
+    else bwd_assemble<R, ST, CONTACT>(M, scr, st, cd, lo, hi, bt);
   }
 }
 
@@ -825,9 +894,10 @@
   const int kFree = M.nb * 21, kQdd = M.nb * 21 + M.nfree * 33;
   V6<R> A0; A0.a = zero3<R>(); A0.l = mk3<R>(-M.gravity[0], -M.gravity[1], -M.gravity[2]);
   for (int i = lo; i < hi; i++) {
-    const int jt = M.jtype[i], p = M.parent[i], o = M.dof_off[i];
+    const BodyRec br = body_rec(M, bt, i);
+    const int jt = br.jt, p = br.p, o = br.o;
     R* bs = scr + (size_t)(L.oBody + NB2_FWD_BODY_WORDS * i) * ST;
-    const Xf<R> T = body_xf_fwd<R, ST>(M, bt, i, scr, L);
+    const Xf<R> T = body_xf_fwd<R, ST>(M, bt, br, i, scr, L);
     const V6<R> Ap = AdInvT(T, (p >= 0) ? ld6<R, ST>(scr + (size_t)(L.oBody + NB2_FWD_BODY_WORDS * p + 8) * ST) : A0);
     const V6<R> V = ld6<R, ST>(bs);
     V6<R> A = Ap;
@@ -843,8 +913,8 @@
       A = Ap + a + ad(V, Vj);
       if (save) {
         sv_st6(sv + (size_t)(kQdd + o) * B, B, 0, a);
-        const R* fr = scr + (size_t)(L.oFree + 18 * M.free_idx[i]) * ST;
-        R* sf = sv + (size_t)(kFree + M.free_idx[i] * 33 + 21) * B;
+        const R* fr = scr + (size_t)(L.oFree + 18 * br.fi) * ST;
+        R* sf = sv + (size_t)(kFree + br.fi * 33 + 21) * B;
         for (int k = 0; k < 12; k++) sf[(size_t)k * B] = fr[(size_t)k * ST];
       }
     }
@@ -864,26 +934,28 @@
   V6<R> hf = zero6<R>();
   bool hvalid = false;
   for (int i = hi - 1; i >= lo; i--) {
-    const int jt = M.jtype[i], p = M.parent[i], o = M.dof_off[i], fl = M.flags[i];
+    const BodyRec br = body_rec(M, bt, i);
+    const int jt = br.jt, p = br.p, o = br.o, fl = br.fl;
     const R* bs = scr + (size_t)(L.oBody + NB2_FWD_BODY_WORDS * i) * ST;
     R m; V3<R> h; S3<R> Ib; inertia_of(M, bt, wi, wiB, i, &m, &h, &Ib);
     const V6<R> V = ld6<R, ST>(bs), A = ld6<R, ST>(bs + 8 * ST);
     V6<R> f = mulG(m, h, Ib, A) + crf(V, mulG(m, h, Ib, V));
     if (hvalid) f = f + hf;
     if (fl & NB2_F_HAS_SLOT)
-      for (int k = 0; k < M.slot_count[i]; k++) f = f + ld6<R, ST>(scr + (size_t)(L.oSlot + 27 * (M.slot_self[i] + k)) * ST);
+      for (int k = 0; k < br.slot_count; k++) f = f + ld6<R, ST>(scr + (size_t)(L.oSlot + 27 * (br.slot_self + k)) * ST);
     const int nd = (jt == NB2_JT_FREE) ? 6 : 1;
     for (int k = 0; k < nd; k++) {
       const int d = o + k;
+      const DofRec<R> dr = dof_rec(M, bt, d);
       const R qd = scr[(size_t)(L.oQ + d) * ST], vd = scr[(size_t)(L.oV + d) * ST];
       const R fk = (jt == NB2_JT_FREE) ? comp6(f, k) : S_dot(jt, f);
-      scr[(size_t)(L.oAct + d) * ST] = fk + M.spring[d] * (qd - M.rest[d] + vd * dt) + M.damping[d] * vd;
+      scr[(size_t)(L.oAct + d) * ST] = fk + dr.spring * (qd - dr.rest + vd * dt) + dr.damping * vd;
     }
     hvalid = false;
     if (p >= 0) {
-      const V6<R> fc = dAdInvT(body_xf_fwd<R, ST>(M, bt, i, scr, L), f);
+      const V6<R> fc = dAdInvT(body_xf_fwd<R, ST>(M, bt, br, i, scr, L), f);
       if (fl & NB2_F_HANDOFF) { hf = fc; hvalid = true; }
-      else st6<R, ST>(scr + (size_t)(L.oSlot + 27 * M.slot_parent[i]) * ST, fc);
+      else st6<R, ST>(scr + (size_t)(L.oSlot + 27 * br.slot_parent) * ST, fc);
     }
   }
 }
@@ -918,21 +990,22 @@
 
 NB2_HD int id_bwd_words(int nb, int n, int nslots, int nfree) { return bwd_layout(nb, n, nslots, nfree).total + 6 * nslots; }
 template <class R, int ST>
-NB2_HD Xf<R> id_saved_xf(const Nb2ModelDev<R>& M, const R* bt, int i, const R* scr, const BwdLayout& L, const R* sv, size_t B) {
-  const int jt = M.jtype[i];
+NB2_HD Xf<R> id_saved_xf(const Nb2ModelDev<R>& M, const R* bt, const BodyRec& br, int i, const R* scr, const BwdLayout& L, const R* sv, size_t B) {
+  const int jt = br.jt;
   const R* s = sv + (size_t)(i * 21) * B;
   if (jt == NB2_JT_REV) return xf_rev(M, bt, i, s[19 * B], s[20 * B]);
-  if (jt == NB2_JT_PRIS) return xf_pris(M, bt, i, scr[(size_t)(L.oSt + M.dof_off[i]) * ST]);
+  if (jt == NB2_JT_PRIS) return xf_pris(M, bt, i, scr[(size_t)(L.oSt + br.o) * ST]);
   R t12[12];
-  for (int k = 0; k < 12; k++) t12[k] = sv[(size_t)(M.nb * 21 + M.free_idx[i] * 33 + 21 + k) * B];
+  for (int k = 0; k < 12; k++) t12[k] = sv[(size_t)(M.nb * 21 + br.fi * 33 + 21 + k) * B];
   return ldXf<R, 1>(t12);
 }
 template <class R, int ST>
 NB2_HD void id_bwd_field(const Nb2ModelDev<R>& M, R* scr, const R* sv, size_t B, int lo, int hi, const R* bt) {
   const BwdLayout L = bwd_layout(M.nb, M.ndof, M.nslots, M.nfree);
   for (int i = lo; i < hi; i++) {
-    const int jt = M.jtype[i], p = M.parent[i], o = M.dof_off[i];
-    V6<R> W = (p >= 0) ? AdInvT(id_saved_xf<R, ST>(M, bt, i, scr, L, sv, B), ld6<R, ST>(scr + (size_t)(L.oBody + 7 * p + 1) * ST)) : zero6<R>();
+    const BodyRec br = body_rec(M, bt, i);
+    const int jt = br.jt, p = br.p, o = br.o;
+    V6<R> W = (p >= 0) ? AdInvT(id_saved_xf<R, ST>(M, bt, br, i, scr, L, sv, B), ld6<R, ST>(scr + (size_t)(L.oBody + 7 * p + 1) * ST)) : zero6<R>();
     if (jt != NB2_JT_FREE) W = W + S_times<R>(jt, scr[(size_t)(L.oLam + o) * ST]);
     else W = W + ld6<R, ST>(scr + (size_t)(L.oLam + o) * ST);
     st6<R, ST>(scr + (size_t)(L.oBody + 7 * i + 1) * ST, W);
@@ -947,13 +1020,14 @@
   V6<R> hA = zero6<R>();
   bool hvalid = false;
   for (int i = hi - 1; i >= lo; i--) {
-    const int jt = M.jtype[i], p = M.parent[i], o = M.dof_off[i], fl = M.flags[i];
+    const BodyRec br = body_rec(M, bt, i);
+    const int jt = br.jt, p = br.p, o = br.o, fl = br.fl;
     R m; V3<R> h; S3<R> Ib; inertia_of(M, bt, wi, wiB, i, &m, &h, &Ib);
     const V6<R> W = ld6<R, ST>(scr + (size_t)(L.oBody + 7 * i + 1) * ST);
     V6<R> Ab = mulG(m, h, Ib, W);
     if (hvalid) Ab = Ab + hA;
     if (fl & NB2_F_HAS_SLOT)
-      for (int k = 0; k < M.slot_count[i]; k++) Ab = Ab + ld6<R, ST>(scr + (size_t)(oS + 6 * (M.slot_self[i] + k)) * ST);
+      for (int k = 0; k < br.slot_count; k++) Ab = Ab + ld6<R, ST>(scr + (size_t)(oS + 6 * (br.slot_self + k)) * ST);
     if (gI) {
       const R* s = sv + (size_t)(i * 21) * B;
       const V6<R> V = sv_ld6<R>(s, B, 0), A = sv_ld6<R>(s, B, 6);
@@ -968,16 +1042,17 @@
     const int nd = (jt == NB2_JT_FREE) ? 6 : 1;
     for (int k = 0; k < nd; k++) {
       const int d = o + k;
+      const DofRec<R> dr = dof_rec(M, bt, d);
       const R ml = ((jt == NB2_JT_FREE) ? comp6(Ab, k) : S_dot(jt, Ab)) * rdt, lam = scr[(size_t)(L.oLam + d) * ST];
-      scr[(size_t)(L.oQb + d) * ST] += M.spring[d] * lam;
-      scr[(size_t)(L.oVb + d) * ST] += (M.damping[d] + dt * M.spring[d]) * lam - ml;
+      scr[(size_t)(L.oQb + d) * ST] += dr.spring * lam;
+      scr[(size_t)(L.oVb + d) * ST] += (dr.damping + dt * dr.spring) * lam - ml;
       scr[(size_t)(L.oGQ + d) * ST] = ml;
     }
     hvalid = false;
     if (p >= 0) {
-      const V6<R> cA = dAdInvT(id_saved_xf<R, ST>(M, bt, i, scr, L, sv, B), Ab);
+      const V6<R> cA = dAdInvT(id_saved_xf<R, ST>(M, bt, br, i, scr, L, sv, B), Ab);
       if (fl & NB2_F_HANDOFF) { hA = cA; hvalid = true; }
-      else st6<R, ST>(scr + (size_t)(oS + 6 * M.slot_parent[i]) * ST, cA);
+      else st6<R, ST>(scr + (size_t)(oS + 6 * br.slot_parent) * ST, cA);
     }
   }
 }
diff --git a/nimblephysics_b200/csrc/nb2_kernels.cu b/nimblephysics_b200/csrc/nb2_kernels.cu
--- a/nimblephysics_b200/csrc/nb2_kernels.cu
+++ b/nimblephysics_b200/csrc/nb2_kernels.cu
@@ -3,6 +3,8 @@
 #include <stdlib.h>
 
 #include <atomic>
+#include <map>
+#include <string.h>
 #include <mutex>
 #include <string>
 #include <type_traits>
@@ -33,24 +35,8 @@
   static constexpr int ST = (K == 1) ? 32 : WPW + 1;
 };
 
-template <int K> __host__ __device__ constexpr int body_table_words(int nb) { return (K > 1) ? ((nb * NB2_BT_WORDS + 3) & ~3) : 0; }
-template <class R, int K>
-__device__ __forceinline__ const R* stage_body_table(const Nb2ModelDev<R>& M, R* tab) {
-  if constexpr (K == 1) return nullptr;
-  else {
-  using U = std::conditional_t<sizeof(R) == 4, float2, double>;
-  constexpr int XU = 12 * sizeof(R) / sizeof(U), IU = 10 * sizeof(R) / sizeof(U), BU = XU + IU;
-  static_assert(offsetof(Nb2ModelDev<R>, Xtree) % sizeof(U) == 0 && offsetof(Nb2ModelDev<R>, inertia) % sizeof(U) == 0, "unaligned body tables");
-  const U* xs = reinterpret_cast<const U*>(&M.Xtree[0][0]);
-  const U* is = reinterpret_cast<const U*>(&M.inertia[0][0]);
-  U* t = reinterpret_cast<U*>(tab);
-  for (int k = threadIdx.x; k < M.nb * BU; k += blockDim.x) {
-    const int i = k / BU, j = k - i * BU;
-    t[k] = (j < XU) ? xs[i * XU + j] : is[i * IU + j - XU];
-  }
-  __syncthreads();
-  return tab;
-  }
+template <class R, int K> __host__ __device__ constexpr int body_table_words(int nb, int ndof) {
+  return (K > 1) ? (nb2::BodyTab<R>::bytes(nb, ndof) + 16) / (int)sizeof(R) : 0;
 }
 
 __device__ __forceinline__ unsigned smem_u32(const void* p) { return (unsigned)__cvta_generic_to_shared(p); }
@@ -75,6 +61,23 @@
   __trap();
 }
 __device__ __forceinline__ bool bulk_ok(const void* p, size_t bytes) { return ((reinterpret_cast<size_t>(p) | bytes) & 15) == 0 && bytes > 0; }
+
+template <class R, int K>
+__device__ __forceinline__ const R* stage_body_table(const Nb2ModelDev<R>& M, R* tab, const void* src) {
+  if constexpr (K == 1) return nullptr;
+  else {
+    const unsigned bytes = (unsigned)nb2::BodyTab<R>::bytes(M.nb, M.ndof);
+    unsigned long long* bar = reinterpret_cast<unsigned long long*>(reinterpret_cast<unsigned char*>(tab) + bytes);
+    if (threadIdx.x == 0) {
+      mbar_init(bar);
+      mbar_expect_tx(bar, bytes);
+      bulk_g2s(tab, src, bytes, bar);
+    }
+    __syncthreads();
+    mbar_wait(bar, 0);
+    return tab;
+  }
+}
 template <int K> __host__ __device__ constexpr size_t staging_bytes(int floats_per_world) {
   return (((size_t)floats_per_world * CoopShape<K>::WPW * sizeof(float) + 15) & ~(size_t)15) + 16;
 }
@@ -97,7 +100,7 @@
 __global__ void __launch_bounds__(128)
 k_step_fwd(const __grid_constant__ Nb2ModelDev<R> M, int B, int w0, int count, const float* __restrict__ state,
            const float* __restrict__ action, float* __restrict__ next, R* __restrict__ saved, int words,
-           float* __restrict__ state_copy, float* __restrict__ action_copy, const double* __restrict__ winertia) {
+           float* __restrict__ state_copy, float* __restrict__ action_copy, const double* __restrict__ winertia, const void* __restrict__ body_tab) {
   extern __shared__ __align__(16) unsigned char nb2_smem[];
   NB2_CLK(0, 0);
   constexpr int WPW = CoopShape<K>::WPW, ST = CoopShape<K>::ST;
@@ -106,7 +109,7 @@
   const int nworlds = min(WPW, count - g0);
   const bool valid = slot < nworlds;
   const size_t wg = (size_t)w0 + (nworlds > 0 ? g0 : 0);
-  R* scr0 = reinterpret_cast<R*>(nb2_smem) + body_table_words<K>(M.nb) + (size_t)(threadIdx.x >> 5) * words * ST;
+  R* scr0 = reinterpret_cast<R*>(nb2_smem) + body_table_words<R, K>(M.nb, M.ndof) + (size_t)(threadIdx.x >> 5) * words * ST;
   R* scr = scr0 + slot;
   R* sv = saved ? saved + wg + (valid ? slot : 0) : nullptr;
   const double* wi = PW ? winertia + wg + (valid ? slot : 0) : nullptr;
@@ -117,7 +120,7 @@
   if (nworlds > 0) {
     const size_t sb = (size_t)nworlds * 2 * M.ndof * sizeof(float), ab = (size_t)nworlds * M.na * sizeof(float);
     if (bulk_ok(st_src, sb) && bulk_ok(act_src, ab)) {
-      unsigned char* stg = nb2_smem + (((size_t)body_table_words<K>(M.nb) + (size_t)(blockDim.x >> 5) * words * ST) * sizeof(R) + 15 & ~(size_t)15) +
+      unsigned char* stg = nb2_smem + (((size_t)body_table_words<R, K>(M.nb, M.ndof) + (size_t)(blockDim.x >> 5) * words * ST) * sizeof(R) + 15 & ~(size_t)15) +
                            (size_t)(threadIdx.x >> 5) * staging_bytes<K>(2 * M.ndof + M.na);
       bar = reinterpret_cast<unsigned long long*>(stg + staging_bytes<K>(2 * M.ndof + M.na) - 16);
       if (li == 0) {
@@ -130,7 +133,7 @@
       act_src = reinterpret_cast<const float*>(stg + sb);
     }
   }
-  const R* bt = stage_body_table<R, K>(M, reinterpret_cast<R*>(nb2_smem));
+  const R* bt = stage_body_table<R, K>(M, reinterpret_cast<R*>(nb2_smem), body_tab);
   if (bar) {
     __syncwarp();
     mbar_wait(bar, 0);
@@ -154,7 +157,7 @@
 k_step_bwd(const __grid_constant__ Nb2ModelDev<R> M, int B, int w0, int count, const float* __restrict__ state,
            const float* __restrict__ action, const R* __restrict__ saved, const float* __restrict__ gnext,
            float* __restrict__ gstate, float* __restrict__ gaction, float* __restrict__ ginertia, int words,
-           int stage_saved, int accumulate_state, unsigned in_stage_off, const double* __restrict__ winertia, double* __restrict__ ginertia_acc) {
+           int stage_saved, int accumulate_state, unsigned in_stage_off, const double* __restrict__ winertia, double* __restrict__ ginertia_acc, const void* __restrict__ body_tab) {
   extern __shared__ __align__(16) unsigned char nb2_smem[];
   NB2_CLK(1, 0);
   constexpr int WPW = CoopShape<K>::WPW, ST = CoopShape<K>::ST;
@@ -164,7 +167,7 @@
   const bool valid = slot < nworlds;
   const size_t wg = (size_t)w0 + (nworlds > 0 ? g0 : 0);
   const size_t w = wg + (valid ? slot : 0);
-  R* scr0 = reinterpret_cast<R*>(nb2_smem) + body_table_words<K>(M.nb) + (size_t)(threadIdx.x >> 5) * words * ST;
+  R* scr0 = reinterpret_cast<R*>(nb2_smem) + body_table_words<R, K>(M.nb, M.ndof) + (size_t)(threadIdx.x >> 5) * words * ST;
   R* scr = scr0 + slot;
   const float* g_src = gnext + wg * 2 * M.ndof;
   const float* st_src = state + wg * 2 * M.ndof;
@@ -191,7 +194,7 @@
   size_t svB = (size_t)B;
   if (stage_saved && nworlds == WPW) {
     const int sw = nb2_saved_words(M.nb, M.ndof, M.nfree);
-    R* svs = reinterpret_cast<R*>(nb2_smem) + ((body_table_words<K>(M.nb) + (size_t)(blockDim.x >> 5) * words * ST + 3) & ~(size_t)3)
+    R* svs = reinterpret_cast<R*>(nb2_smem) + ((body_table_words<R, K>(M.nb, M.ndof) + (size_t)(blockDim.x >> 5) * words * ST + 3) & ~(size_t)3)
              + (size_t)(threadIdx.x >> 5) * sw * WPW;
     constexpr int CH = (WPW * (int)sizeof(R)) / 16;
     const unsigned dst0 = (unsigned)__cvta_generic_to_shared(svs);
@@ -206,7 +209,7 @@
     svB = WPW;
   }
   constexpr unsigned sync_mask = (K > 1) ? NB2_BWD_SYNC_MASK : NB2_BWD_SYNC_MASK_1LANE;
-  const R* bt = stage_body_table<R, K>(M, reinterpret_cast<R*>(nb2_smem));
+  const R* bt = stage_body_table<R, K>(M, reinterpret_cast<R*>(nb2_smem), body_tab);
   if (bar) {
     __syncwarp();
     mbar_wait(bar, 0);
@@ -228,7 +231,7 @@
 template <class R, int K>
 __global__ void __launch_bounds__(128)
 k_id_fwd(const __grid_constant__ Nb2ModelDev<R> M, int B, const R* __restrict__ state, const R* __restrict__ next_vel, R* __restrict__ tau,
-         R* __restrict__ saved, int words, const double* __restrict__ winertia) {
+         R* __restrict__ saved, int words, const double* __restrict__ winertia, const void* __restrict__ body_tab) {
   extern __shared__ __align__(16) unsigned char nb2_smem[];
   constexpr int WPW = CoopShape<K>::WPW, ST = CoopShape<K>::ST;
   const int li = threadIdx.x & 31, slot = li / K, lane = li % K;
@@ -236,8 +239,8 @@
   const int nworlds = min(WPW, B - g0);
   const bool valid = slot < nworlds;
   const size_t wg = nworlds > 0 ? g0 : 0, w = wg + (valid ? slot : 0);
-  const R* bt = stage_body_table<R, K>(M, reinterpret_cast<R*>(nb2_smem));
-  R* scr0 = reinterpret_cast<R*>(nb2_smem) + body_table_words<K>(M.nb) + (size_t)(threadIdx.x >> 5) * words * ST;
+  const R* bt = stage_body_table<R, K>(M, reinterpret_cast<R*>(nb2_smem), body_tab);
+  R* scr0 = reinterpret_cast<R*>(nb2_smem) + body_table_words<R, K>(M.nb, M.ndof) + (size_t)(threadIdx.x >> 5) * words * ST;
   R* scr = scr0 + slot;
   R* sv = saved ? saved + w : nullptr;
   const double* wi = winertia ? winertia + w : nullptr;
@@ -254,7 +257,7 @@
 template <class R, int K>
 __global__ void __launch_bounds__(128)
 k_id_bwd(const __grid_constant__ Nb2ModelDev<R> M, int B, const R* __restrict__ state, const R* __restrict__ saved, const R* __restrict__ gtau,
-         R* __restrict__ gstate, R* __restrict__ gnext, double* __restrict__ ginertia, int words, const double* __restrict__ winertia) {
+         R* __restrict__ gstate, R* __restrict__ gnext, double* __restrict__ ginertia, int words, const double* __restrict__ winertia, const void* __restrict__ body_tab) {
   extern __shared__ __align__(16) unsigned char nb2_smem[];
   constexpr int WPW = CoopShape<K>::WPW, ST = CoopShape<K>::ST;
   const int li = threadIdx.x & 31, slot = li / K, lane = li % K;
@@ -262,8 +265,8 @@
   const int nworlds = min(WPW, B - g0);
   const bool valid = slot < nworlds;
   const size_t wg = nworlds > 0 ? g0 : 0, w = wg + (valid ? slot : 0);
-  const R* bt = stage_body_table<R, K>(M, reinterpret_cast<R*>(nb2_smem));
-  R* scr0 = reinterpret_cast<R*>(nb2_smem) + body_table_words<K>(M.nb) + (size_t)(threadIdx.x >> 5) * words * ST;
+  const R* bt = stage_body_table<R, K>(M, reinterpret_cast<R*>(nb2_smem), body_tab);
+  R* scr0 = reinterpret_cast<R*>(nb2_smem) + body_table_words<R, K>(M.nb, M.ndof) + (size_t)(threadIdx.x >> 5) * words * ST;
   R* scr = scr0 + slot;
   const double* wi = winertia ? winertia + w : nullptr;
   double* gI = ginertia ? ginertia + w : nullptr;
@@ -829,6 +832,7 @@
   int fwd_words, bwd_words, id_bwd_words;
   int depth;
   LaunchShape shape[4][2];
+  std::map<int, std::pair<void*, unsigned>> tab[2];
 };
 enum { LF_STEP_FWD = 0, LF_STEP_BWD = 1, LF_ID_FWD = 2, LF_ID_BWD = 3 };
 
@@ -853,6 +857,9 @@
   int hc_cap = 0;
   cudaStream_t host_streams[4] = {nullptr, nullptr, nullptr, nullptr};
   std::mutex mu;
+  std::atomic<unsigned> table_ver{1};
+  std::mutex tab_mu;
+  std::vector<void*> tab_retired;
 };
 
 template <class R> static const Nb2ModelDev<R>& model_of(const nb2_variant& v);
@@ -901,7 +908,7 @@
       dir == LF_ID_FWD ? (size_t)v.fwd_words * ST * sizeof(R) : dir == LF_ID_BWD ? (size_t)v.id_bwd_words * ST * sizeof(R) :
       (size_t)(dir ? v.bwd_words : v.fwd_words) * ST * sizeof(R) +
           (dir ? staging_bytes<K>(4 * v.mf.ndof + v.mf.na) : staging_bytes<K>(2 * v.mf.ndof + v.mf.na));
-  const size_t per_block = (size_t)body_table_words<K>(v.mf.nb) * sizeof(R) + 16;
+  const size_t per_block = (size_t)body_table_words<R, K>(v.mf.nb, v.mf.ndof) * sizeof(R) + 16;
   if (scratch_and_staging + per_block > (size_t)kMaxSmem) {
     g_err = "model needs " + std::to_string(scratch_and_staging) + " B of shared memory per warp (> 227 KB)"; return NB2_ERR_UNSUPPORTED;
   }
@@ -947,18 +954,60 @@
   return NB2_OK;
 }
 
+template <class R> static std::vector<unsigned char> body_table_image(const Nb2ModelDev<R>& M) {
+  using BT = nb2::BodyTab<R>;
+  std::vector<unsigned char> img((size_t)BT::bytes(M.nb, M.ndof), 0);
+  for (int i = 0; i < M.nb; i++) {
+    unsigned char* r = img.data() + (size_t)BT::REC * i;
+    memcpy(r, M.Xtree[i], 12 * sizeof(R));
+    memcpy(r + 12 * sizeof(R), M.inertia[i], 10 * sizeof(R));
+    const int16_t q[8] = {M.parent[i], M.jtype[i], M.dof_off[i], M.flags[i], M.slot_self[i], M.slot_parent[i], M.slot_count[i], M.free_idx[i]};
+    memcpy(r + BT::QUAD, q, sizeof(q));
+  }
+  for (int d = 0; d < M.ndof; d++) {
+    unsigned char* r = img.data() + (size_t)BT::REC * M.nb + (size_t)BT::DOF * d;
+    const R w[3] = {M.spring[d], M.damping[d], M.rest[d]};
+    const int a = M.act_of_dof[d];
+    const float c[6] = {M.pos_lo[d], M.pos_hi[d], M.vel_lo[d], M.vel_hi[d], M.force_lo[d], M.force_hi[d]};
+    memcpy(r, w, sizeof(w));
+    memcpy(r + 3 * sizeof(R), &a, sizeof(a));
+    memcpy(r + BT::CLIP, c, sizeof(c));
+  }
+  return img;
+}
+template <class R> static int body_table_dev(nb2_model* m, nb2_variant& v, cudaStream_t st, const void** out) {
+  *out = nullptr;
+  if (v.mf.lanes == 1) return NB2_OK;
+  int dev = 0;
+  NB2_CUDA(cudaGetDevice(&dev));
+  std::lock_guard<std::mutex> lk(m->tab_mu);
+  const unsigned ver = m->table_ver.load();
+  auto& e = v.tab[sizeof(R) == 8][dev];
+  if (!e.first || e.second != ver) {
+    const std::vector<unsigned char> img = body_table_image(model_of<R>(v));
+    void* p = nullptr;
+    NB2_CUDA(cudaMalloc(&p, img.size()));
+    const cudaError_t ce = cudaMemcpyAsync(p, img.data(), img.size(), cudaMemcpyHostToDevice, st);
+    if (ce != cudaSuccess) { cudaFree(p); g_err = std::string("body table copy: ") + cudaGetErrorString(ce); return NB2_ERR_CUDA; }
+    if (e.first) m->tab_retired.push_back(e.first);
+    e = {p, ver};
+  }
+  *out = e.first;
+  return NB2_OK;
+}
+
 template <class R, int K>
 static int launch_fwd_k(const nb2_variant& v, int sm_count, int Btot, int w0, int B, const float* state, const float* action,
-                        float* next, R* saved, cudaStream_t st, float* state_copy, float* action_copy, const double* wi) {
+                        float* next, R* saved, cudaStream_t st, float* state_copy, float* action_copy, const double* wi, const void* tab) {
   constexpr int WPW = CoopShape<K>::WPW, ST = CoopShape<K>::ST;
   const LaunchShape& sh = v.shape[0][sizeof(R) == 8];
   const size_t per_warp = (size_t)v.fwd_words * ST * sizeof(R) + staging_bytes<K>(2 * v.mf.ndof + v.mf.na);
   const int total_warps = (B + WPW - 1) / WPW;
   const int warps = block_warps(total_warps, sm_count, sh, per_warp);
   const int blocks = (total_warps + warps - 1) / warps;
-  const size_t smem = per_warp * warps + (size_t)body_table_words<K>(v.mf.nb) * sizeof(R) + 16;
-  if (wi) k_step_fwd<R, K, true><<<blocks, warps * 32, smem, st>>>(model_of<R>(v), Btot, w0, B, state, action, next, saved, v.fwd_words, state_copy, action_copy, wi);
-  else k_step_fwd<R, K, false><<<blocks, warps * 32, smem, st>>>(model_of<R>(v), Btot, w0, B, state, action, next, saved, v.fwd_words, state_copy, action_copy, nullptr);
+  const size_t smem = per_warp * warps + (size_t)body_table_words<R, K>(v.mf.nb, v.mf.ndof) * sizeof(R) + 16;
+  if (wi) k_step_fwd<R, K, true><<<blocks, warps * 32, smem, st>>>(model_of<R>(v), Btot, w0, B, state, action, next, saved, v.fwd_words, state_copy, action_copy, wi, tab);
+  else k_step_fwd<R, K, false><<<blocks, warps * 32, smem, st>>>(model_of<R>(v), Btot, w0, B, state, action, next, saved, v.fwd_words, state_copy, action_copy, nullptr, tab);
   g_launches++;
   NB2_CUDA(cudaGetLastError());
   return NB2_OK;
@@ -970,8 +1019,10 @@
   nb2_variant* pv = nullptr;
   int rc = pick_variant<R>(m, B, 0, &pv);
   if (rc) return rc;
+  const void* tab = nullptr;
+  if ((rc = body_table_dev<R>(m, *pv, st, &tab))) return rc;
   return with_lanes(pv->mf.lanes, [&](auto k) {
-    return launch_fwd_k<R, decltype(k)::value>(*pv, m->sm_count, Btot, w0, B, state, action, next, saved, st, state_copy, action_copy, wi);
+    return launch_fwd_k<R, decltype(k)::value>(*pv, m->sm_count, Btot, w0, B, state, action, next, saved, st, state_copy, action_copy, wi, tab);
   });
 }
 static bool no_stage_saved() {
@@ -981,14 +1032,14 @@
 template <class R, int K>
 static int launch_bwd_k(const nb2_variant& v, int sm_count, int Btot, int w0, int B, const float* state, const float* action,
                         const R* saved, const float* gnext, float* gstate, float* gaction, float* ginertia, cudaStream_t st, int accumulate,
-                        const double* wi, double* gIa) {
+                        const double* wi, double* gIa, const void* body_tab) {
   constexpr int WPW = CoopShape<K>::WPW, ST = CoopShape<K>::ST;
   const LaunchShape& sh = v.shape[1][sizeof(R) == 8];
   const size_t scratch_per_warp = (size_t)v.bwd_words * ST * sizeof(R);
   const int total_warps = (B + WPW - 1) / WPW;
   const int warps = block_warps(total_warps, sm_count, sh, scratch_per_warp);
   const int blocks = (total_warps + warps - 1) / warps;
-  const size_t tab = (size_t)body_table_words<K>(v.mf.nb) * sizeof(R);
+  const size_t tab = (size_t)body_table_words<R, K>(v.mf.nb, v.mf.ndof) * sizeof(R);
   const size_t stage_per_warp = (size_t)nb2_saved_words(v.mf.nb, v.mf.ndof, v.mf.nfree) * WPW * sizeof(R);
   const bool aligned = (((size_t)Btot * sizeof(R)) % 16 == 0) && (((size_t)w0 * sizeof(R)) % 16 == 0) && ((reinterpret_cast<size_t>(saved) & 15) == 0) &&
                        ((WPW * sizeof(R)) % 16 == 0);
@@ -1000,9 +1051,9 @@
   const bool in_stage = base + in_per_warp * warps <= (size_t)kMaxSmem;
   const size_t smem = in_stage ? base + in_per_warp * warps : base;
   if (wi || gIa) k_step_bwd<R, K, true><<<blocks, warps * 32, smem, st>>>(model_of<R>(v), Btot, w0, B, state, action, saved, gnext, gstate, gaction, ginertia,
-                                                                   v.bwd_words, stage ? 1 : 0, accumulate, in_stage ? (unsigned)base : 0u, wi, gIa);
+                                                                   v.bwd_words, stage ? 1 : 0, accumulate, in_stage ? (unsigned)base : 0u, wi, gIa, body_tab);
   else k_step_bwd<R, K, false><<<blocks, warps * 32, smem, st>>>(model_of<R>(v), Btot, w0, B, state, action, saved, gnext, gstate, gaction, ginertia,
-                                                                 v.bwd_words, stage ? 1 : 0, accumulate, in_stage ? (unsigned)base : 0u, nullptr, nullptr);
+                                                                 v.bwd_words, stage ? 1 : 0, accumulate, in_stage ? (unsigned)base : 0u, nullptr, nullptr, body_tab);
   g_launches++;
   NB2_CUDA(cudaGetLastError());
   return NB2_OK;
@@ -1015,23 +1066,26 @@
   nb2_variant* pv = nullptr;
   int rc = pick_variant<R>(m, B, 1, &pv);
   if (rc) return rc;
+  const void* tab = nullptr;
+  if ((rc = body_table_dev<R>(m, *pv, st, &tab))) return rc;
   return with_lanes(pv->mf.lanes, [&](auto k) {
-    return launch_bwd_k<R, decltype(k)::value>(*pv, m->sm_count, Btot, w0, B, state, action, saved, gnext, gstate, gaction, ginertia, st, accumulate, wi, gIa);
+    return launch_bwd_k<R, decltype(k)::value>(*pv, m->sm_count, Btot, w0, B, state, action, saved, gnext, gstate, gaction, ginertia, st, accumulate, wi, gIa,
+                                               tab);
   });
 }
 
 template <class R, int K>
 static int launch_id_k(const nb2_variant& v, int sm_count, int B, int dir, const R* state, const R* next_vel, R* tau, R* saved, const R* gtau,
-                       R* gstate, R* gnext, double* gI, const double* wi, cudaStream_t st) {
+                       R* gstate, R* gnext, double* gI, const double* wi, cudaStream_t st, const void* tab) {
   constexpr int WPW = CoopShape<K>::WPW, ST = CoopShape<K>::ST;
   const int words = dir == LF_ID_FWD ? v.fwd_words : v.id_bwd_words;
   const size_t per_warp = (size_t)words * ST * sizeof(R);
   const int total_warps = (B + WPW - 1) / WPW;
   const int warps = block_warps(total_warps, sm_count, v.shape[dir][sizeof(R) == 8], per_warp);
   const int blocks = (total_warps + warps - 1) / warps;
-  const size_t smem = per_warp * warps + (size_t)body_table_words<K>(v.mf.nb) * sizeof(R);
-  if (dir == LF_ID_FWD) k_id_fwd<R, K><<<blocks, warps * 32, smem, st>>>(model_of<R>(v), B, state, next_vel, tau, saved, words, wi);
-  else k_id_bwd<R, K><<<blocks, warps * 32, smem, st>>>(model_of<R>(v), B, state, saved, gtau, gstate, gnext, gI, words, wi);
+  const size_t smem = per_warp * warps + (size_t)body_table_words<R, K>(v.mf.nb, v.mf.ndof) * sizeof(R);
+  if (dir == LF_ID_FWD) k_id_fwd<R, K><<<blocks, warps * 32, smem, st>>>(model_of<R>(v), B, state, next_vel, tau, saved, words, wi, tab);
+  else k_id_bwd<R, K><<<blocks, warps * 32, smem, st>>>(model_of<R>(v), B, state, saved, gtau, gstate, gnext, gI, words, wi, tab);
   g_launches++;
   NB2_CUDA(cudaGetLastError());
   return NB2_OK;
@@ -1042,8 +1096,10 @@
   nb2_variant* pv = nullptr;
   int rc = pick_variant<R>(m, B, dir, &pv);
   if (rc) return rc;
+  const void* tab = nullptr;
+  if ((rc = body_table_dev<R>(m, *pv, st, &tab))) return rc;
   return with_lanes(pv->mf.lanes, [&](auto k) {
-    return launch_id_k<R, decltype(k)::value>(*pv, m->sm_count, B, dir, state, next_vel, tau, saved, gtau, gstate, gnext, gI, wi, st);
+    return launch_id_k<R, decltype(k)::value>(*pv, m->sm_count, B, dir, state, next_vel, tau, saved, gtau, gstate, gnext, gI, wi, st, tab);
   });
 }
 
@@ -1231,6 +1287,7 @@
   };
   put(m->mf, m->md);
   for (auto& v : m->variants) put(v.mf, v.md);
+  m->table_ver++;
   return NB2_OK;
 }
 int nb2_model_set_lanes(nb2_model* m, int lanes) {
@@ -1256,6 +1313,8 @@
   cudaFree(m->d_gnext); cudaFree(m->d_gstate); cudaFree(m->d_gaction);
   cudaFree(m->hc_ws); cudaFree(m->hc_x); cudaFree(m->hc_rec); cudaFree(m->hc_m); cudaFree(m->hc_labels); cudaFree(m->hc_status); cudaFree(m->hc_nc); cudaFree(m->hc_sticky);
   for (auto& hs : m->host_streams) if (hs) cudaStreamDestroy(hs);
+  for (auto& v : m->variants) for (auto& t : v.tab) for (auto& e : t) cudaFree(e.second.first);
+  for (void* p : m->tab_retired) cudaFree(p);
   delete m;
 }
 int nb2_model_has_contacts(const nb2_model* m) { return (m && m->has_contacts) ? 1 : 0; }
```

After: 70.13 million, median of 6. 1.08x the previous value.
